# RozDavid/LanguageGroundedSemseg

Measured on AMD Instinct MI355X. Metric: voxels/sec fwd+bwd Res16UNet34C @2cm ScanNet200, higher is better.
Workload: dtype bf16

## Files before the change

### include/lgs_engine.h

```cpp
#ifndef LGS_ENGINE_H
#define LGS_ENGINE_H

#include <stdint.h>

#ifdef __cplusplus
extern "C" {
#endif

#define LGS_ABI_VERSION 18

enum lgs_dtype { LGS_F32 = 0, LGS_BF16 = 1 };
enum lgs_supcon_distance { LGS_SUPCON_COS = 0, LGS_SUPCON_L2 = 1 };

typedef struct lgs_manager lgs_manager;
typedef struct lgs_kmap lgs_kmap;
typedef struct lgs_segmap lgs_segmap;

int lgs_abi_version(void);
const char *lgs_last_error(void);

int lgs_tuning_set(const char *name, int64_t value);
int lgs_tuning_get(const char *name, int64_t *value);
int64_t lgs_tuning_describe(char *buf, int64_t cap);
int64_t lgs_debug_dispatch_counts(char *buf, int64_t cap, int reset);

int lgs_manager_create(int device, lgs_manager **out);
int lgs_manager_destroy(lgs_manager *mgr);
int lgs_manager_insert(lgs_manager *mgr, const int32_t *coords, int64_t n, int64_t *unique_index,
                       int64_t *inverse, void *stream, int *key, int64_t *n_unique);

int lgs_manager_stride2(lgs_manager *mgr, int in_key, void *stream, int *out_key, int64_t *n_out);
int lgs_manager_check(lgs_manager *mgr, int *flags);

int lgs_manager_parent_of(lgs_manager *mgr, int key, int *fine_key);

int lgs_manager_map_size(lgs_manager *mgr, int key, int64_t *n, int *tensor_stride);
int lgs_manager_get_coords(lgs_manager *mgr, int key, int32_t *dst, void *stream);

int lgs_manager_kernel_map(lgs_manager *mgr, int in_key, int out_key, int kernel_size, void *stream,
                           lgs_kmap **out);

int lgs_manager_kernel_map_ex(lgs_manager *mgr, int in_key, int out_key, int kernel_size, int dilation, void *stream,
                              lgs_kmap **out);

typedef struct lgs_kmap_relation_query {
  int entry;
  int ks, dilation;
  int link;
  int tensor_stride;
  int out_sorted;
  int in_origin, out_origin;
} lgs_kmap_relation_query;
typedef struct lgs_kmap_relation_info {
  int rc;
  int relation;
  int K;
  int strided;
  int bwd_mirror;
  int transposed_ok;
  int pairs_only[2];
  int served_by_old_entry;
} lgs_kmap_relation_info;
int lgs_debug_kmap_relation(const lgs_kmap_relation_query *q, lgs_kmap_relation_info *out);

int lgs_kmap_export(lgs_kmap *km, int32_t *k, int32_t *in_row, int32_t *out_row, void *stream, int64_t *m);

int lgs_manager_origin(lgs_manager *mgr, void *stream, int *out_key, int64_t *n_out);
int lgs_manager_segment_map(lgs_manager *mgr, int fine_key, int coarse_key, void *stream, lgs_segmap **out);
int lgs_segmap_size(const lgs_segmap *sm, int64_t *n_fine, int64_t *n_coarse);
int64_t lgs_seg_workspace_bytes(const lgs_segmap *sm, int c);
int lgs_seg_reduce(lgs_segmap *sm, int op, const void *x, const void *x2, int64_t x_ld, int c, void *out, int32_t *argmax,
                   int dtype, void *workspace, void *stream);
int lgs_seg_broadcast(lgs_segmap *sm, int op, const void *g, int c, const void *x, int64_t x_ld, void *out, int64_t out_ld,
                      int dtype, void *stream);
int lgs_seg_max_backward(lgs_segmap *sm, const void *dy, const int32_t *argmax, int c, void *dx, int dtype, void *stream);

int64_t lgs_in_workspace_bytes(const lgs_segmap *sm, int c);
int lgs_in_forward(lgs_segmap *sm, const void *x, int c, const float *weight, const float *bias, float eps, void *y,
                   float *stats , int dtype, void *workspace, void *stream);
int lgs_in_backward(lgs_segmap *sm, const void *x, const void *dy, int c, const float *weight, const float *stats, void *dx,
                    float *dweight, float *dbias, int dtype, void *workspace, void *stream);

int64_t lgs_conv_workspace_bytes(const lgs_kmap *km, int cin, int cout, int dtype, int op );

typedef struct lgs_pack_desc {
  const float *weight;
  void *packed;
  int64_t bytes, total;
  int K, cin_w, cout_w, transposed, mirror, g_real, o_real, ncp, nbp, dtype;
} lgs_pack_desc;
int lgs_conv_pack_desc(const lgs_kmap *km, int op , int transposed, int cin, int cout, int dtype,
                       lgs_pack_desc *out);
int lgs_pack_weights_batch(const lgs_pack_desc *descs_device, int n, int64_t max_total, void *stream);

int lgs_conv_bn_partial_rows(const lgs_kmap *km, int transposed, int cout, int dtype);
int lgs_conv_forward(lgs_kmap *km, int transposed, const void *in, int cin, const float *weight, int cout,
                     const float *bias, void *out, int dtype, void *workspace, float *bn_partial, const float *bn_pivot,
                     void *packed, int pack_mode, int in_row_stride , void *stream);
int lgs_conv_dgrad(lgs_kmap *km, int transposed, const void *grad_out, int cout, const float *weight, int cin,
                   void *grad_in, int dtype, void *workspace, void *packed, int pack_mode, void *stream);

int lgs_conv_dgrad_can_accumulate(const lgs_kmap *km, int transposed, int cin, int cout, int dtype);
int lgs_conv_dgrad_accumulate(lgs_kmap *km, int transposed, const void *grad_out, int cout, const float *weight, int cin,
                              void *grad_in, int dtype, void *workspace, void *packed, int pack_mode, void *stream);
int lgs_conv_wgrad(lgs_kmap *km, int transposed, const void *in, int cin, const void *grad_out, int cout,
                   float *grad_weight, int dtype, void *workspace, int in_row_stride , void *stream);
int lgs_conv_wgrad_supports_stride(const lgs_kmap *km, int transposed, int cin, int cout, int dtype, int in_row_stride);

typedef struct lgs_conv_plan_view {
  int64_t n_pad, n_in, n_out;
  int KS, K;
  int has_nbr, has_tile_k, has_out_row;
} lgs_conv_plan_view;
typedef struct lgs_conv_plan_query {
  lgs_conv_plan_view fwd, bwd;
  int ks;
  int op, transposed, cin, cout, dtype;
  int epilogue;
} lgs_conv_plan_query;
typedef struct lgs_conv_plan_region { int64_t offset, bytes; } lgs_conv_plan_region;
typedef struct lgs_conv_plan_info {
  int path;
  int tile_id, sc, wb, tm;
  int nc, nb_total, ncp, nbp, gc, wld;
  int64_t total;
  int pad_input, scratch_out, packed_ext_ok, split, bn_rows, can_accumulate;
  int64_t grid_x; int grid_y, grid_z;
  lgs_conv_plan_region packed, padded_in, scratch, bias, partials;
  int64_t bytes_total;
  int64_t workspace_bytes;
  int q_bn_partial_rows, q_can_accumulate;
  lgs_pack_desc pack_desc;
} lgs_conv_plan_info;
int lgs_debug_conv_plan(const lgs_conv_plan_query *q, lgs_conv_plan_info *out);

typedef struct lgs_wgrad_plan_query {
  lgs_conv_plan_view fwd, bwd;
  int ks, transposed, cin, cout, dtype, in_row_stride;
} lgs_wgrad_plan_query;
typedef struct lgs_wgrad_plan_info {
  int path;
  int bwd_view;
  int in_place;
  int pad_in, pad_gout;
  int all_cus;
  int f32_kernel;
  int t0, t1;
  int pad_a, pad_b;
  int slots;
  int64_t span;
  int n_ranges, kpw;
  int tasks_a, tasks_b;
  int cpl, n_chunks, xcd_map;
  int ntile;
  int64_t grid_x; int grid_y, grid_z, lds_bytes;
  int64_t reduce_blocks;
  lgs_conv_plan_region partials, padded_in, padded_gout, ww_count, ww_offset, ww_total, ww_pair_in, ww_pair_out;
  int64_t bytes_total;
  int64_t workspace_bytes;
  int supports_stride;
} lgs_wgrad_plan_info;
int lgs_debug_wgrad_plan(const lgs_wgrad_plan_query *q, lgs_wgrad_plan_info *out);

int64_t lgs_bn_workspace_bytes(int64_t n, int c);
int lgs_bn_forward(const void *x, int64_t n, int c, const float *gamma, const float *beta, float eps,
                   float momentum, float *running_mean, float *running_var, int64_t *num_batches_tracked,
                   const void *residual, int relu, void *y, float *stats, int dtype, void *workspace,
                   const float *conv_partials , int conv_partial_rows,
                   const float *pivot , int64_t y_row_stride ,
                   void *stream);
int lgs_bn_backward(const void *x, const void *y, const void *dy, int64_t dy_row_stride, int64_t n, int c,
                    const float *gamma, const float *beta, const float *stats, int relu, void *dx, void *dresidual,
                    float *dgamma, float *dbeta, int dtype, void *workspace, int64_t y_row_stride ,
                    void *stream);

int lgs_bn_stats(const void *x, int64_t n, int c, float *rec , int dtype, void *workspace,
                 const float *conv_partials, int conv_partial_rows, const float *pivot, void *stream);
int lgs_bn_sync_combine(const float *all_stats, int world, int c, float eps, float momentum, float *running_mean,
                        float *running_var, int64_t *num_batches_tracked, float *stats, float *inv_n_total, void *stream);
int lgs_bn_apply(const void *x, int64_t n, int c, const float *gamma, const float *beta, const float *stats,
                 const void *residual, int relu, void *y, int dtype, int64_t y_row_stride, void *stream);
int lgs_bn_backward_reduce(const void *x, const void *y, const void *dy, int64_t n, int c, const float *gamma,
                           const float *beta, const float *stats, int relu, float *sums, float *dgamma, float *dbeta,
                           int dtype, void *workspace, int64_t dy_row_stride, int64_t y_row_stride, void *stream);
int lgs_bn_backward_apply(const void *x, const void *y, const void *dy, int64_t n, int c, const float *gamma,
                          const float *beta, const float *stats, const float *sums, float inv_n_total,
                          const float *inv_n_device, int relu, void *dx, void *dresidual, int dtype, int64_t dy_row_stride,
                          int64_t y_row_stride, void *stream);

typedef struct lgs_norm_plan_query {
  int direction;
  int c, dtype;
  int conv_partial_rows;
  int resident_cap;
  int64_t n;
} lgs_norm_plan_query;
typedef struct lgs_norm_plan_info {
  int path;
  int from_partials;
  int reduce_grid;
  int64_t rows_per_block;
  int partial_rpb;
  int fold_rows;
  int fold_grid;
  int apply_grid;
  lgs_conv_plan_region partials, sums, spill;
  int64_t bytes_total;
  int64_t workspace_bytes;
} lgs_norm_plan_info;
int lgs_debug_norm_plan(const lgs_norm_plan_query *q, lgs_norm_plan_info *out);

struct lgs_bn_params;
typedef struct lgs_norm_pair_plan_info {
  int path;
  int single_path;
  int launches;
  int reduce_grid;
  int64_t rows_per_block;
  int fold_rows, fold_grid, apply_grid;
  lgs_conv_plan_region partials_a, partials_b, sums_a, sums_b;
  int64_t bytes_total;
  int64_t workspace_bytes;
} lgs_norm_pair_plan_info;
int64_t lgs_bn_pair_workspace_bytes(int64_t n, int c);
int lgs_bn_pair_plan(int direction , int64_t n, int c, int dtype, lgs_norm_pair_plan_info *out);
int lgs_debug_norm_pair_plan(const lgs_norm_plan_query *q , lgs_norm_pair_plan_info *out);
int lgs_bn_forward_pair(const void *xa, const struct lgs_bn_params *norm_a, float *stats_a, const void *xb,
                        const struct lgs_bn_params *norm_b, float *stats_b, int64_t n, int c, int relu, void *y,
                        int64_t y_row_stride , void *res , int dtype, void *workspace, void *stream);
int lgs_bn_backward_pair(const void *xa, const void *ya, const float *gamma_a, const float *beta_a, const float *stats_a, int relu,
                         const void *xb, const float *gamma_b, const float *stats_b, const void *dy, int64_t dy_row_stride,
                         int64_t n, int c, void *dxa, void *dxb, float *dgamma_a, float *dbeta_a, float *dgamma_b, float *dbeta_b,
                         void *dresidual , int dtype, void *workspace, int64_t ya_row_stride ,
                         void *stream);

typedef struct lgs_instnorm_plan_query {
  int direction;
  int c, dtype;
  int64_t n_fine, n_seg, n_items;
} lgs_instnorm_plan_query;
typedef struct lgs_instnorm_plan_info {
  int vec;
  int lanes_log2;
  int rows_per_apply_block;
  int64_t reduce_grid;
  int64_t combine_grid;
  int64_t apply_grid;
  lgs_conv_plan_region partials, sums;
  int64_t bytes_total;
  int64_t workspace_bytes;
} lgs_instnorm_plan_info;
int lgs_debug_instnorm_plan(const lgs_instnorm_plan_query *q, lgs_instnorm_plan_info *out);

typedef struct lgs_seg_plan_query {
  int family;
  int c, dtype;
  int single_pass;
  int vec_ok;
  int64_t n_fine, n_coarse, n_items;
} lgs_seg_plan_query;
typedef struct lgs_seg_plan_info {
  int vec;
  int lanes_log2;
  int combine_lanes_log2;
  int64_t reduce_grid;
  int64_t combine_grid;
  int64_t bcast_grid;
  int64_t max_bwd_grid;
  lgs_conv_plan_region partials, partial_argmax;
  int64_t bytes_total;
  int64_t workspace_bytes;
} lgs_seg_plan_info;
int lgs_debug_seg_plan(const lgs_seg_plan_query *q, lgs_seg_plan_info *out);

typedef struct lgs_comm lgs_comm;
int lgs_comm_unique_id(void *id128);
int lgs_comm_create(const void *id128, int world, int rank, int device, lgs_comm **out);
int lgs_comm_create_ipc(int world, int rank, int device, lgs_comm **out, void *handle64);
int lgs_comm_ipc_open(lgs_comm *comm, const void *handles64);
int lgs_comm_destroy(lgs_comm *comm);
int lgs_comm_world(const lgs_comm *comm);
int64_t lgs_bn_sync_workspace_bytes(int64_t n, int c, int world);
int lgs_bn_forward_sync(lgs_comm *comm, const void *x, int64_t n, int c, const float *gamma, const float *beta, float eps,
                        float momentum, float *running_mean, float *running_var, int64_t *num_batches_tracked,
                        const void *residual, int relu, void *y, float *stats, float *inv_n, int dtype, void *workspace,
                        int64_t y_row_stride, void *stream);
int lgs_bn_backward_sync(lgs_comm *comm, const void *x, const void *y, const void *dy, int64_t n, int c, const float *gamma,
                         const float *beta, const float *stats, const float *inv_n, int relu, void *dx, void *dresidual,
                         float *dgamma, float *dbeta, int dtype, void *workspace, int64_t dy_row_stride, int64_t y_row_stride,
                         void *stream);

typedef struct lgs_bn_params {
  const float *gamma, *beta;
  float *running_mean, *running_var;
  int64_t *num_batches_tracked;
  float eps, momentum;
} lgs_bn_params;
typedef struct lgs_block_fwd {
  lgs_kmap *km3, *km1;
  int dtype, relu_final, cin, planes;
  int64_t n;
  const void *x;
  const float *w1, *w2, *wd;
  void *pk1, *pk2, *pkd;
  int pm1, pm2, pmd;
  lgs_bn_params n1, n2, nd;
  void *o1, *y1, *o2, *od, *res, *y2;
  float *st1, *st2, *std_;
  void *conv_ws, *bn_ws;
} lgs_block_fwd;
typedef struct lgs_block_bwd {
  lgs_kmap *km3, *km1;
  int dtype, relu_final, cin, planes, want_gin, x_row_stride;
  int64_t n, dy_row_stride;
  const void *dy;
  const void *x, *o1, *y1, *o2, *y2, *od;
  const float *st1, *st2, *std_;
  const float *w1, *w2, *wd;
  void *pk1, *pk2, *pkd;
  int pm1, pm2, pmd;
  const float *gamma1, *beta1, *gamma2, *beta2, *gammad, *betad;
  void *dx2, *dres, *dy1, *dx1, *dxd, *gind;
  float *gw1, *gw2, *gwd;
  float *dgamma1, *dbeta1, *dgamma2, *dbeta2, *dgammad, *dbetad;
  void *conv_ws, *bn_ws;
  void *wgrad_stream, *wgrad_ws, *fork_event, *ev_w1, *ev_w2, *ev_wd;
} lgs_block_bwd;
int64_t lgs_block_workspace_bytes(const lgs_kmap *km3, const lgs_kmap *km1, int cin, int planes, int dtype);
int lgs_block_forward(const lgs_block_fwd *args, void *stream);
int lgs_block_backward(const lgs_block_bwd *args, void *stream);

int lgs_clip_similarity(const void *feat, int64_t n, int c, const float *anchors, int n_anchor, float *sim,
                        float *inv_norm_f, int dtype, void *workspace, void *stream);
int64_t lgs_clip_workspace_bytes(int c, int n_anchor, int dtype);

int64_t lgs_clip_loss_workspace_bytes(int c, int n_anchor, int dtype);
int lgs_clip_loss_forward(const void *feat, int64_t n, int c, const float *anchors, int n_anchor, const int64_t *labels,
                          const int64_t *neg, int k_neg, int64_t ignore_label, float *d_pos, float *d_neg, int64_t *pred,
                          float *inv_norm_f, float *anchors_n, float *sim, int dtype, void *workspace, void *stream);
int lgs_clip_loss_backward(const void *feat, int64_t n, int c, const float *anchors_n, int n_anchor, const int64_t *labels,
                           const int64_t *neg, int k_neg, int64_t ignore_label, const float *inv_norm_f, const float *d_pos,
                           const float *d_neg, const float *g_dpos, const float *g_dneg, void *grad_feat, int dtype,
                           void *stream);
int64_t lgs_clip_anchor_grad_workspace_bytes(int64_t n, int c, int n_anchor, int dtype);
int lgs_clip_loss_backward_anchors(const void *feat, int64_t n, int c, int n_anchor, const int64_t *labels, const int64_t *neg,
                                   int k_neg, int64_t ignore_label, const float *inv_norm_f, const float *g_dpos,
                                   const float *g_dneg, float *grad_anchors_t, int dtype, void *workspace, void *stream);

int lgs_sgd_step(float *params, const float *grads, float *momentum_buf, const float *mask, int64_t n, float lr,
                 float momentum, float dampening, float weight_decay, int first_step, void *stream);

int lgs_voxelize(const float *points, int64_t n, const double *affine, int batch, int32_t *coords, void *stream);
int lgs_label_vote(const int64_t *labels, int64_t n, const int64_t *unique_index, const int64_t *inverse,
                   int64_t n_unique, int64_t ignore_label, int64_t *labels_out, void *stream);

int64_t lgs_cluster_workspace_bytes(int64_t n);
int lgs_cluster(const float *xyz, const int32_t *batch_idx, const int32_t *semantic_label, int64_t n, float radius,
                int threshold, int32_t *component, int32_t *n_clusters, void *workspace, void *stream);

int lgs_ce_forward_backward(const void *logits, int64_t n, int c, const int64_t *labels, int64_t ignore_index,
                            const float *scale, float *loss_rows, void *dlogits, int dtype, void *stream);
int lgs_ce_forward_backward_rows(const void *logits, int64_t n, int c, const int64_t *labels, int64_t ignore_index,
                                 const float *scale, const float *row_scale, float *loss_rows, void *dlogits, int dtype,
                                 void *stream);
int lgs_split_stats(const float *loss_rows, const int64_t *labels, int64_t n, const int32_t *group_of_class, int n_classes,
                    int64_t ignore_index, float *partial, int partial_rows, void *stream);
int lgs_ce_count_valid(const int64_t *labels, int64_t n, int c, int64_t ignore_index, int32_t *count, void *stream);

// ... 54 lines not shown
```

### languagegroundedsemseg_amd/csrc/lgs_common.h

```cpp
#pragma once
#include <hip/hip_runtime.h>
#include <stdint.h>
#include <stdio.h>
#include <string>
#include <vector>

#include "../../include/lgs_engine.h"

struct lgs_kmap;
struct lgs_segmap;

namespace lgs {

void set_error(const std::string &msg);

#define LGS_HIP(expr)                                                                              \
  do {                                                                                             \
    hipError_t _e = (expr);                                                                        \
    if (_e != hipSuccess) {                                                                        \
      lgs::set_error(std::string(#expr) + " failed: " + hipGetErrorString(_e) + " (" __FILE__ ":" + \
                     std::to_string(__LINE__) + ")");                                              \
      return 1;                                                                                    \
    }                                                                                              \
  } while (0)

#define LGS_REQUIRE(cond, msg)                                                     \
  do {                                                                             \
    if (!(cond)) {                                                                 \
      lgs::set_error(std::string(msg) + " [" #cond "] (" __FILE__ ":" + std::to_string(__LINE__) + ")"); \
      return 2;                                                                    \
    }                                                                              \
  } while (0)

enum Tune {
  T_WW_MIN_ROWS, T_WW_RANGE, T_WGRAD_WIDE, T_BN_FUSED, T_BN_FUSED_MAX_MB, T_BN_FUSED_FWD_MAX_MB, T_BN_FUSED_BLOCKS, T_PS_CUS, T_PS_WIDE3, T_WGRAD_PS,
  T_MASK_WINDOW, T_CONV_SPLIT, T_SMALL_CFG, T_WIDE_GC64, T_ARENA_DBG, T_CONV_WIDE, T_MASK_ORDER,
  T_BN_FOLD, T_BN_FOLD_MAX_MB, T_BN_FOLD_PARTS, T_BN_FOLD_GRID, T_FP32_SPLIT, T_BLOCK_WGRAD_LATE, T_WGRAD_F32_LDS, T_WIDE_SCHED, T_HEAD_TILE, T_POINTWISE,
  T_INSTANCE_NORM, T_METRICS_BLOCKS, T_SUPCON_FUSED, T_BN_PAIR,
  T_COUNT
};
int64_t tune(Tune t);
int dispatch_site(const char *kernel_text, const char *pretty_function);
void dispatch_hit(int site);
#define LGS_KLAUNCH(kernel, ...)                                                                 \
  do {                                                                                           \
    static const int _lgs_site = lgs::dispatch_site(#kernel, __PRETTY_FUNCTION__);               \
    lgs::dispatch_hit(_lgs_site);                                                                \
    hipLaunchKernelGGL(kernel, __VA_ARGS__);                                                     \
  } while (0)

constexpr int kPadRows = 256;
constexpr int kGroup = 64;

inline int64_t pad_rows(int64_t n) { return (n + kPadRows - 1) / kPadRows * kPadRows; }

struct View {
  const int32_t *nbr = nullptr;
  const uint32_t *mask64 = nullptr;
  const int32_t *tile_k = nullptr;
  const int32_t *out_row = nullptr;
  int64_t n_pad = 0;
  int64_t n_out = 0;
  int64_t n_in = 0;
  int KS = 1;
  int K = 1;
  int mirror = 0;
};

constexpr int kSegChunk = 512;
struct SegMap {
  const int32_t *fine_row = nullptr;
  const int32_t *seg_start = nullptr;
  const int32_t *coarse_of = nullptr;
  const int32_t *item_start = nullptr;
  const int32_t *item_seg = nullptr;
  const int32_t *row_seg = nullptr;
  int64_t n_fine = 0, n_coarse = 0, n_items = 0;
  int64_t max_len = 0;
  bool single_pass() const { return max_len > 0 && max_len <= kSegChunk; }
};

inline int pad32(int c) { return (c + 31) / 32 * 32; }
inline int esize(int dtype) { return dtype == LGS_BF16 ? 2 : 4; }
inline int epl(int dtype) { return dtype == LGS_BF16 ? 8 : 4; }
inline int64_t align256(int64_t b) { return (b + 255) / 256 * 256; }

#if defined(__HIPCC__)
using f32x16 = __attribute__((ext_vector_type(16))) float;
using bf16x8 = __attribute__((ext_vector_type(8))) __bf16;
typedef uint16_t bf16_t;
__device__ inline float bf16_to_f32(uint16_t b) { return __uint_as_float((uint32_t)b << 16); }
__device__ inline uint16_t f32_to_bf16(float f) {
  uint32_t u = __float_as_uint(f);
  u += 0x7fffu + ((u >> 16) & 1u);
  return (uint16_t)(u >> 16);
}
__device__ inline float ld_elem(const float *p) { return *p; }
__device__ inline float ld_elem(const bf16_t *p) { return bf16_to_f32(*p); }
template <typename T>
__global__ void k_pad_rows(const T *__restrict__ src, int64_t n, int c, int cpad, T *__restrict__ dst) {
  int64_t i = (int64_t)blockIdx.x * blockDim.x + threadIdx.x;
  if (i >= n * cpad) return;
  int64_t r = i / cpad;
  int ch = (int)(i % cpad);
  dst[i] = ch < c ? src[r * c + ch] : (T)0;
}
#define LGS_AS3(p) ((__attribute__((address_space(3))) void *)(p))
#define LGS_VMCNT(n) __builtin_amdgcn_s_waitcnt((((n) & 15) | (7 << 4) | (15 << 8) | (((n) >> 4) << 14)))
#endif

using WgradPlan = lgs_wgrad_plan_info;
enum WgradPath { kWgEmpty = 0, kWgWide = 1, kWgPs = 2, kWgPairs = 3, kWgF32 = 4 };
int64_t wgrad_workspace_bytes(const lgs_kmap *km, int cin, int cout, int dtype);
inline lgs_conv_plan_region take_region(int64_t &used, int64_t bytes) {
  const lgs_conv_plan_region r = {used, align256(bytes)};
  used += r.bytes;
  return r;
}
bool pointwise_supported(const View &v, int K, int g_real, int o_real, int64_t in_ld);
int launch_pointwise(const View &v, const void *in, int64_t in_ld, int g_real, const float *w, int cin_w, int cout_w, int transposed,
                     int o_real, const float *bias, void *out, hipStream_t s);
bool pointwise_f32_supported(const View &v, int K, int g_real, int o_real, int64_t in_ld);
int launch_pointwise_f32(const View &v, const void *in, int64_t in_ld, int g_real, const float *w, int cin_w, int cout_w, int transposed,
                         int o_real, const float *bias, void *out, hipStream_t s);
int launch_conv_wide(const View &v, const void *in, int cin_real, int in_ld, const void *wp, int nb_total, int ncp, int nbp, int K,
                     void *out, int cout_real, const float *bias, int gc64, hipStream_t s);
bool wgrad_wide_plan(const View &v, int cin, int cout, int in_ld, WgradPlan &p);
int launch_wgrad_wide(const View &v, const WgradPlan &p, const void *in, int cin, int in_ld, const void *gout, int cout, float *gw,
                      void *workspace, hipStream_t s);
int kmap_wait(lgs_kmap *km, hipStream_t stream);
int segmap_wait(lgs_segmap *sm, hipStream_t stream);

}

namespace lgs {
enum KmapRelation {
  kRelIdentity = 0,
  kRelConv3 = 1,
  kRelConv2S2 = 2,
  kRelConv3Dilated = 3,
  kRelConv3S2 = 4,
  kRelConv1S2 = 5,
};
struct KmapTraits {
  int ks, K;
  bool strided;
  bool bwd_mirror;
  bool transposed_ok;
  bool old_entry;
  constexpr bool wgrad_pairs_only(bool transposed) const { return ks == 3 && (strided || transposed); }
};
constexpr KmapTraits traits_of(KmapRelation r) {
  switch (r) {
    case kRelConv3:        return KmapTraits{3, 27, false, true, false, true};
    case kRelConv2S2:      return KmapTraits{2, 8, true, false, true, true};
    case kRelConv3Dilated: return KmapTraits{3, 27, false, true, true, false};
    case kRelConv3S2:      return KmapTraits{3, 27, true, false, true, false};
    case kRelConv1S2:      return KmapTraits{1, 1, true, false, true, false};
    default:               return KmapTraits{1, 1, false, false, true, true};
  }
}
constexpr int kCoordBits = 18;
struct KmapRequest {
  bool ex;
  bool same_key;
  bool out_is_stride2;
  bool out_sorted;
  bool origin;
  int ks, dilation, ts_in;
};
inline const char *classify_kmap(const KmapRequest &q, KmapRelation &rel) {
  if (q.origin) return q.ex ? "lgs_manager_kernel_map_ex: no kernel maps on the origin map" : "lgs_manager_kernel_map: no kernel maps on the origin map";
  const int d = q.ex ? q.dilation : 1;
  const bool strided = !q.same_key && q.out_is_stride2;
  if (d < 1) return "lgs_manager_kernel_map_ex: dilation must be >= 1";
  if (strided && d > 1) return "lgs_manager_kernel_map_ex: stride 2 combined with dilation > 1 is not supported";
  if (d > 1 && q.ks != 3) return "lgs_manager_kernel_map_ex: dilation > 1 needs kernel_size 3";
  if (d > 1) {
    if (!q.same_key) return "lgs_manager_kernel_map_ex: out_key must be in_key or stride2(in_key)";
    rel = kRelConv3Dilated;
  } else if (q.ks == 1 || q.ks == 3) {
    const char *refusal = q.ks == 1 ? "kernel_size 1 needs in_key == out_key" : "kernel_size 3 is supported for stride 1 (in_key == out_key) only";
    if (!q.same_key && !strided) return refusal;
    rel = q.ks == 1 ? (strided ? kRelConv1S2 : kRelIdentity) : (strided ? kRelConv3S2 : kRelConv3);
    if (!q.ex && !traits_of(rel).old_entry) return refusal;
  } else if (q.ks == 2) {
    if (!strided) return "kernel_size 2 needs out_key == stride2(in_key)";
    rel = kRelConv2S2;
  } else {
    return "unsupported kernel_size (the model family uses 1, 2 and 3 only)";
  }
  if (!traits_of(rel).old_entry) {
    if (strided && !q.out_sorted) return "lgs_manager_kernel_map_ex: the stride-2 map's rows are not in sorted order";
    if ((int64_t)d * q.ts_in >= (1ll << (kCoordBits - 1))) return "lgs_manager_kernel_map_ex: dilation * tensor_stride must stay below 2^17";
  }
  return nullptr;
}
}

struct lgs_kmap {
  lgs_manager *mgr = nullptr;
  int in_key = -1, out_key = -1, ks = 1, K = 1;
  lgs::KmapRelation relation = lgs::kRelIdentity;
  int dilation = 1;
  lgs::View fwd;
  lgs::View bwd;
};

namespace lgs {
inline KmapTraits traits_of(const lgs_kmap *km) { return traits_of(km->relation); }
inline const char *synthetic_kmap_relation(lgs_kmap &km) {
  const bool same = km.ks != 2 && km.fwd.n_in == km.fwd.n_out;
  const char *refusal = classify_kmap(KmapRequest{true, same, !same, true, false, km.ks, 1, 1}, km.relation);
  if (!refusal) km.bwd.mirror = traits_of(km.relation).bwd_mirror ? 1 : 0;
  return refusal;
}
}

struct lgs_segmap {
  lgs_manager *mgr = nullptr;
  int fine_key = -1, coarse_key = -1;
  lgs::SegMap sm;
};
```

### languagegroundedsemseg_amd/csrc/lgs_manager.hip

```cpp
#include "lgs_common.h"

#include <cstring>
#include <memory>
#include <rocprim/rocprim.hpp>

namespace lgs {

static thread_local std::string g_err;
void set_error(const std::string &msg) { g_err = msg; }

constexpr int kBias = 1 << (kCoordBits - 1);
constexpr uint64_t kEmpty = ~0ull;

__host__ __device__ inline uint64_t spread3(uint64_t x) {
  x &= 0x1fffff;
  x = (x | x << 32) & 0x1f00000000ffffull;
  x = (x | x << 16) & 0x1f0000ff0000ffull;
  x = (x | x << 8) & 0x100f00f00f00f00full;
  x = (x | x << 4) & 0x10c30c30c30c30c3ull;
  x = (x | x << 2) & 0x1249249249249249ull;
  return x;
}
__host__ __device__ inline uint32_t compact3(uint64_t x) {
  x &= 0x1249249249249249ull;
  x = (x ^ (x >> 2)) & 0x10c30c30c30c30c3ull;
  x = (x ^ (x >> 4)) & 0x100f00f00f00f00full;
  x = (x ^ (x >> 8)) & 0x1f0000ff0000ffull;
  x = (x ^ (x >> 16)) & 0x1f00000000ffffull;
  x = (x ^ (x >> 32)) & 0x1fffff;
  return (uint32_t)x;
}
__device__ inline uint64_t pack_key(int b, int xb, int yb, int zb) {
  return ((uint64_t)b << 54) | spread3((uint64_t)xb) | (spread3((uint64_t)yb) << 1) | (spread3((uint64_t)zb) << 2);
}
__device__ inline void unpack_key(uint64_t key, int &b, int &xb, int &yb, int &zb) {
  b = (int)(key >> 54);
  uint64_t m = key & ((1ull << 54) - 1);
  xb = (int)compact3(m);
  yb = (int)compact3(m >> 1);
  zb = (int)compact3(m >> 2);
}
__device__ inline uint64_t hash64(uint64_t k) {
  k ^= k >> 33; k *= 0xff51afd7ed558ccdull; k ^= k >> 33; k *= 0xc4ceb9fe1a85ec53ull; k ^= k >> 33;
  return k;
}

__global__ void k_pack_keys(const int32_t *coords, int64_t n, uint64_t *keys, int32_t *vals, int *err) {
  int64_t i = (int64_t)blockIdx.x * blockDim.x + threadIdx.x;
  if (i >= n) return;
  int4 c = reinterpret_cast<const int4 *>(coords)[i];
  bool ok = c.x >= 0 && c.x < 1024 && c.y > -kBias && c.y < kBias - 64 && c.z > -kBias && c.z < kBias - 64 &&
            c.w > -kBias && c.w < kBias - 64;
  if (!ok) { atomicOr(err, 1); c = make_int4(0, 0, 0, 0); }
  keys[i] = pack_key(c.x, c.y + kBias, c.z + kBias, c.w + kBias);
  vals[i] = (int32_t)i;
}

__global__ void k_heads(const uint64_t *skeys, int64_t n, uint64_t keep_mask, int32_t *head) {
  int64_t p = (int64_t)blockIdx.x * blockDim.x + threadIdx.x;
  if (p >= n) return;
  uint64_t k = skeys[p] & keep_mask;
  head[p] = (p == 0 || (skeys[p - 1] & keep_mask) != k) ? 1 : 0;
}

__global__ void k_mark_first(const int32_t *svals, const int32_t *head, int64_t n, int32_t *is_first) {
  int64_t p = (int64_t)blockIdx.x * blockDim.x + threadIdx.x;
  if (p >= n) return;
  is_first[svals[p]] = head[p];
}
__global__ void k_emit_unique(const int32_t *coords, const int32_t *is_first, const int32_t *urow, int64_t n,
                              int32_t *ucoords, int64_t *unique_index) {
  int64_t i = (int64_t)blockIdx.x * blockDim.x + threadIdx.x;
  if (i >= n || !is_first[i]) return;
  int32_t u = urow[i];
  reinterpret_cast<int4 *>(ucoords)[u] = reinterpret_cast<const int4 *>(coords)[i];
  if (unique_index) unique_index[u] = i;
}
__global__ void k_emit_sorted(const uint64_t *skeys, const int32_t *svals, const int32_t *head,
                              const int32_t *runid_incl, const int32_t *urow, int64_t n, uint64_t *ukeys,
                              int32_t *order) {
  int64_t p = (int64_t)blockIdx.x * blockDim.x + threadIdx.x;
  if (p >= n || !head[p]) return;
  int32_t q = runid_incl[p] - 1;
  ukeys[q] = skeys[p];
  order[q] = urow[svals[p]];
}
__global__ void k_emit_inverse(const int32_t *svals, const int32_t *runid_incl, const int32_t *order, int64_t n,
                               int64_t *inverse) {
  int64_t p = (int64_t)blockIdx.x * blockDim.x + threadIdx.x;
  if (p >= n) return;
  inverse[svals[p]] = order[runid_incl[p] - 1];
}

__global__ void k_emit_coarse(const uint64_t *fkeys, const int32_t *head, const int32_t *cidx_incl, int64_t n,
                              uint64_t keep_mask, uint64_t *ckeys, int32_t *ccoords, int32_t *cstart,
                              int32_t *fine_cidx, int64_t nc, int *d_err) {
  int64_t p = (int64_t)blockIdx.x * blockDim.x + threadIdx.x;
  if (p >= n) return;
  int32_t q = cidx_incl[p] - 1;
  fine_cidx[p] = q;
  if (p == n - 1 && (int64_t)q + 1 != nc && d_err) atomicOr(d_err, 2);
  if (q >= nc) return;
  if (head[p]) {
    uint64_t k = fkeys[p] & keep_mask;
    ckeys[q] = k;
    cstart[q] = (int32_t)p;
    int b, x, y, z;
    unpack_key(k, b, x, y, z);
    reinterpret_cast<int4 *>(ccoords)[q] = make_int4(b, x - kBias, y - kBias, z - kBias);
  }
  if (p == n - 1) cstart[q + 1] = (int32_t)n;
}

__global__ void k_hash_fill(uint64_t *hkeys, int64_t cap) {
  int64_t i = (int64_t)blockIdx.x * blockDim.x + threadIdx.x;
  if (i < cap) hkeys[i] = kEmpty;
}
__global__ void k_hash_insert(const uint64_t *skeys, const int32_t *order, int64_t n, uint64_t *hkeys,
                              int32_t *hvals, uint64_t capm1) {
  int64_t p = (int64_t)blockIdx.x * blockDim.x + threadIdx.x;
  if (p >= n) return;
  uint64_t key = skeys[p];
  uint64_t s = hash64(key) & capm1;
  for (;;) {
    unsigned long long prev = atomicCAS(reinterpret_cast<unsigned long long *>(hkeys + s), (unsigned long long)kEmpty,
                                        (unsigned long long)key);
    if (prev == kEmpty) { hvals[s] = order ? order[p] : (int32_t)p; return; }
    s = (s + 1) & capm1;
  }
}

constexpr int kPreLevels = 8;
constexpr int kCountPerThread = 16;
constexpr int kBatchShift = 54;
__global__ __launch_bounds__(256) void k_count_levels(const uint64_t *__restrict__ skeys, int64_t n, int32_t *__restrict__ counts) {
  __shared__ int32_t l_cnt[kPreLevels + 1];
  if (threadIdx.x <= kPreLevels) l_cnt[threadIdx.x] = 0;
  __syncthreads();
  int32_t c[kPreLevels + 1];
#pragma unroll
  for (int L = 0; L <= kPreLevels; ++L) c[L] = 0;
  const int64_t base = (int64_t)blockIdx.x * 256 * kCountPerThread;
#pragma unroll 4
  for (int i = 0; i < kCountPerThread; ++i) {
    const int64_t p = base + (int64_t)i * 256 + threadIdx.x;
    if (p >= n) break;
    const uint64_t k = skeys[p], q = p > 0 ? skeys[p - 1] : ~0ull, d = k ^ q;
#pragma unroll
    for (int L = 1; L <= kPreLevels; ++L) c[L - 1] += (p == 0 || (d >> (3 * L)) != 0) ? 1 : 0;
    c[kPreLevels] += (p == 0 || (d >> kBatchShift) != 0) ? 1 : 0;
  }
#pragma unroll
  for (int L = 0; L <= kPreLevels; ++L) {
    int32_t v = c[L];
#pragma unroll
    for (int o = 32; o > 0; o >>= 1) v += __shfl_down(v, o, 64);
    if ((threadIdx.x & 63) == 0 && v) atomicAdd(&l_cnt[L], v);
  }
  __syncthreads();
  if (threadIdx.x <= kPreLevels && l_cnt[threadIdx.x]) atomicAdd(&counts[threadIdx.x], l_cnt[threadIdx.x]);
}

__global__ void k_build_map3(const uint64_t *skeys, int64_t n, int64_t n_pad, int ts, const uint64_t *hkeys,
                             const int32_t *hvals, uint64_t capm1, int32_t *nbr, uint32_t *pmask) {
  int64_t p = (int64_t)blockIdx.x * blockDim.x + threadIdx.x;
  bool live = p < n;
  int b = 0, x = 0, y = 0, z = 0;
  if (live) unpack_key(skeys[p], b, x, y, z);
  uint32_t m = 0;
#pragma unroll 1
  for (int g = 0; g < 3; ++g) {
    uint64_t key[9], slot[9], hk[9];
    bool ok[9];
    const int zz = z + (g - 1) * ts;
#pragma unroll
    for (int j = 0; j < 9; ++j) {
      const int xx = x + (j % 3 - 1) * ts, yy = y + (j / 3 - 1) * ts;
      ok[j] = live && (((unsigned)xx | (unsigned)yy | (unsigned)zz) < (1u << kCoordBits));
      key[j] = ok[j] ? pack_key(b, xx, yy, zz) : 0ull;
      slot[j] = hash64(key[j]) & capm1;
    }
#pragma unroll
    for (int j = 0; j < 9; ++j) hk[j] = ok[j] ? hkeys[slot[j]] : kEmpty;
#pragma unroll
    for (int j = 0; j < 9; ++j) {
      if (ok[j]) {
        uint64_t cur = hk[j], sl = slot[j];
        while (cur != key[j] && cur != kEmpty) {
          sl = (sl + 1) & capm1;
          cur = hkeys[sl];
        }
        slot[j] = sl;
        ok[j] = cur == key[j];
      }
    }
    int32_t r[9];
#pragma unroll
    for (int j = 0; j < 9; ++j) r[j] = ok[j] ? hvals[slot[j]] : -1;
#pragma unroll
    for (int j = 0; j < 9; ++j) {
      const int k = 9 * g + j;
      nbr[(int64_t)k * n_pad + p] = r[j];
      if (r[j] >= 0) m |= 1u << k;
    }
  }
  pmask[p] = m;
}

constexpr int kMaskWindow = 16384;
__device__ inline uint32_t mask_sort_code(uint32_t m, int order) {
  if (order == 0) return m;
  if (order == 3) return ((uint32_t)__popc(m) << 27) | m;
  uint32_t corner = 0, edge = 0, face = 0, centre = (m >> 13) & 1u;
  int nc = 0, ne = 0, nf = 0;
#pragma unroll
  for (int k = 0; k < 27; ++k) {
    const int dx = k % 3 - 1, dy = (k / 3) % 3 - 1, dz = k / 9 - 1;
    const int cls = (dx != 0) + (dy != 0) + (dz != 0);
    const uint32_t b = (m >> k) & 1u;
    if (cls == 3) corner |= b << nc++;
    else if (cls == 2) edge |= b << ne++;
    else if (cls == 1) face |= b << nf++;
  }
  if (order == 1) return (corner << 19) | (edge << 7) | (face << 1) | centre;
  return (face << 21) | (edge << 9) | (corner << 1) | centre;
}
__global__ void k_mask_sort_keys(const uint32_t *pmask, int64_t n, int64_t n_pad, int window, int order, uint64_t *keys, int32_t *vals) {
  int64_t p = (int64_t)blockIdx.x * blockDim.x + threadIdx.x;
  if (p >= n_pad) return;
  keys[p] = p < n ? (((uint64_t)(p / window)) << 32) | mask_sort_code(pmask[p], order) : ~0ull;
  vals[p] = (int32_t)p;
}
inline unsigned mask_sort_bits(int64_t n_pad, int window) {
  const uint64_t nw = (uint64_t)((n_pad + window - 1) / window);
  unsigned wb = 1;
  while ((1ull << wb) - 1 < nw) ++wb;
  return 32u + wb > 64u ? 64u : 32u + wb;
}
__global__ void k_permute_map3(const int32_t *nbr_tmp, const uint32_t *pmask, const int32_t *perm, const int32_t *order,
                               int64_t n, int64_t n_pad, int32_t *nbr, int32_t *out_row, uint32_t *mask64) {
  int64_t q = (int64_t)blockIdx.x * blockDim.x + threadIdx.x;
  int32_t src = q < n ? perm[q] : -1;
  uint32_t pm = src >= 0 ? pmask[src] : 0u;
  out_row[q] = src >= 0 ? (order ? order[src] : src) : -1;
  uint32_t m = 0;
  for (int k = 0; k < 27; ++k) {
    nbr[(int64_t)k * n_pad + q] = src >= 0 ? nbr_tmp[(int64_t)k * n_pad + src] : -1;
    if (__ballot((pm >> k) & 1u)) m |= 1u << k;
  }
  if ((threadIdx.x & 63) == 0) mask64[q >> 6] = m;
}

__global__ void k_build_map3_fine(const uint64_t *fkeys, int64_t n, int64_t n_pad, int log2ts, const uint64_t *hkeys,
                                  const int32_t *hvals, uint64_t capm1, int32_t *nbr, uint32_t *pmask) {
  int64_t p = (int64_t)blockIdx.x * blockDim.x + threadIdx.x;
  const bool live = p < n;
  int b = 0, x = 0, y = 0, z = 0;
  if (live) unpack_key(fkeys[p], b, x, y, z);
  const int ts = 1 << log2ts;
  const int ox = (x >> log2ts) & 1, oy = (y >> log2ts) & 1, oz = (z >> log2ts) & 1;
  uint64_t key[8], slot[8], hk[8];
  int kk[8];
  bool ok[8];
#pragma unroll
  for (int j = 0; j < 8; ++j) {
    const int jx = j & 1, jy = (j >> 1) & 1, jz = j >> 2;
    const int dx = ox ? 2 * jx - 1 : 0, dy = oy ? 2 * jy - 1 : 0, dz = oz ? 2 * jz - 1 : 0;
    const int xx = x - dx * ts, yy = y - dy * ts, zz = z - dz * ts;
    ok[j] = live && (ox || !jx) && (oy || !jy) && (oz || !jz) && (((unsigned)xx | (unsigned)yy | (unsigned)zz) < (1u << kCoordBits));
    kk[j] = (dx + 1) + 3 * (dy + 1) + 9 * (dz + 1);
    key[j] = ok[j] ? pack_key(b, xx, yy, zz) : 0ull;
    slot[j] = hash64(key[j]) & capm1;
  }
#pragma unroll
  for (int j = 0; j < 8; ++j) hk[j] = ok[j] ? hkeys[slot[j]] : kEmpty;
#pragma unroll
  for (int j = 0; j < 8; ++j) {
    if (ok[j]) {
      uint64_t cur = hk[j], sl = slot[j];
      while (cur != key[j] && cur != kEmpty) {
        sl = (sl + 1) & capm1;
        cur = hkeys[sl];
      }
      slot[j] = sl;
      ok[j] = cur == key[j];
    }
  }
  uint32_t m = 0;
#pragma unroll
  for (int j = 0; j < 8; ++j)
    if (ok[j]) m |= 1u << kk[j];
  int32_t r[8];
#pragma unroll
  for (int j = 0; j < 8; ++j) r[j] = ok[j] ? hvals[slot[j]] : -1;
  for (int k = 0; k < 27; ++k) {
    int32_t v = -1;
#pragma unroll
    for (int j = 0; j < 8; ++j)
      if (ok[j] && kk[j] == k) v = r[j];
    nbr[(int64_t)k * n_pad + p] = v;
  }
  pmask[p] = m;
}

__global__ void k_build_map1_coarse(const uint64_t *fkeys, const int32_t *forder, const uint64_t *ckeys, const int32_t *cstart,
                                    int64_t n_c, int64_t nc_pad, int32_t *nbr) {
  int64_t q = (int64_t)blockIdx.x * blockDim.x + threadIdx.x;
  if (q >= nc_pad) return;
  int32_t r = -1;
  if (q < n_c) {
    const int32_t p = cstart[q];
    if (fkeys[p] == ckeys[q]) r = forder ? forder[p] : p;
  }
  nbr[q] = r;
}
__global__ void k_build_map1_fine(const uint64_t *fkeys, const int32_t *forder, const int32_t *fine_cidx, int64_t n, int64_t n_pad,
                                  uint64_t child_bits, int32_t *nbr, int32_t *out_row) {
  int64_t p = (int64_t)blockIdx.x * blockDim.x + threadIdx.x;
  if (p >= n_pad) return;
  const bool live = p < n;
  nbr[p] = (live && (fkeys[p] & child_bits) == 0) ? fine_cidx[p] : -1;
  out_row[p] = live ? (forder ? forder[p] : (int32_t)p) : -1;
}

__global__ void k_build_map2_coarse(const uint64_t *fkeys, const int32_t *forder, const int32_t *cstart,
                                    int64_t n_c, int64_t nc_pad, int shift, int32_t *nbr8, uint32_t *mask64) {
  int64_t q = (int64_t)blockIdx.x * blockDim.x + threadIdx.x;
  int32_t child[8];
#pragma unroll
  for (int k = 0; k < 8; ++k) child[k] = -1;
  if (q < n_c) {
    int32_t s = cstart[q], e = cstart[q + 1];
    for (int32_t p = s; p < e; ++p) {
      int k = (int)((fkeys[p] >> shift) & 7);
      int32_t row = forder ? forder[p] : p;
#pragma unroll
      for (int j = 0; j < 8; ++j)
        if (j == k) child[j] = row;
    }
  }
  uint32_t m = 0;
#pragma unroll
  for (int k = 0; k < 8; ++k) {
    nbr8[(int64_t)k * nc_pad + q] = child[k];
    if (__ballot(child[k] >= 0)) m |= 1u << k;
  }
  if ((threadIdx.x & 63) == 0) mask64[q >> 6] = m;
}

__global__ void k_child_keys(const uint64_t *fkeys, int64_t n, int shift, uint32_t *kk, int32_t *pp, int32_t *cnt) {
  __shared__ int32_t h[8];
  if (threadIdx.x < 8) h[threadIdx.x] = 0;
  __syncthreads();
  int64_t p = (int64_t)blockIdx.x * blockDim.x + threadIdx.x;
  if (p < n) {
    uint32_t k = (uint32_t)((fkeys[p] >> shift) & 7);
    kk[p] = k;
    pp[p] = (int32_t)p;
    atomicAdd(&h[k], 1);
  }
  __syncthreads();
  if (threadIdx.x < 8 && h[threadIdx.x]) atomicAdd(&cnt[threadIdx.x], h[threadIdx.x]);
}
__global__ void k_group_offsets(const int32_t *cnt, int32_t *goff , int32_t *gsrc ) {
  if (threadIdx.x == 0 && blockIdx.x == 0) {
    int32_t a = 0, b = 0;
    for (int k = 0; k < 8; ++k) {
      goff[k] = a; gsrc[k] = b;
      a += (cnt[k] + kPadRows - 1) / kPadRows * kPadRows;
      b += cnt[k];
    }
    goff[8] = a; gsrc[8] = b;
  }
}
__global__ void k_fill_i32(int32_t *p, int64_t n, int32_t v) {
  int64_t i = (int64_t)blockIdx.x * blockDim.x + threadIdx.x;
  if (i < n) p[i] = v;
}
__global__ void k_build_map2_fine(const uint32_t *kk_sorted, const int32_t *pp_sorted, int64_t n, const int32_t *goff,
                                  const int32_t *gsrc, const int32_t *fine_cidx, const int32_t *forder,
                                  int32_t *g_nbr, int32_t *g_out, int32_t *tile_k) {
  int64_t s = (int64_t)blockIdx.x * blockDim.x + threadIdx.x;
  if (s >= n) return;
  int k = (int)kk_sorted[s];
  int32_t p = pp_sorted[s];
  int32_t slot = goff[k] + ((int32_t)s - gsrc[k]);
  g_nbr[slot] = fine_cidx[p];
  g_out[slot] = forder ? forder[p] : p;
  if (((s - gsrc[k]) & (kGroup - 1)) == 0) tile_k[slot >> 6] = k;
}

__global__ void k_view_count(View v, int32_t *count) {
  int64_t p = (int64_t)blockIdx.x * blockDim.x + threadIdx.x;
  if (p >= v.n_pad) return;
  int32_t orow = v.out_row ? v.out_row[p] : (p < v.n_out ? (int32_t)p : -1);
  int c = 0;
  if (orow >= 0) {
    if (!v.nbr) c = 1;
    else
      for (int s = 0; s < v.KS; ++s) c += v.nbr[(int64_t)s * v.n_pad + p] >= 0;
  }
  if (c) atomicAdd(count, c);
}
__global__ void k_view_export(View v, int32_t *cursor, int32_t *ek, int32_t *ein, int32_t *eout) {
  int64_t p = (int64_t)blockIdx.x * blockDim.x + threadIdx.x;
  if (p >= v.n_pad) return;
  int32_t orow = v.out_row ? v.out_row[p] : (p < v.n_out ? (int32_t)p : -1);
  if (orow < 0) return;
  for (int s = 0; s < v.KS; ++s) {
    int32_t i = v.nbr ? v.nbr[(int64_t)s * v.n_pad + p] : (int32_t)p;
    if (i < 0) continue;
    int k = v.tile_k ? v.tile_k[p >> 6] : (v.mirror ? v.K - 1 - s : s);
    int32_t at = atomicAdd(cursor, 1);
    ek[at] = k; ein[at] = i; eout[at] = orow;
  }
}

__global__ void k_origin_coords(const uint64_t *skeys, const int32_t *head, const int32_t *cincl, int64_t n, int64_t nb,
                                int32_t *coords, int *d_err) {
  int64_t p = (int64_t)blockIdx.x * blockDim.x + threadIdx.x;
  if (p >= n) return;
  const int32_t q = cincl[p] - 1;
  if (p == n - 1 && (int64_t)q + 1 != nb && d_err) atomicOr(d_err, 4);
  if (q >= nb || !head[p]) return;
  reinterpret_cast<int4 *>(coords)[q] = make_int4((int)(skeys[p] >> kBatchShift), 0, 0, 0);
}
__global__ void k_origin_segments(const int32_t *head, const int32_t *cincl, int64_t n, int64_t nb, int32_t *seg_start,
                                  int32_t *coarse_of) {
  int64_t p = (int64_t)blockIdx.x * blockDim.x + threadIdx.x;
  if (p >= n) return;
  const int32_t q = cincl[p] - 1;
  coarse_of[p] = q < nb ? q : (int32_t)(nb - 1);
  if (q >= nb) return;
  if (head[p]) seg_start[q] = (int32_t)p;
  if (p == n - 1) seg_start[q + 1] = (int32_t)n;
}
__global__ void k_row_seg(const int32_t *fine_row, const int32_t *coarse_of, int64_t n, int32_t *row_seg) {
  int64_t p = (int64_t)blockIdx.x * blockDim.x + threadIdx.x;
  if (p >= n) return;
  const int32_t r = fine_row[p];
  if (r >= 0 && r < n) row_seg[r] = coarse_of[p];
}
constexpr int kMaxChain = 12;
struct Chain {
  const int32_t *fine_cidx[kMaxChain];
  const int32_t *cstart[kMaxChain];
  int k;
};
__global__ void k_compose_coarse_of(Chain ch, int64_t n, int32_t *coarse_of) {
  int64_t p = (int64_t)blockIdx.x * blockDim.x + threadIdx.x;
  if (p >= n) return;
  int32_t v = (int32_t)p;
  for (int j = 0; j < ch.k; ++j) v = ch.fine_cidx[j][v];
  coarse_of[p] = v;
}
__global__ void k_compose_seg_start(Chain ch, int64_t nc, int32_t *seg_start) {
  int64_t q = (int64_t)blockIdx.x * blockDim.x + threadIdx.x;
  if (q > nc) return;
  int32_t v = (int32_t)q;
  for (int j = ch.k - 1; j >= 0; --j) v = ch.cstart[j][v];
  seg_start[q] = v;
}
__global__ void k_item_counts(const int32_t *seg_start, int64_t nc, int32_t *cnt) {
  int64_t q = (int64_t)blockIdx.x * blockDim.x + threadIdx.x;
  if (q >= nc) return;
  cnt[q] = (seg_start[q + 1] - seg_start[q] + kSegChunk - 1) / kSegChunk;
}
__global__ void k_item_fill(const int32_t *item_start, int64_t nc, int64_t n_items, int32_t *item_seg) {
  int64_t q = (int64_t)blockIdx.x * blockDim.x + threadIdx.x;
  if (q >= nc) return;
  for (int32_t j = item_start[q]; j < item_start[q + 1] && j < n_items; ++j) item_seg[j] = (int32_t)q;
}

struct CoordMap {
  int ts = 1, log2ts = 0;
  int64_t n = 0, n_pad = 0;
  int32_t *coords = nullptr;
  int32_t *order = nullptr;
  uint64_t *skeys = nullptr;
  uint64_t *hkeys = nullptr;
  int32_t *hvals = nullptr;
  int64_t hcap = 0;
  int fine_key = -1, coarse_key = -1;
  bool origin = false;
  int32_t *cstart = nullptr;
  int32_t *fine_cidx = nullptr;
};

}

using namespace lgs;

struct lgs_manager {
  int device = 0;
  hipMemPool_t pool = nullptr;
  hipStream_t ms = nullptr;
  hipEvent_t ev_ready = nullptr, ev_in = nullptr;
  std::vector<hipStream_t> users;
  hipStream_t last_stream = nullptr;
  std::vector<CoordMap> maps;
  std::vector<lgs_kmap *> kmaps;
  std::vector<void *> allocs;
  int *d_err = nullptr;
  char *arena = nullptr;
  size_t arena_cap = 0, arena_used = 0, arena_peak = 0;
  struct Blk { size_t off, size; bool freed; };
  std::vector<Blk> blks;
  size_t pool_live = 0, pool_peak = 0;
  int64_t precount[8] = {-1, -1, -1, -1, -1, -1, -1, -1};
  int64_t precount_batches = -1;
  int origin_key = -1;
  std::vector<lgs_segmap *> segmaps;
};

namespace {

struct DeviceGuard {
  int prev = -1;
  bool switched = false;
  explicit DeviceGuard(int dev) {
    if (hipGetDevice(&prev) == hipSuccess && prev != dev) switched = hipSetDevice(dev) == hipSuccess;
  }
  ~DeviceGuard() {
    if (switched) (void)hipSetDevice(prev);
  }
};

hipMemPool_t g_pool[64] = {nullptr};
int ensure_pool(int device) {
  if (g_pool[device]) return 0;
  hipMemPoolProps props;
  memset(&props, 0, sizeof(props));
  props.allocType = hipMemAllocationTypePinned;
  props.handleTypes = hipMemHandleTypeNone;
  props.location.type = hipMemLocationTypeDevice;
  props.location.id = device;
  hipMemPool_t pool = nullptr;
  LGS_HIP(hipMemPoolCreate(&pool, &props));
  uint64_t thr = UINT64_MAX;
  LGS_HIP(hipMemPoolSetAttribute(pool, hipMemPoolAttrReleaseThreshold, &thr));
  int off = 0;
  (void)hipMemPoolSetAttribute(pool, hipMemPoolReuseAllowInternalDependencies, &off);
  g_pool[device] = pool;
  return 0;
}
struct ArenaBlock { char *base; size_t cap; std::vector<hipEvent_t> ready; };
std::vector<ArenaBlock> g_arenas[64];
size_t g_arena_need[64] = {0};

inline hipError_t pool_alloc(lgs_manager *m, void **q, size_t bytes, hipStream_t s) {
  return hipMallocFromPoolAsync(q, bytes, m->pool, s);
}
int raw_alloc(lgs_manager *m, void **p, size_t bytes, hipStream_t s) {
  bytes = (bytes + 255) / 256 * 256;
  if (m->arena && m->arena_used + bytes <= m->arena_cap) {
    *p = m->arena + m->arena_used;
    m->blks.push_back({m->arena_used, bytes, false});
    m->arena_used += bytes;
    if (m->arena_used > m->arena_peak) m->arena_peak = m->arena_used;
    return 0;
  }
  void *q = nullptr;
  LGS_HIP(pool_alloc(m, &q, bytes, s));
  m->allocs.push_back(q);
  m->pool_live += bytes;
  if (m->pool_live > m->pool_peak) m->pool_peak = m->pool_live;
  *p = q;
  return 0;
}
template <typename T>
int dalloc(lgs_manager *m, T **p, int64_t count, hipStream_t s) {
  void *q = nullptr;
  if (raw_alloc(m, &q, sizeof(T) * (size_t)(count > 0 ? count : 1), s)) return 1;
  *p = reinterpret_cast<T *>(q);
  return 0;
}
int dfree_now(lgs_manager *m, void *q, hipStream_t s) {
  char *c = reinterpret_cast<char *>(q);
  if (m->arena && c >= m->arena && c < m->arena + m->arena_cap) {
    const size_t off = (size_t)(c - m->arena);
    for (size_t i = m->blks.size(); i-- > 0;)
      if (m->blks[i].off == off) { m->blks[i].freed = true; break; }
    while (!m->blks.empty() && m->blks.back().freed) { m->arena_used = m->blks.back().off; m->blks.pop_back(); }
    return 0;
  }
  for (size_t i = 0; i < m->allocs.size(); ++i)
    if (m->allocs[i] == q) { m->allocs[i] = m->allocs.back(); m->allocs.pop_back(); break; }
  LGS_HIP(hipFreeAsync(q, s));
  return 0;
}
int arena_acquire(lgs_manager *m) {
  const int dev = m->device;
  const size_t need = g_arena_need[dev];
  if (need == 0) return 0;
  std::vector<ArenaBlock> &q = g_arenas[dev];
  for (size_t i = 0; q.size() >= 2 && i + 1 < q.size(); ++i) {
    if (q[i].cap >= need) {
      ArenaBlock b = q[i];
      q.erase(q.begin() + (long)i);
      if (tune(T_ARENA_DBG)) {
        int pending = 0;
        for (hipEvent_t e : b.ready) pending += hipEventQuery(e) == hipSuccess ? 0 : 1;
        fprintf(stderr, "[arena] reuse block %zu of %zu (cap %zu MB, need %zu MB): %d of %zu events still pending\n", i, q.size() + 1, b.cap >> 20,
                need >> 20, pending, b.ready.size());
      }
      for (hipEvent_t e : b.ready) { (void)hipStreamWaitEvent(m->ms, e, 0); (void)hipEventDestroy(e); }
      m->arena = b.base; m->arena_cap = b.cap;
      return 0;
    }
    if (i == 0 && q.size() >= 4) {
      for (hipEvent_t e : q[0].ready) { (void)hipEventSynchronize(e); (void)hipEventDestroy(e); }
      (void)hipFree(q[0].base);
      q.erase(q.begin());
      i = (size_t)-1;
    }
  }
  const size_t cap = (need + need / 4 + (2u << 20)) / (2u << 20) * (2u << 20);
  if (tune(T_ARENA_DBG)) fprintf(stderr, "[arena] hipMalloc %zu MB (need %zu MB, %zu queued)\n", cap >> 20, need >> 20, q.size());
  void *p = nullptr;
  if (hipMalloc(&p, cap) != hipSuccess) { (void)hipGetLastError(); return 0; }
  m->arena = reinterpret_cast<char *>(p); m->arena_cap = cap;
  return 0;
}
void arena_release(lgs_manager *m) {
  const size_t need = m->arena_peak + m->pool_peak;
  if (need > g_arena_need[m->device]) g_arena_need[m->device] = need;
  if (!m->arena) return;
  ArenaBlock b{m->arena, m->arena_cap, {}};
  std::vector<hipStream_t> streams = m->users;
  streams.push_back(m->ms);
  for (hipStream_t u : streams) {
    hipEvent_t e = nullptr;
    if (hipEventCreateWithFlags(&e, hipEventDisableTiming) == hipSuccess) {
      if (hipEventRecord(e, u) == hipSuccess) b.ready.push_back(e); else (void)hipEventDestroy(e);
    }
  }
  g_arenas[m->device].push_back(b);
  m->arena = nullptr;
}
void add_user(lgs_manager *m, hipStream_t caller) {
  for (hipStream_t u : m->users)
    if (u == caller) return;
  m->users.push_back(caller);
}
int begin_from_caller(lgs_manager *m, hipStream_t caller) {
  LGS_HIP(hipEventRecord(m->ev_in, caller));
  LGS_HIP(hipStreamWaitEvent(m->ms, m->ev_in, 0));
  return 0;
}
int publish(lgs_manager *m, hipStream_t caller, bool caller_waits) {
  LGS_HIP(hipEventRecord(m->ev_ready, m->ms));
  if (caller_waits) {
    LGS_HIP(hipStreamWaitEvent(caller, m->ev_ready, 0));
    add_user(m, caller);
  }
  return 0;
}
inline unsigned nblk(int64_t n, int t = 256) { return (unsigned)((n + t - 1) / t > 0 ? (n + t - 1) / t : 1); }

int ensure_hash(lgs_manager *m, CoordMap &cm, hipStream_t s) {
  if (cm.hkeys) return 0;
  int64_t cap = 1024;
  while (cap < 2 * cm.n) cap <<= 1;
  cm.hcap = cap;
  if (dalloc(m, &cm.hkeys, cap, s)) return 1;
  if (dalloc(m, &cm.hvals, cap, s)) return 1;
  LGS_KLAUNCH(k_hash_fill, nblk(cap), 256, 0, s, cm.hkeys, cap);
  if (cm.n > 0)
    LGS_KLAUNCH(k_hash_insert, nblk(cm.n), 256, 0, s, cm.skeys, cm.order, cm.n, cm.hkeys, cm.hvals,
                       (uint64_t)(cap - 1));
  LGS_HIP(hipGetLastError());
  return 0;
}

int scan_incl(lgs_manager *m, const int32_t *in, int32_t *out, int64_t n, hipStream_t s) {
  size_t tb = 0;
  LGS_HIP(rocprim::inclusive_scan(nullptr, tb, in, out, (size_t)n, rocprim::plus<int32_t>(), s));
  void *tmp = nullptr;
  if (raw_alloc(m, &tmp, tb ? tb : 16, s)) return 1;
  LGS_HIP(rocprim::inclusive_scan(tmp, tb, in, out, (size_t)n, rocprim::plus<int32_t>(), s));
  if (dfree_now(m, tmp, s)) return 1;
  return 0;
}

template <typename K, typename V>
int sort_pairs(lgs_manager *m, K *keys, K *keys_out, V *vals, V *vals_out, int64_t n, unsigned begin_bit, unsigned end_bit, hipStream_t s) {
  size_t tb = 0;
  LGS_HIP(rocprim::radix_sort_pairs(nullptr, tb, keys, keys_out, vals, vals_out, (size_t)n, begin_bit, end_bit, s));
  void *tmp = nullptr;
  if (raw_alloc(m, &tmp, tb ? tb : 16, s)) return 1;
  LGS_HIP(rocprim::radix_sort_pairs(tmp, tb, keys, keys_out, vals, vals_out, (size_t)n, begin_bit, end_bit, s));
  return dfree_now(m, tmp, s);
}

int batch_heads(lgs_manager *m, const uint64_t *skeys, int64_t n, int32_t *head, int32_t *cincl, hipStream_t s) {
  LGS_KLAUNCH(k_heads, nblk(n), 256, 0, s, skeys, n, ~((1ull << kBatchShift) - 1), head);
  return scan_incl(m, head, cincl, n, s);
}

int sort_map3(lgs_manager *m, int64_t n, int64_t n_pad, const int32_t *nbr_tmp, const uint32_t *pmask, const int32_t *order, uint64_t *keys,
              uint64_t *skeys2, int32_t *vals, int32_t *perm, int32_t *nbr, int32_t *orow, uint32_t *mask, hipStream_t s) {
  const int window = (int)tune(T_MASK_WINDOW);
  LGS_KLAUNCH(k_mask_sort_keys, (unsigned)(n_pad / 256), 256, 0, s, pmask, n, n_pad, window, (int)tune(T_MASK_ORDER), keys, vals);
  if (sort_pairs(m, keys, skeys2, vals, perm, n_pad, 0, mask_sort_bits(n_pad, window), s)) return 1;
  LGS_KLAUNCH(k_permute_map3, (unsigned)(n_pad / 256), 256, 0, s, nbr_tmp, pmask, perm, order, n, n_pad, nbr, orow, mask);
  LGS_HIP(hipGetLastError());
  return 0;
}

template <typename Build>
int make_view27(lgs_manager *m, const CoordMap &st, int64_t n_in, hipStream_t s, View &v, Build &&build) {
  v = View();
  v.n_pad = st.n_pad; v.n_out = st.n; v.n_in = n_in; v.KS = 27; v.K = 27;
  if (st.n == 0) return 0;
  int32_t *nbr, *orow, *nbr_tmp, *vals, *perm; uint32_t *mask, *pmask; uint64_t *keys, *skeys2;
  if (dalloc(m, &nbr, 27 * st.n_pad, s) || dalloc(m, &mask, st.n_pad / kGroup, s) || dalloc(m, &orow, st.n_pad, s) ||
      dalloc(m, &nbr_tmp, 27 * st.n_pad, s) || dalloc(m, &pmask, st.n_pad, s) || dalloc(m, &keys, st.n_pad, s) ||
      dalloc(m, &skeys2, st.n_pad, s) || dalloc(m, &vals, st.n_pad, s) || dalloc(m, &perm, st.n_pad, s))
    return 1;
  if (build(nbr_tmp, pmask)) return 1;
  if (sort_map3(m, st.n, st.n_pad, nbr_tmp, pmask, st.order, keys, skeys2, vals, perm, nbr, orow, mask, s)) return 1;
  if (dfree_now(m, nbr_tmp, s) || dfree_now(m, pmask, s) || dfree_now(m, keys, s) || dfree_now(m, skeys2, s) ||
      dfree_now(m, vals, s) || dfree_now(m, perm, s))
    return 1;
  v.nbr = nbr; v.mask64 = mask; v.out_row = orow;
  return 0;
}


void build_identity(const CoordMap &ci, lgs_kmap *km) {
  View v; v.n_pad = ci.n_pad; v.n_out = ci.n; v.n_in = ci.n; v.KS = 1; v.K = 1;
  km->fwd = v; km->bwd = v;
}

int probe_view27(lgs_manager *m, const CoordMap &st, const CoordMap &probed, int scale, hipStream_t s, View &v) {
  return make_view27(m, st, probed.n, s, v, [&](int32_t *nbr_tmp, uint32_t *pmask) {
    LGS_KLAUNCH(k_build_map3, (unsigned)(st.n_pad / 256), 256, 0, s, st.skeys, st.n, st.n_pad, scale, probed.hkeys, probed.hvals,
                (uint64_t)(probed.hcap - 1), nbr_tmp, pmask);
    return 0;
  });
}

int build_conv3(lgs_manager *m, CoordMap &ci, int dilation, hipStream_t s, lgs_kmap *km) {
  if (ci.n > 0 && ensure_hash(m, ci, s)) return 1;
  View v;
  if (probe_view27(m, ci, ci, dilation * ci.ts, s, v)) return 1;
  km->fwd = v;
  km->bwd = v; km->bwd.mirror = 1;
  return 0;
}

int build_conv2_s2(lgs_manager *m, const CoordMap &ci, const CoordMap &co, hipStream_t s, lgs_kmap *km) {
  int shift = 3 * ci.log2ts;
  View vf, vb;
  vf.KS = 8; vf.K = 8; vf.n_pad = co.n_pad; vf.n_out = co.n; vf.n_in = ci.n;
  vb.KS = 1; vb.K = 8; vb.n_out = ci.n; vb.n_in = co.n;
  if (ci.n > 0) {
    int32_t *nbr8; uint32_t *mask;
    if (dalloc(m, &nbr8, 8 * co.n_pad, s) || dalloc(m, &mask, co.n_pad / kGroup, s)) return 1;
    LGS_KLAUNCH(k_build_map2_coarse, (unsigned)(co.n_pad / 256), 256, 0, s, ci.skeys, ci.order, co.cstart, co.n,
                       co.n_pad, shift, nbr8, mask);
    vf.nbr = nbr8; vf.mask64 = mask;
    int64_t n = ci.n, gp = pad_rows(n + 8 * kPadRows);
    uint32_t *kk, *kks; int32_t *pp, *pps, *cnt, *goff, *gsrc, *g_nbr, *g_out, *tile_k;
    if (dalloc(m, &kk, n, s) || dalloc(m, &kks, n, s) || dalloc(m, &pp, n, s) || dalloc(m, &pps, n, s) ||
        dalloc(m, &cnt, 8, s) || dalloc(m, &goff, 9, s) || dalloc(m, &gsrc, 9, s) || dalloc(m, &g_nbr, gp, s) ||
        dalloc(m, &g_out, gp, s) || dalloc(m, &tile_k, gp / kGroup, s))
      return 1;
    LGS_HIP(hipMemsetAsync(cnt, 0, 8 * sizeof(int32_t), s));
    LGS_KLAUNCH(k_child_keys, nblk(n), 256, 0, s, ci.skeys, n, shift, kk, pp, cnt);
    if (sort_pairs(m, kk, kks, pp, pps, n, 0, 3, s)) return 1;
    LGS_KLAUNCH(k_group_offsets, 1, 64, 0, s, cnt, goff, gsrc);
    LGS_KLAUNCH(k_fill_i32, nblk(gp), 256, 0, s, g_nbr, gp, -1);
    LGS_KLAUNCH(k_fill_i32, nblk(gp), 256, 0, s, g_out, gp, -1);
    LGS_KLAUNCH(k_fill_i32, nblk(gp / kGroup), 256, 0, s, tile_k, gp / kGroup, -1);
    LGS_KLAUNCH(k_build_map2_fine, nblk(n), 256, 0, s, kks, pps, n, goff, gsrc, co.fine_cidx, ci.order, g_nbr,
                       g_out, tile_k);
    LGS_HIP(hipGetLastError());
    vb.nbr = g_nbr; vb.out_row = g_out; vb.tile_k = tile_k; vb.n_pad = gp;
    if (dfree_now(m, kk, s) || dfree_now(m, kks, s) || dfree_now(m, pp, s) || dfree_now(m, pps, s) ||
        dfree_now(m, cnt, s) || dfree_now(m, goff, s) || dfree_now(m, gsrc, s))
      return 1;
  }
  km->fwd = vf; km->bwd = vb;
  return 0;
}

int build_conv3_s2(lgs_manager *m, CoordMap &ci, CoordMap &co, hipStream_t s, lgs_kmap *km) {
  if (ci.n > 0 && (ensure_hash(m, ci, s) || ensure_hash(m, co, s))) return 1;
  if (probe_view27(m, co, ci, ci.ts, s, km->fwd)) return 1;
  return make_view27(m, ci, co.n, s, km->bwd, [&](int32_t *nbr_tmp, uint32_t *pmask) {
    LGS_KLAUNCH(k_build_map3_fine, (unsigned)(ci.n_pad / 256), 256, 0, s, ci.skeys, ci.n, ci.n_pad, ci.log2ts, co.hkeys, co.hvals,
                (uint64_t)(co.hcap - 1), nbr_tmp, pmask);
    return 0;
  });
}

int build_conv1_s2(lgs_manager *m, const CoordMap &ci, const CoordMap &co, hipStream_t s, lgs_kmap *km) {
  View vf, vb;
  vf.KS = 1; vf.K = 1; vf.n_pad = co.n_pad; vf.n_out = co.n; vf.n_in = ci.n;
  vb.KS = 1; vb.K = 1; vb.n_pad = ci.n_pad; vb.n_out = ci.n; vb.n_in = co.n;
  if (ci.n > 0) {
    int32_t *nf, *nb, *ob;
    if (dalloc(m, &nf, co.n_pad, s) || dalloc(m, &nb, ci.n_pad, s) || dalloc(m, &ob, ci.n_pad, s)) return 1;
    LGS_KLAUNCH(k_build_map1_coarse, nblk(co.n_pad), 256, 0, s, ci.skeys, ci.order, co.skeys, co.cstart, co.n, co.n_pad, nf);
    LGS_KLAUNCH(k_build_map1_fine, nblk(ci.n_pad), 256, 0, s, ci.skeys, ci.order, co.fine_cidx, ci.n, ci.n_pad, 7ull << (3 * ci.log2ts), nb, ob);
    LGS_HIP(hipGetLastError());
    vf.nbr = nf; vb.nbr = nb; vb.out_row = ob;
  }
  km->fwd = vf; km->bwd = vb;
  return 0;
}

int kernel_map(bool ex, const char *who, lgs_manager *m, int in_key, int out_key, int ks, int dilation, lgs_kmap **out) {
  LGS_REQUIRE(m && out, std::string(who) + ": null argument");
  const int nm = (int)m->maps.size();
  LGS_REQUIRE(in_key >= 0 && in_key < nm && out_key >= 0 && out_key < nm, std::string(who) + ": bad key");
  CoordMap &ci = m->maps[in_key], &co = m->maps[out_key];
  KmapRelation rel = kRelIdentity;
  const char *refusal = classify_kmap(KmapRequest{ex, in_key == out_key, co.fine_key == in_key, co.order == nullptr, ci.origin || co.origin, ks,
                                                  dilation, ci.ts}, rel);
  LGS_REQUIRE(refusal == nullptr, refusal);
  const KmapTraits t = traits_of(rel);
  if (rel != kRelConv3Dilated) dilation = 1;
  for (lgs_kmap *k : m->kmaps)
    if (k->in_key == in_key && k->out_key == out_key && k->relation == rel && k->dilation == dilation) { *out = k; return 0; }
  hipStream_t s = m->ms;
  DeviceGuard guard(m->device);
  std::unique_ptr<lgs_kmap> km(new lgs_kmap());
  km->mgr = m; km->in_key = in_key; km->out_key = out_key; km->ks = t.ks; km->K = t.K; km->relation = rel; km->dilation = dilation;
  int rc = 0;
  switch (rel) {
    case kRelIdentity: build_identity(ci, km.get()); break;
    case kRelConv3:
    case kRelConv3Dilated: rc = build_conv3(m, ci, dilation, s, km.get()); break;
    case kRelConv2S2: rc = build_conv2_s2(m, ci, co, s, km.get()); break;
    case kRelConv3S2: rc = build_conv3_s2(m, ci, co, s, km.get()); break;
    case kRelConv1S2: rc = build_conv1_s2(m, ci, co, s, km.get()); break;
  }
  if (rc) return rc;
  m->kmaps.push_back(km.get());
  *out = km.release();
  return publish(m, nullptr, false);
}
}

namespace lgs {
int kmap_wait(lgs_kmap *km, hipStream_t stream) {
  lgs_manager *m = km->mgr;
  LGS_HIP(hipStreamWaitEvent(stream, m->ev_ready, 0));
  add_user(m, stream);
  return 0;
}
int segmap_wait(lgs_segmap *sm, hipStream_t stream) {
  lgs_manager *m = sm->mgr;
  LGS_HIP(hipStreamWaitEvent(stream, m->ev_ready, 0));
  add_user(m, stream);
  return 0;
}
}

extern "C" {

int lgs_abi_version(void) { return LGS_ABI_VERSION; }
const char *lgs_last_error(void) { return g_err.c_str(); }

int lgs_manager_create(int device, lgs_manager **out) {
  LGS_REQUIRE(out != nullptr, "lgs_manager_create: null out");
  LGS_REQUIRE(device >= 0 && device < 64, "lgs_manager_create: device index out of range");
  DeviceGuard guard(device);
  if (ensure_pool(device)) return 1;
  lgs_manager *m = new lgs_manager();
  m->device = device;
  m->pool = g_pool[device];
  static hipStream_t g_map_stream[64] = {nullptr};
  if (!g_map_stream[device]) LGS_HIP(hipStreamCreateWithFlags(&g_map_stream[device], hipStreamNonBlocking));
  m->ms = g_map_stream[device];
  LGS_HIP(hipEventCreateWithFlags(&m->ev_ready, hipEventDisableTiming));
  LGS_HIP(hipEventCreateWithFlags(&m->ev_in, hipEventDisableTiming));
  arena_acquire(m);
  *out = m;
  return 0;
}

int lgs_manager_destroy(lgs_manager *m) {
  if (!m) return 0;
  DeviceGuard guard(m->device);
  hipStream_t fs = m->users.empty() ? m->ms : m->users.back();
  if (!m->users.empty()) {
    for (hipStream_t u : m->users) {
      if (u == fs) continue;
      if (hipEventRecord(m->ev_in, u) == hipSuccess) (void)hipStreamWaitEvent(fs, m->ev_in, 0);
    }
    (void)hipStreamWaitEvent(fs, m->ev_ready, 0);
  }
  for (void *p : m->allocs) (void)hipFreeAsync(p, fs);
  arena_release(m);
  for (lgs_kmap *k : m->kmaps) delete k;
  for (lgs_segmap *k : m->segmaps) delete k;
  (void)hipEventDestroy(m->ev_ready);
  (void)hipEventDestroy(m->ev_in);
  delete m;
  return 0;
}

int lgs_manager_insert(lgs_manager *m, const int32_t *coords, int64_t n, int64_t *unique_index, int64_t *inverse,
                       void *stream, int *key, int64_t *n_unique) {
  LGS_REQUIRE(m && key && n_unique, "lgs_manager_insert: null argument");
  LGS_REQUIRE(m->maps.empty(), "lgs_manager_insert: manager already holds a stride-1 map");
  LGS_REQUIRE(n >= 0 && n < (1ll << 31) - 1024, "lgs_manager_insert: row count out of range");
  hipStream_t caller = (hipStream_t)stream;
  hipStream_t s = m->ms;
  DeviceGuard guard(m->device);
  m->last_stream = caller;
  if (begin_from_caller(m, caller)) return 1;
  CoordMap cm;
  if (n == 0) {
    cm.n = 0; cm.n_pad = 0;
    m->maps.push_back(cm);
    *key = 0; *n_unique = 0;
    return 0;
  }
  if (!m->d_err) { if (dalloc(m, &m->d_err, 1, s)) return 1; }
  LGS_HIP(hipMemsetAsync(m->d_err, 0, sizeof(int), s));
  uint64_t *keys, *skeys; int32_t *vals, *svals, *head, *runid, *is_first, *urow;
  if (dalloc(m, &keys, n, s) || dalloc(m, &skeys, n, s) || dalloc(m, &vals, n, s) || dalloc(m, &svals, n, s) ||
      dalloc(m, &head, n, s) || dalloc(m, &runid, n, s) || dalloc(m, &is_first, n, s) || dalloc(m, &urow, n + 1, s))
    return 1;
  LGS_KLAUNCH(k_pack_keys, nblk(n), 256, 0, s, coords, n, keys, vals, m->d_err);
  if (sort_pairs(m, keys, skeys, vals, svals, n, 0, 64, s)) return 1;
  LGS_KLAUNCH(k_heads, nblk(n), 256, 0, s, skeys, n, ~0ull, head);
  LGS_KLAUNCH(k_mark_first, nblk(n), 256, 0, s, svals, head, n, is_first);
  if (scan_incl(m, head, runid, n, s)) return 1;
  {
    LGS_HIP(hipMemsetAsync(urow, 0, sizeof(int32_t), s));
    if (scan_incl(m, is_first, urow + 1, n, s)) return 1;
  }
  int32_t *lvl_counts;
  if (dalloc(m, &lvl_counts, kPreLevels + 1, s)) return 1;
  LGS_HIP(hipMemsetAsync(lvl_counts, 0, sizeof(int32_t) * (kPreLevels + 1), s));
  LGS_KLAUNCH(k_count_levels, (unsigned)((n + 256 * kCountPerThread - 1) / (256 * kCountPerThread)), 256, 0, s, skeys, n, lvl_counts);
  int32_t h_nu = 0; int h_err = 0; int32_t h_lvl[kPreLevels + 1];
  LGS_HIP(hipMemcpyAsync(&h_nu, urow + n, sizeof(int32_t), hipMemcpyDeviceToHost, s));
  LGS_HIP(hipMemcpyAsync(&h_err, m->d_err, sizeof(int), hipMemcpyDeviceToHost, s));
  LGS_HIP(hipMemcpyAsync(h_lvl, lvl_counts, sizeof(int32_t) * (kPreLevels + 1), hipMemcpyDeviceToHost, s));
  LGS_HIP(hipStreamSynchronize(s));
  for (int i = 0; i < kPreLevels; ++i) m->precount[i] = h_lvl[i];
  m->precount_batches = h_lvl[kPreLevels];
  LGS_REQUIRE(h_err == 0,
              "lgs_manager_insert: coordinate out of range (batch must be in [0,1024), |x|,|y|,|z| < 131008)");
  int64_t nu = h_nu;
  cm.n = nu; cm.n_pad = pad_rows(nu);
  if (dalloc(m, &cm.coords, nu * 4, s) || dalloc(m, &cm.order, nu, s) || dalloc(m, &cm.skeys, nu, s)) return 1;
  LGS_KLAUNCH(k_emit_unique, nblk(n), 256, 0, s, coords, is_first, urow, n, cm.coords, unique_index);
  LGS_KLAUNCH(k_emit_sorted, nblk(n), 256, 0, s, skeys, svals, head, runid, urow, n, cm.skeys, cm.order);
  if (inverse) LGS_KLAUNCH(k_emit_inverse, nblk(n), 256, 0, s, svals, runid, cm.order, n, inverse);
  LGS_HIP(hipGetLastError());
  if (dfree_now(m, keys, s) || dfree_now(m, skeys, s) || dfree_now(m, vals, s) || dfree_now(m, svals, s) ||
      dfree_now(m, head, s) || dfree_now(m, runid, s) || dfree_now(m, is_first, s) || dfree_now(m, urow, s) || dfree_now(m, lvl_counts, s))
    return 1;
  m->maps.push_back(cm);
  *key = 0; *n_unique = nu;
  return publish(m, caller, true);
}

int lgs_manager_stride2(lgs_manager *m, int in_key, void *stream, int *out_key, int64_t *n_out) {
  LGS_REQUIRE(m && out_key && n_out, "lgs_manager_stride2: null argument");
  LGS_REQUIRE(in_key >= 0 && in_key < (int)m->maps.size(), "lgs_manager_stride2: bad key");
  LGS_REQUIRE(!m->maps[in_key].origin, "lgs_manager_stride2: the origin map has no coarser map");
  hipStream_t s = m->ms;
  (void)stream;
  DeviceGuard guard(m->device);
  if (m->maps[in_key].coarse_key >= 0) {
    *out_key = m->maps[in_key].coarse_key; *n_out = m->maps[*out_key].n;
    return 0;
  }
  CoordMap f = m->maps[in_key];
  LGS_REQUIRE(f.log2ts < 12, "lgs_manager_stride2: tensor stride too large");
  CoordMap c;
  c.ts = f.ts * 2; c.log2ts = f.log2ts + 1; c.fine_key = in_key;
  int64_t n = f.n;
  if (n == 0) {
    m->maps.push_back(c);
    m->maps[in_key].coarse_key = (int)m->maps.size() - 1;
    *out_key = m->maps[in_key].coarse_key; *n_out = 0;
    return 0;
  }
  uint64_t keep = ~(7ull << (3 * f.log2ts));
  int32_t *head, *cincl;
  if (dalloc(m, &head, n, s) || dalloc(m, &cincl, n, s)) return 1;
  LGS_KLAUNCH(k_heads, nblk(n), 256, 0, s, f.skeys, n, keep, head);
  if (scan_incl(m, head, cincl, n, s)) return 1;
  int64_t nc;
  if (c.log2ts >= 1 && c.log2ts <= kPreLevels && m->precount[c.log2ts - 1] >= 0) {
    nc = m->precount[c.log2ts - 1];
  } else {
    int32_t h_nc = 0;
    LGS_HIP(hipMemcpyAsync(&h_nc, cincl + (n - 1), sizeof(int32_t), hipMemcpyDeviceToHost, s));
    LGS_HIP(hipStreamSynchronize(s));
    nc = h_nc;
  }
  c.n = nc; c.n_pad = pad_rows(nc);
  if (dalloc(m, &c.coords, nc * 4, s) || dalloc(m, &c.skeys, nc, s) || dalloc(m, &c.cstart, nc + 1, s) ||
      dalloc(m, &c.fine_cidx, n, s))
    return 1;
  LGS_KLAUNCH(k_emit_coarse, nblk(n), 256, 0, s, f.skeys, head, cincl, n, keep, c.skeys, c.coords, c.cstart,
                     c.fine_cidx, nc, m->d_err);
  LGS_HIP(hipGetLastError());
  if (dfree_now(m, head, s) || dfree_now(m, cincl, s)) return 1;
  m->maps.push_back(c);
  int ck = (int)m->maps.size() - 1;
  m->maps[in_key].coarse_key = ck;
  *out_key = ck; *n_out = nc;
  return publish(m, nullptr, false);
}

int lgs_manager_check(lgs_manager *m, int *flags) {
  LGS_REQUIRE(m && flags, "lgs_manager_check: null argument");
  *flags = 0;
  if (!m->d_err) return 0;
  DeviceGuard guard(m->device);
  int h = 0;
  LGS_HIP(hipMemcpyAsync(&h, m->d_err, sizeof(int), hipMemcpyDeviceToHost, m->ms));
  LGS_HIP(hipStreamSynchronize(m->ms));
  *flags = h;
  return 0;
}

int lgs_manager_parent_of(lgs_manager *m, int key, int *fine_key) {
  LGS_REQUIRE(m && fine_key && key >= 0 && key < (int)m->maps.size(), "lgs_manager_parent_of: bad argument");
  *fine_key = m->maps[key].fine_key;
  return 0;
}

int lgs_manager_map_size(lgs_manager *m, int key, int64_t *n, int *tensor_stride) {
  LGS_REQUIRE(m && key >= 0 && key < (int)m->maps.size(), "lgs_manager_map_size: bad key");
  if (n) *n = m->maps[key].n;
  if (tensor_stride) *tensor_stride = m->maps[key].ts;
  return 0;
}

int lgs_manager_get_coords(lgs_manager *m, int key, int32_t *dst, void *stream) {
  LGS_REQUIRE(m && key >= 0 && key < (int)m->maps.size(), "lgs_manager_get_coords: bad key");
  const CoordMap &cm = m->maps[key];
  if (begin_from_caller(m, (hipStream_t)stream)) return 1;
  if (cm.n > 0)
    LGS_HIP(hipMemcpyAsync(dst, cm.coords, sizeof(int32_t) * 4 * (size_t)cm.n, hipMemcpyDeviceToDevice, m->ms));
  return publish(m, (hipStream_t)stream, true);
}

int lgs_manager_kernel_map(lgs_manager *m, int in_key, int out_key, int ks, void *stream, lgs_kmap **out) {
  (void)stream;
  return kernel_map(false, "lgs_manager_kernel_map", m, in_key, out_key, ks, 1, out);
}

int lgs_manager_kernel_map_ex(lgs_manager *m, int in_key, int out_key, int ks, int dilation, void *stream, lgs_kmap **out) {
  (void)stream;
  return kernel_map(true, "lgs_manager_kernel_map_ex", m, in_key, out_key, ks, dilation, out);
}

int lgs_debug_kmap_relation(const lgs_kmap_relation_query *q, lgs_kmap_relation_info *out) {
  LGS_REQUIRE(q && out && (q->entry == 0 || q->entry == 1) && q->link >= 0 && q->link <= 3, "lgs_debug_kmap_relation: bad argument");
  *out = lgs_kmap_relation_info{};
  KmapRelation rel = kRelIdentity;
  const char *refusal = classify_kmap(KmapRequest{q->entry == 1, q->link == 0, q->link == 1, q->out_sorted != 0, q->in_origin || q->out_origin, q->ks,
                                                  q->dilation, q->tensor_stride}, rel);
  out->rc = refusal ? 2 : 0;
  out->relation = -1;
  LGS_REQUIRE(refusal == nullptr, refusal);
  const KmapTraits t = traits_of(rel);
  out->relation = rel; out->K = t.K; out->strided = t.strided; out->bwd_mirror = t.bwd_mirror; out->transposed_ok = t.transposed_ok;
  out->pairs_only[0] = t.wgrad_pairs_only(false); out->pairs_only[1] = t.wgrad_pairs_only(true);
  out->served_by_old_entry = t.old_entry;
  return 0;
}

int lgs_manager_origin(lgs_manager *m, void *stream, int *out_key, int64_t *n_out) {
  LGS_REQUIRE(m && out_key && n_out, "lgs_manager_origin: null argument");
  LGS_REQUIRE(!m->maps.empty(), "lgs_manager_origin: the manager holds no map yet");
  (void)stream;
  if (m->origin_key >= 0) {
    *out_key = m->origin_key; *n_out = m->maps[m->origin_key].n;
    return 0;
  }
  hipStream_t s = m->ms;
  DeviceGuard guard(m->device);
  const CoordMap f = m->maps[0];
  CoordMap o;
  o.ts = 0; o.log2ts = 0; o.origin = true;
  const int64_t n = f.n;
  const int64_t nb = n > 0 ? m->precount_batches : 0;
  LGS_REQUIRE(nb >= 0, "lgs_manager_origin: batch count unknown");
  o.n = nb; o.n_pad = pad_rows(nb);
  if (n > 0) {
    int32_t *head, *cincl;
    if (dalloc(m, &o.coords, nb * 4, s) || dalloc(m, &head, n, s) || dalloc(m, &cincl, n, s)) return 1;
    if (batch_heads(m, f.skeys, n, head, cincl, s)) return 1;
    LGS_KLAUNCH(k_origin_coords, nblk(n), 256, 0, s, f.skeys, head, cincl, n, nb, o.coords, m->d_err);
    LGS_HIP(hipGetLastError());
    if (dfree_now(m, head, s) || dfree_now(m, cincl, s)) return 1;
  }
  m->maps.push_back(o);
  m->origin_key = (int)m->maps.size() - 1;
  *out_key = m->origin_key; *n_out = nb;
  return publish(m, nullptr, false);
}

int lgs_manager_segment_map(lgs_manager *m, int fine_key, int coarse_key, void *stream, lgs_segmap **out) {
  LGS_REQUIRE(m && out, "lgs_manager_segment_map: null argument");
  const int nm = (int)m->maps.size();
  LGS_REQUIRE(fine_key >= 0 && fine_key < nm && coarse_key >= 0 && coarse_key < nm, "lgs_manager_segment_map: bad key");
  LGS_REQUIRE(!m->maps[fine_key].origin, "lgs_manager_segment_map: the fine map is the origin map");
  for (lgs_segmap *k : m->segmaps)
    if (k->fine_key == fine_key && k->coarse_key == coarse_key) { *out = k; return 0; }
  (void)stream;
  const CoordMap &cf = m->maps[fine_key];
  const CoordMap &cc = m->maps[coarse_key];
  Chain ch;
  ch.k = 0;
  if (!cc.origin) {
    int levels[kMaxChain];
    int c = coarse_key;
    while (c != fine_key) {
      LGS_REQUIRE(c >= 0 && !m->maps[c].origin && ch.k < kMaxChain,
                  "lgs_manager_segment_map: the coarse map is neither the origin map nor a stride-2^k descendant of the fine map");
      levels[ch.k++] = c;
      c = m->maps[c].fine_key;
    }
    LGS_REQUIRE(ch.k >= 1, "lgs_manager_segment_map: fine and coarse map are the same map");
    for (int j = 0; j < ch.k; ++j) {
      const CoordMap &lv = m->maps[levels[ch.k - 1 - j]];
      ch.fine_cidx[j] = lv.fine_cidx;
      ch.cstart[j] = lv.cstart;
    }
  }
  hipStream_t s = m->ms;
  DeviceGuard guard(m->device);
  SegMap sm;
  sm.n_fine = cf.n; sm.n_coarse = cc.n;
  sm.fine_row = cf.order;
  sm.max_len = cc.origin ? 0 : (int64_t)1 << (3 * ch.k);
  const int64_t n = cf.n, nc = cc.n;
  if (n > 0) {
    if (cc.origin) {
      int32_t *head, *cincl, *seg_start, *coarse_of;
      if (dalloc(m, &seg_start, nc + 1, s) || dalloc(m, &coarse_of, n, s) || dalloc(m, &head, n, s) || dalloc(m, &cincl, n, s))
        return 1;
      if (batch_heads(m, cf.skeys, n, head, cincl, s)) return 1;
      LGS_KLAUNCH(k_origin_segments, nblk(n), 256, 0, s, head, cincl, n, nc, seg_start, coarse_of);
      LGS_HIP(hipGetLastError());
      if (dfree_now(m, head, s) || dfree_now(m, cincl, s)) return 1;
      sm.seg_start = seg_start; sm.coarse_of = coarse_of; sm.row_seg = coarse_of;
      if (cf.order) {
        int32_t *row_seg;
        if (dalloc(m, &row_seg, n, s)) return 1;
        LGS_KLAUNCH(k_row_seg, nblk(n), 256, 0, s, cf.order, coarse_of, n, row_seg);
        LGS_HIP(hipGetLastError());
        sm.row_seg = row_seg;
      }
    } else if (ch.k == 1) {
      sm.seg_start = ch.cstart[0]; sm.coarse_of = ch.fine_cidx[0];
    } else {
      int32_t *seg_start, *coarse_of;
      if (dalloc(m, &seg_start, nc + 1, s) || dalloc(m, &coarse_of, n, s)) return 1;
      LGS_KLAUNCH(k_compose_coarse_of, nblk(n), 256, 0, s, ch, n, coarse_of);
      LGS_KLAUNCH(k_compose_seg_start, nblk(nc + 1), 256, 0, s, ch, nc, seg_start);
      LGS_HIP(hipGetLastError());
      sm.seg_start = seg_start; sm.coarse_of = coarse_of;
    }
    if (!sm.single_pass()) {
      const int64_t n_items = n / kSegChunk + nc + 1;
      int32_t *cnt, *item_start, *item_seg;
      if (dalloc(m, &item_start, nc + 1, s) || dalloc(m, &item_seg, n_items, s) || dalloc(m, &cnt, nc, s)) return 1;
      LGS_KLAUNCH(k_item_counts, nblk(nc), 256, 0, s, sm.seg_start, nc, cnt);
      LGS_HIP(hipMemsetAsync(item_start, 0, sizeof(int32_t), s));
      if (scan_incl(m, cnt, item_start + 1, nc, s)) return 1;
      LGS_KLAUNCH(k_fill_i32, nblk(n_items), 256, 0, s, item_seg, n_items, -1);
      LGS_KLAUNCH(k_item_fill, nblk(nc), 256, 0, s, item_start, nc, n_items, item_seg);
      LGS_HIP(hipGetLastError());
      if (dfree_now(m, cnt, s)) return 1;
      sm.item_start = item_start; sm.item_seg = item_seg; sm.n_items = n_items;
    }
  }
  lgs_segmap *h = new lgs_segmap();
  h->mgr = m; h->fine_key = fine_key; h->coarse_key = coarse_key; h->sm = sm;
  m->segmaps.push_back(h);
  *out = h;
  return publish(m, nullptr, false);
}

int lgs_kmap_export(lgs_kmap *km, int32_t *ek, int32_t *ein, int32_t *eout, void *stream, int64_t *mcount) {
  LGS_REQUIRE(km && mcount, "lgs_kmap_export: null argument");
  lgs_manager *m = km->mgr;
  hipStream_t caller = (hipStream_t)stream;
  hipStream_t s = m->ms;
  DeviceGuard guard(m->device);
  if (begin_from_caller(m, caller)) return 1;
  const View &v = km->fwd;
  int32_t *cnt;
  if (raw_alloc(m, (void **)&cnt, sizeof(int32_t), s)) return 1;
  LGS_HIP(hipMemsetAsync(cnt, 0, sizeof(int32_t), s));
  if (v.n_pad > 0) {
    if (ek) LGS_KLAUNCH(k_view_export, nblk(v.n_pad), 256, 0, s, v, cnt, ek, ein, eout);
    else LGS_KLAUNCH(k_view_count, nblk(v.n_pad), 256, 0, s, v, cnt);
  }
  int32_t h = 0;
  LGS_HIP(hipMemcpyAsync(&h, cnt, sizeof(int32_t), hipMemcpyDeviceToHost, s));
  LGS_HIP(hipStreamSynchronize(s));
  if (dfree_now(m, cnt, s)) return 1;
  *mcount = h;
  return publish(m, caller, true);
}

}
```

### languagegroundedsemseg_amd/csrc/lgs_tuning.hip

```cpp
#include <atomic>
#include <mutex>
#include <stdio.h>
#include <stdlib.h>
#include <string.h>

#include "lgs_common.h"

namespace lgs {

namespace {
struct Knob { Tune id; const char *name; int64_t def; const char *doc; };
const Knob kKnobs[T_COUNT] = {
    {T_WW_MIN_ROWS, "WW_MIN_ROWS", 200000, "k_wgrad_wide (per-offset GEMM over compacted pair lists) is used for 3^3 weight gradients with >= 256 x 256 "
                            "channels on maps of at least this many positions; below, k_wgrad_ps wins (81 k rows, 256->256: 0.82 vs 0.31 ms)"},
    {T_WW_RANGE, "WW_RANGE", 16384, "positions per k_wgrad_wide workgroup range (multiple of 256; 8192 overflows the partial-tile cap, 65536: 8.6 vs 7.5 ms)"},
    {T_WGRAD_WIDE, "WGRAD_WIDE", 1, "0 = never use k_wgrad_wide (A/B)"},
    {T_BN_FUSED, "BN_FUSED", 1, "0 = BatchNorm always as three launches (column sums, fold, apply) instead of the persistent grid-barrier kernels; "
                    "required when several processes time-share one GPU"},
    {T_BN_FUSED_MAX_MB, "BN_FUSED_MAX_MB", 24, "layers above this size use the three-launch BatchNorm (they are bandwidth-bound; the 4096-workgroup apply streams faster)"},
    {T_BN_FUSED_FWD_MAX_MB, "BN_FUSED_FWD_MAX_MB", 0, "the same bound for the FORWARD direction alone; 0 = the forward is always three launches.  Round 4: with the host "
                               "no longer the bound the one-launch forward loses at every size (8-scene step 27.93 vs 28.15 ms, one scene 10.17 vs "
                               "10.30; stand-alone 20 MB: 22.8 vs 33.0 us), the one-launch BACKWARD still wins (16.4 vs 16.8 ms of backward)"},
    {T_BN_FUSED_BLOCKS, "BN_FUSED_BLOCKS", 0, "workgroups of the fused BatchNorm kernels; 0 = min(256, co-resident workgroups of the device)"},
    {T_PS_CUS, "PS_CUS", 20, "CUs per XCD that k_wgrad_ps fills (of 32): the compute stream keeps CUs of its own next to the CU-owning weight gradient"},
    {T_PS_WIDE3, "PS_WIDE3", 1, "k_wgrad_ps: three-block stationary slices for >= 256-channel layers (0 = two-block)"},
    {T_WGRAD_PS, "WGRAD_PS", 1, "0 = force the round-1 pair-list weight gradient (k_wgrad_bf16) everywhere (debugging)"},
    {T_MASK_WINDOW, "MASK_WINDOW", 16384, "3^3 maps: positions per window inside which rows are re-sorted by their 27-bit neighbour mask (1024 .. 65536 swept)"},
    {T_CONV_SPLIT, "CONV_SPLIT", 1, "0 = no slot split (3 x 9 offsets into fp32 partial images) for under-filled coarse-level 3^3 launches"},
    {T_SMALL_CFG, "SMALL_CFG", 0, "k_conv_gather tile for maps < 65536 positions: 0 = automatic (id 8), 5 / 9 / 10 / 11 = the other measured shapes"},
    {T_WIDE_GC64, "WIDE_GC64", 1, "k_conv_wide: 64-channel stages per reduction group"},
    {T_ARENA_DBG, "ARENA_DBG", 0, "print coordinate-manager arena allocations to stderr"},
    {T_CONV_WIDE, "CONV_WIDE", 1, "0 = >= 256-output-channel layers stay on k_conv_gather's 8-wave tile (id 16) instead of k_conv_wide (A/B)"},
    {T_MASK_ORDER, "MASK_ORDER", 0, "3^3 maps: sort code of the neighbourhood mask inside a window: 0 the mask, 1 corners > edges > faces, 2 faces > edges > corners, 3 popcount-major"},
    {T_BN_FOLD, "BN_FOLD", 1, "1 = BatchNorm layers up to BN_FOLD_MAX_MB run as TWO launches per direction: column sums into <= BN_FOLD_PARTS partial rows, "
                   "then an apply kernel whose workgroups fold the partial rows themselves (no fold launch, no grid barrier); 0 = the round-4 "
                   "policies (grid-barrier kernel backward, three launches forward)"},
    {T_BN_FOLD_MAX_MB, "BN_FOLD_MAX_MB", 6, "layers above this size keep the round-4 policies.  Stand-alone (tools/dbg/bn_small.py, bf16): 2.6 MB 15.2 / 21.1 us forward / backward against 16.1 / 29.0 (three launches / grid barriers), 5 MB 17.8 / 26.0 against 16.0 / 27.6; at 10 - 20 MB the wider 512-row reduction wins (22 / 37 - 59 against 16 - 23 / 32 - 46)"},
    {T_BN_FOLD_PARTS, "BN_FOLD_PARTS", 64, "partial rows of the two-launch BatchNorm (<= 64): fewer = a shorter fold in every apply workgroup, more = a wider reduction"},
    {T_BN_FOLD_GRID, "BN_FOLD_GRID", 256, "apply workgroups of the two-launch BatchNorm (each folds the partial rows redundantly)"},
    {T_FP32_SPLIT, "FP32_SPLIT", 1, "fp32 tensors: 1 = convolution forward / dgrad multiply on the bf16 matrix pipe with exactly split operands (x = hi + mid + lo, "
                      "six bf16 products accumulated in fp32: error below 2^-22 |x||w|, 2.7 x the MFMA rate of v_mfma_f32_32x32x2_f32); "
                      "0 = the exact-fp32 MFMA instance"},
    {T_BLOCK_WGRAD_LATE, "BLOCK_WGRAD_LATE", 0, "A/B: 1 = lgs_block_backward forks the FIRST convolution's weight gradient after the block's last dgrad instead of "
                            "beside it (the 96->128 dgrad of block8.0 runs 2.1 x its stand-alone time next to k_wgrad_ps 128->96)"},
    {T_WGRAD_F32_LDS, "WGRAD_F32_LDS", 2, "fp32 weight gradients: 2 = rows staged through LDS as three exactly-split bf16 planes, six bf16 MFMAs per 16 pairs "
                                          "(k_wgrad_f32s_lds; dropped terms < 2^-24 |x g|, fp32 accumulate).  Stand-alone it wins at >= 96 input channels only "
                                          "(96 -> 96: 3.06 vs 3.38 ms; 32 -> 32: 1.06 vs 0.84), in the STEP it wins everywhere: 82.4 - 82.9 vs 86.1 - 86.7 ms -- it "
                                          "holds the matrix pipe 2.7 x shorter than the exact-fp32 MFMA and the convolutions on the other stream get it "
                                          "(round 6); 3 = split only where it also wins stand-alone (83.5 - 83.7 ms); 1 = exact-fp32 MFMA on staged rows "
                                          "(k_wgrad_f32_lds; bit-identical to 0); 0 = k_wgrad_f32 (one 4-byte load per lane and MFMA operand)"},
    {T_WIDE_SCHED, "WIDE_SCHED", 0, "k_conv_wide: where the two waves of a SIMD issue the next stage's LDS-DMA between their four row blocks.  0 = "
                                    "weights first / gathers after block 1 (round 3); 1 = gathers first, weights after block 1; 2 = gathers first, "
                                    "weights after block 0; 3 = gathers first, weights after block 2; 4 = both first (round 2's schedule)"},
    {T_HEAD_TILE, "HEAD_TILE", 0, "1x1 layers with 5 - 7 output blocks on the big maps (the 200-class head): 0 = one 128-position tile spans all output "
                                  "channels (the feature matrix is streamed once; 7 x 16 accumulator registers per wave), 1 = the generic 4-block tile "
                                  "(two column tiles, features read twice, 3 waves per SIMD)"},
    {T_POINTWISE, "POINTWISE", 1, "bf16 1x1 stride-1 convolutions (and their dgrads) on maps of >= 65536 positions with <= 224 output channels run on "
                                  "k_pointwise (persistent streaming GEMM, lgs_pointwise.hip) instead of k_conv_gather's identity-map tiles where that wins (5 - 7 output "
                                  "blocks, or > 128 reduction channels into 3 blocks: the 200-class head and its dgrad); 2 = every shape it serves; 0 = off (A/B)"},
    {T_INSTANCE_NORM, "INSTANCE_NORM", 1, "MinkowskiInstanceNorm on HIP tensors: 1 = the per-scene kernels of lgs_instnorm.hip (two passes per direction, no host "
                                          "synchronisation, reproducible); 0 = the torch lines the CPU path uses (index_add_ on fp32 copies, one .item() per "
                                          "call) -- read at call time: for timing the old path in the same process and for switching the kernels off in the field"},
    {T_METRICS_BLOCKS, "METRICS_BLOCKS", 8192, "most workgroups of a k_seg_metrics launch (lgs_metrics.hip); each walks tiles blockIdx.x, + gridDim.x, ... and adds its "
                                               "LDS table of (label, pred) counts to the confusion matrix once at its end, so a cell costs at most this many "
                                               "global atomics per call.  1.2 M x 200 bf16, no prob, uniform / 90 %-on-one-cell labels: 2048 373 / 273 us (two "
                                               "uneven rounds of resident workgroups), 4096 284 / 228, 8192 242 / 220, 16384 231 / 264, one tile per workgroup "
                                               "234 / 497 (37 500 adds on one address); small values let a test walk many tiles per workgroup on a few thousand rows"},
    {T_SUPCON_FUSED, "SUPCON_FUSED", 1, "PointSupConLoss on HIP tensors: 1 = the kernels of lgs_supcon.hip (k_supcon_sample, k_supcon_fwd, k_supcon_bwd: (1 + P + K) row "
                                        "reads per point, no [N, P + K, C] tensor); 0 = the torch gather path CPU tensors take (index gathers, normalise, mean) and "
                                        "the torch restatement of the sampler -- read at call time: for timing the two next to each other and for switching "
                                        "the kernels off in the field"},
    {T_BN_PAIR, "BN_PAIR", 1, "BatchNorm passes shared inside a residual block (paths `three` and `fold`; A/B): 1 = lgs_bn_backward masks dy ONCE when it "
                              "also returns the residual gradient (the reduce launch writes the masked gradient, the apply reads it back: 7 tensor "
                              "passes instead of 8), and lgs_bn_forward_pair / lgs_bn_backward_pair run the two norms of a downsample block on shared "
                              "reads (5 instead of 7 passes forward, 10 instead of 13 backward, 3 launches instead of 6); 0 = the single calls, dy "
                              "masked in both launches.  Bit-identical either way"},
};
std::atomic<int64_t> g_val[T_COUNT];
std::once_flag g_once;

void init_knobs() {
  for (int i = 0; i < T_COUNT; ++i) {
    if ((int)kKnobs[i].id != i) {
      fprintf(stderr, "lgs_engine: tuning table row %d is %s but enum Tune says otherwise -- fix csrc/lgs_tuning.hip\n", i, kKnobs[i].name);
      abort();
    }
    const std::string env = std::string("LGS_") + kKnobs[i].name;
    const char *e = getenv(env.c_str());
    g_val[i].store(e ? atoll(e) : kKnobs[i].def, std::memory_order_relaxed);
  }
}
int find_knob(const char *name) {
  if (!name) return -1;
  if (!strncmp(name, "LGS_", 4)) name += 4;
  for (int i = 0; i < T_COUNT; ++i)
    if (!strcmp(name, kKnobs[i].name)) return i;
  return -1;
}

constexpr int kMaxSites = 1024;
struct Site { std::string name; std::atomic<int64_t> hits{0}; };
Site g_sites[kMaxSites];
int g_nsites = 0;
std::mutex g_site_mu;

std::string squeeze(const char *s) {
  std::string o;
  for (; *s; ++s)
    if (*s != ' ' && *s != '\t' && *s != '\n') o.push_back(*s);
  while (o.size() >= 2 && o.front() == '(' && o.back() == ')') o = o.substr(1, o.size() - 2);
  return o;
}
}

int64_t tune(Tune t) {
  std::call_once(g_once, init_knobs);
  return g_val[t].load(std::memory_order_relaxed);
}

int dispatch_site(const char *kernel_text, const char *pretty_function) {
  std::string name = squeeze(kernel_text);
  if (pretty_function) {
    const char *b = strrchr(pretty_function, '[');
    if (b && strchr(b, '=')) name += " " + squeeze(b);
  }
  std::lock_guard<std::mutex> lk(g_site_mu);
  for (int i = 0; i < g_nsites; ++i)
    if (g_sites[i].name == name) return i;
  if (g_nsites >= kMaxSites) return kMaxSites - 1;
  g_sites[g_nsites].name = name;
  return g_nsites++;
}

void dispatch_hit(int site) { g_sites[site].hits.fetch_add(1, std::memory_order_relaxed); }

}

extern "C" {

int lgs_tuning_set(const char *name, int64_t value) {
  std::call_once(lgs::g_once, lgs::init_knobs);
  const int i = lgs::find_knob(name);
  LGS_REQUIRE(i >= 0, std::string("lgs_tuning_set: unknown knob '") + (name ? name : "(null)") + "'");
  lgs::g_val[i].store(value, std::memory_order_relaxed);
  return 0;
}

int lgs_tuning_get(const char *name, int64_t *value) {
  std::call_once(lgs::g_once, lgs::init_knobs);
  const int i = lgs::find_knob(name);
  LGS_REQUIRE(i >= 0 && value, std::string("lgs_tuning_get: unknown knob '") + (name ? name : "(null)") + "'");
  *value = lgs::g_val[i].load(std::memory_order_relaxed);
  return 0;
}

int64_t lgs_tuning_describe(char *buf, int64_t cap) {
  std::call_once(lgs::g_once, lgs::init_knobs);
  std::string s;
  for (int i = 0; i < lgs::T_COUNT; ++i)
    s += std::string(lgs::kKnobs[i].name) + "\t" + std::to_string(lgs::kKnobs[i].def) + "\t" +
         std::to_string(lgs::g_val[i].load()) + "\t" + lgs::kKnobs[i].doc + "\n";
  if (buf && cap > 0) {
    const int64_t n = std::min<int64_t>(cap - 1, (int64_t)s.size());
    memcpy(buf, s.data(), (size_t)n);
    buf[n] = 0;
  }
  return (int64_t)s.size() + 1;
}

int64_t lgs_debug_dispatch_counts(char *buf, int64_t cap, int reset) {
  std::string s;
  {
    std::lock_guard<std::mutex> lk(lgs::g_site_mu);
    for (int i = 0; i < lgs::g_nsites; ++i) {
      const int64_t h = reset ? lgs::g_sites[i].hits.exchange(0) : lgs::g_sites[i].hits.load();
      if (h > 0) s += std::to_string(h) + "\t" + lgs::g_sites[i].name + "\n";
    }
  }
  if (buf && cap > 0) {
    const int64_t n = std::min<int64_t>(cap - 1, (int64_t)s.size());
    memcpy(buf, s.data(), (size_t)n);
    buf[n] = 0;
  }
  return (int64_t)s.size() + 1;
}

}
```

### languagegroundedsemseg_amd/engine.py

```python
import ctypes
import os

from . import build as _build

LGS_F32, LGS_BF16 = 0, 1
LGS_SUPCON_COS, LGS_SUPCON_L2 = 0, 1
LGS_AUG_MAX_SCENES = 32
LGS_AUG_F32X3, LGS_AUG_I32X4 = 0, 1
LGS_COLOR_AUTOCONTRAST, LGS_COLOR_TRANSLATION, LGS_COLOR_JITTER = 1, 2, 4
ABI_VERSION = 18


class PackDesc(ctypes.Structure):
    _fields_ = [("weight", ctypes.c_void_p), ("packed", ctypes.c_void_p), ("bytes", ctypes.c_int64), ("total", ctypes.c_int64),
                ("K", ctypes.c_int), ("cin_w", ctypes.c_int), ("cout_w", ctypes.c_int), ("transposed", ctypes.c_int),
                ("mirror", ctypes.c_int), ("g_real", ctypes.c_int), ("o_real", ctypes.c_int), ("ncp", ctypes.c_int),
                ("nbp", ctypes.c_int), ("dtype", ctypes.c_int)]

class ConvPlanView(ctypes.Structure):
    _fields_ = [("n_pad", ctypes.c_int64), ("n_in", ctypes.c_int64), ("n_out", ctypes.c_int64), ("KS", ctypes.c_int), ("K", ctypes.c_int),
                ("has_nbr", ctypes.c_int), ("has_tile_k", ctypes.c_int), ("has_out_row", ctypes.c_int)]


class ConvPlanQuery(ctypes.Structure):
    _fields_ = [("fwd", ConvPlanView), ("bwd", ConvPlanView), ("ks", ctypes.c_int), ("op", ctypes.c_int), ("transposed", ctypes.c_int),
                ("cin", ctypes.c_int), ("cout", ctypes.c_int), ("dtype", ctypes.c_int), ("epilogue", ctypes.c_int)]


class ConvPlanRegion(ctypes.Structure):
    _fields_ = [("offset", ctypes.c_int64), ("bytes", ctypes.c_int64)]


class ConvPlanInfo(ctypes.Structure):
    _fields_ = [(n, ctypes.c_int) for n in ("path", "tile_id", "sc", "wb", "tm", "nc", "nb_total", "ncp", "nbp", "gc", "wld")] + \
               [("total", ctypes.c_int64)] + \
               [(n, ctypes.c_int) for n in ("pad_input", "scratch_out", "packed_ext_ok", "split", "bn_rows", "can_accumulate")] + \
               [("grid_x", ctypes.c_int64), ("grid_y", ctypes.c_int), ("grid_z", ctypes.c_int)] + \
               [(n, ConvPlanRegion) for n in ("packed", "padded_in", "scratch", "bias", "partials")] + \
               [("bytes_total", ctypes.c_int64), ("workspace_bytes", ctypes.c_int64),
                ("q_bn_partial_rows", ctypes.c_int), ("q_can_accumulate", ctypes.c_int), ("pack_desc", PackDesc)]


class WgradPlanQuery(ctypes.Structure):
    _fields_ = [("fwd", ConvPlanView), ("bwd", ConvPlanView)] + \
               [(n, ctypes.c_int) for n in ("ks", "transposed", "cin", "cout", "dtype", "in_row_stride")]


class WgradPlanInfo(ctypes.Structure):
    _fields_ = [(n, ctypes.c_int) for n in ("path", "bwd_view", "in_place", "pad_in", "pad_gout", "all_cus", "f32_kernel", "t0", "t1",
                                            "pad_a", "pad_b", "slots")] + \
               [("span", ctypes.c_int64)] + \
               [(n, ctypes.c_int) for n in ("n_ranges", "kpw", "tasks_a", "tasks_b", "cpl", "n_chunks", "xcd_map", "ntile")] + \
               [("grid_x", ctypes.c_int64), ("grid_y", ctypes.c_int), ("grid_z", ctypes.c_int), ("lds_bytes", ctypes.c_int),
                ("reduce_blocks", ctypes.c_int64)] + \
               [(n, ConvPlanRegion) for n in ("partials", "padded_in", "padded_gout", "ww_count", "ww_offset", "ww_total", "ww_pair_in",
                                              "ww_pair_out")] + \
               [("bytes_total", ctypes.c_int64), ("workspace_bytes", ctypes.c_int64), ("supports_stride", ctypes.c_int)]


class NormPlanQuery(ctypes.Structure):
    _fields_ = [(n, ctypes.c_int) for n in ("direction", "c", "dtype", "conv_partial_rows", "resident_cap")] + [("n", ctypes.c_int64)]


class NormPlanInfo(ctypes.Structure):
    _fields_ = [("path", ctypes.c_int), ("from_partials", ctypes.c_int), ("reduce_grid", ctypes.c_int), ("rows_per_block", ctypes.c_int64)] + \
               [(n, ctypes.c_int) for n in ("partial_rpb", "fold_rows", "fold_grid", "apply_grid")] + \
               [(n, ConvPlanRegion) for n in ("partials", "sums", "spill")] + \
               [("bytes_total", ctypes.c_int64), ("workspace_bytes", ctypes.c_int64)]


class NormPairPlanInfo(ctypes.Structure):
    _fields_ = [(n, ctypes.c_int) for n in ("path", "single_path", "launches", "reduce_grid")] + [("rows_per_block", ctypes.c_int64)] + \
               [(n, ctypes.c_int) for n in ("fold_rows", "fold_grid", "apply_grid")] + \
               [(n, ConvPlanRegion) for n in ("partials_a", "partials_b", "sums_a", "sums_b")] + \
               [("bytes_total", ctypes.c_int64), ("workspace_bytes", ctypes.c_int64)]


class InstNormPlanQuery(ctypes.Structure):
    _fields_ = [(n, ctypes.c_int) for n in ("direction", "c", "dtype")] + [(n, ctypes.c_int64) for n in ("n_fine", "n_seg", "n_items")]


class InstNormPlanInfo(ctypes.Structure):
    _fields_ = [(n, ctypes.c_int) for n in ("vec", "lanes_log2", "rows_per_apply_block")] + \
               [(n, ctypes.c_int64) for n in ("reduce_grid", "combine_grid", "apply_grid")] + \
               [(n, ConvPlanRegion) for n in ("partials", "sums")] + \
               [("bytes_total", ctypes.c_int64), ("workspace_bytes", ctypes.c_int64)]


class SegPlanQuery(ctypes.Structure):
    _fields_ = [(n, ctypes.c_int) for n in ("family", "c", "dtype", "single_pass", "vec_ok")] + \
               [(n, ctypes.c_int64) for n in ("n_fine", "n_coarse", "n_items")]


class SegPlanInfo(ctypes.Structure):
    _fields_ = [(n, ctypes.c_int) for n in ("vec", "lanes_log2", "combine_lanes_log2")] + \
               [(n, ctypes.c_int64) for n in ("reduce_grid", "combine_grid", "bcast_grid", "max_bwd_grid")] + \
               [(n, ConvPlanRegion) for n in ("partials", "partial_argmax")] + \
               [("bytes_total", ctypes.c_int64), ("workspace_bytes", ctypes.c_int64)]


class KmapRelationQuery(ctypes.Structure):
    _fields_ = [(n, ctypes.c_int) for n in ("entry", "ks", "dilation", "link", "tensor_stride", "out_sorted", "in_origin", "out_origin")]


class KmapRelationInfo(ctypes.Structure):
    _fields_ = [(n, ctypes.c_int) for n in ("rc", "relation", "K", "strided", "bwd_mirror", "transposed_ok")] + \
               [("pairs_only", ctypes.c_int * 2), ("served_by_old_entry", ctypes.c_int)]


class ColorScene(ctypes.Structure):
    _fields_ = [("flags", ctypes.c_int32), ("seed", ctypes.c_int32), ("blend", ctypes.c_float), ("translation", ctypes.c_float * 3),
                ("jitter_std", ctypes.c_float), ("reserved", ctypes.c_float)]


class BnParams(ctypes.Structure):
    _fields_ = [("gamma", ctypes.c_void_p), ("beta", ctypes.c_void_p), ("running_mean", ctypes.c_void_p), ("running_var", ctypes.c_void_p),
                ("num_batches_tracked", ctypes.c_void_p), ("eps", ctypes.c_float), ("momentum", ctypes.c_float)]


class BlockFwd(ctypes.Structure):
    _fields_ = [("km3", ctypes.c_void_p), ("km1", ctypes.c_void_p),
                ("dtype", ctypes.c_int), ("relu_final", ctypes.c_int), ("cin", ctypes.c_int), ("planes", ctypes.c_int),
                ("n", ctypes.c_int64), ("x", ctypes.c_void_p),
                ("w1", ctypes.c_void_p), ("w2", ctypes.c_void_p), ("wd", ctypes.c_void_p),
                ("pk1", ctypes.c_void_p), ("pk2", ctypes.c_void_p), ("pkd", ctypes.c_void_p),
                ("pm1", ctypes.c_int), ("pm2", ctypes.c_int), ("pmd", ctypes.c_int),
                ("n1", BnParams), ("n2", BnParams), ("nd", BnParams),
                ("o1", ctypes.c_void_p), ("y1", ctypes.c_void_p), ("o2", ctypes.c_void_p), ("od", ctypes.c_void_p),
                ("res", ctypes.c_void_p), ("y2", ctypes.c_void_p),
                ("st1", ctypes.c_void_p), ("st2", ctypes.c_void_p), ("std_", ctypes.c_void_p),
                ("conv_ws", ctypes.c_void_p), ("bn_ws", ctypes.c_void_p)]


class BlockBwd(ctypes.Structure):
    _fields_ = [("km3", ctypes.c_void_p), ("km1", ctypes.c_void_p),
                ("dtype", ctypes.c_int), ("relu_final", ctypes.c_int), ("cin", ctypes.c_int), ("planes", ctypes.c_int),
                ("want_gin", ctypes.c_int), ("x_row_stride", ctypes.c_int),
                ("n", ctypes.c_int64), ("dy_row_stride", ctypes.c_int64), ("dy", ctypes.c_void_p),
                ("x", ctypes.c_void_p), ("o1", ctypes.c_void_p), ("y1", ctypes.c_void_p), ("o2", ctypes.c_void_p),
                ("y2", ctypes.c_void_p), ("od", ctypes.c_void_p),
                ("st1", ctypes.c_void_p), ("st2", ctypes.c_void_p), ("std_", ctypes.c_void_p),
                ("w1", ctypes.c_void_p), ("w2", ctypes.c_void_p), ("wd", ctypes.c_void_p),
                ("pk1", ctypes.c_void_p), ("pk2", ctypes.c_void_p), ("pkd", ctypes.c_void_p),
                ("pm1", ctypes.c_int), ("pm2", ctypes.c_int), ("pmd", ctypes.c_int),
                ("gamma1", ctypes.c_void_p), ("beta1", ctypes.c_void_p), ("gamma2", ctypes.c_void_p), ("beta2", ctypes.c_void_p),
                ("gammad", ctypes.c_void_p), ("betad", ctypes.c_void_p),
                ("dx2", ctypes.c_void_p), ("dres", ctypes.c_void_p), ("dy1", ctypes.c_void_p), ("dx1", ctypes.c_void_p),
                ("dxd", ctypes.c_void_p), ("gind", ctypes.c_void_p),
                ("gw1", ctypes.c_void_p), ("gw2", ctypes.c_void_p), ("gwd", ctypes.c_void_p),
                ("dgamma1", ctypes.c_void_p), ("dbeta1", ctypes.c_void_p), ("dgamma2", ctypes.c_void_p), ("dbeta2", ctypes.c_void_p),
                ("dgammad", ctypes.c_void_p), ("dbetad", ctypes.c_void_p),
                ("conv_ws", ctypes.c_void_p), ("bn_ws", ctypes.c_void_p),
                ("wgrad_stream", ctypes.c_void_p), ("wgrad_ws", ctypes.c_void_p), ("fork_event", ctypes.c_void_p),
                ("ev_w1", ctypes.c_void_p), ("ev_w2", ctypes.c_void_p), ("ev_wd", ctypes.c_void_p)]


BLOCK_FWD_FMT = "@PPiiiiqP" + "PPP" + "PPP" + "iii" + "PPPPPff" * 3 + "PPPPPP" + "PPP" + "PP"
BLOCK_BWD_FMT = "@PPiiiiiiqqP" + "PPPPPP" + "PPP" + "PPP" + "PPP" + "iii" + "PPPPPP" + "PPPPPP" + "PPP" + "PPPPPP" + "PP" + "PPPPPP"
import struct as _struct
assert _struct.calcsize(BLOCK_FWD_FMT) == ctypes.sizeof(BlockFwd), (_struct.calcsize(BLOCK_FWD_FMT), ctypes.sizeof(BlockFwd))
assert _struct.calcsize(BLOCK_BWD_FMT) == ctypes.sizeof(BlockBwd), (_struct.calcsize(BLOCK_BWD_FMT), ctypes.sizeof(BlockBwd))
BLOCK_FWD_PACK = _struct.Struct(BLOCK_FWD_FMT)
BLOCK_BWD_PACK = _struct.Struct(BLOCK_BWD_FMT)

_lib = None

EXPORTS = [
    "lgs_abi_version", "lgs_last_error",
    "lgs_tuning_set", "lgs_tuning_get", "lgs_tuning_describe", "lgs_debug_dispatch_counts", "lgs_debug_conv_plan", "lgs_debug_wgrad_plan",
    "lgs_debug_norm_plan", "lgs_debug_instnorm_plan", "lgs_debug_seg_plan", "lgs_debug_kmap_relation",
    "lgs_manager_create", "lgs_manager_destroy", "lgs_manager_insert", "lgs_manager_stride2", "lgs_manager_check",
    "lgs_manager_parent_of", "lgs_manager_map_size", "lgs_manager_get_coords", "lgs_manager_kernel_map", "lgs_manager_kernel_map_ex",
    "lgs_kmap_export",
    "lgs_manager_origin", "lgs_manager_segment_map", "lgs_segmap_size", "lgs_seg_workspace_bytes", "lgs_seg_reduce",
    "lgs_seg_broadcast", "lgs_seg_max_backward",
    "lgs_in_workspace_bytes", "lgs_in_forward", "lgs_in_backward",
    "lgs_conv_workspace_bytes", "lgs_conv_bn_partial_rows", "lgs_conv_forward", "lgs_conv_dgrad", "lgs_conv_wgrad",
    "lgs_conv_wgrad_supports_stride", "lgs_conv_dgrad_can_accumulate", "lgs_conv_dgrad_accumulate",
    "lgs_conv_pack_desc", "lgs_pack_weights_batch",
    "lgs_bn_workspace_bytes", "lgs_bn_forward", "lgs_bn_backward",
    "lgs_bn_pair_workspace_bytes", "lgs_bn_pair_plan", "lgs_debug_norm_pair_plan", "lgs_bn_forward_pair", "lgs_bn_backward_pair",
    "lgs_block_workspace_bytes", "lgs_block_forward", "lgs_block_backward",
    "lgs_bn_stats", "lgs_bn_sync_combine", "lgs_bn_apply", "lgs_bn_backward_reduce", "lgs_bn_backward_apply",
    "lgs_clip_similarity", "lgs_clip_workspace_bytes",
    "lgs_clip_loss_workspace_bytes", "lgs_clip_loss_forward", "lgs_clip_loss_backward",
    "lgs_clip_anchor_grad_workspace_bytes", "lgs_clip_loss_backward_anchors",
    "lgs_ce_forward_backward", "lgs_ce_forward_backward_rows", "lgs_split_stats",
    "lgs_ce_count_valid", "lgs_focal_forward_backward", "lgs_ce_weight_sum", "lgs_seg_metrics",
    "lgs_supcon_sample", "lgs_supcon_forward", "lgs_supcon_backward",
    "lgs_comm_unique_id", "lgs_comm_create", "lgs_comm_create_ipc", "lgs_comm_ipc_open", "lgs_comm_destroy", "lgs_comm_world", "lgs_bn_sync_workspace_bytes",
    "lgs_bn_forward_sync", "lgs_bn_backward_sync",
    "lgs_voxelize", "lgs_label_vote", "lgs_cluster_workspace_bytes", "lgs_cluster", "lgs_sgd_step",
    "lgs_aug_bounds", "lgs_elastic_workspace_bytes", "lgs_elastic_distort", "lgs_voxelize_batched", "lgs_coords_flip_shift",
    "lgs_color_augment", "lgs_aug_status", "lgs_debug_philox",
]


def lib_path():
    return _build.LIB_PATH


def lib():
    global _lib
    if _lib is not None:
        return _lib
    path = lib_path()
    if not os.path.exists(path):
        raise RuntimeError(
            "liblgs_engine.so not found at %s -- run `python -c 'import __graft_entry__ as g; g.build()'` "
            "(or languagegroundedsemseg_amd.build.build()). There is no fallback path." % path)
    L = ctypes.CDLL(path)
    vp, i64, ci = ctypes.c_void_p, ctypes.c_int64, ctypes.c_int
    pi, pi64, pvp = ctypes.POINTER(ctypes.c_int), ctypes.POINTER(ctypes.c_int64), ctypes.POINTER(ctypes.c_void_p)
    cf = ctypes.c_float
    L.lgs_abi_version.restype = ci
    L.lgs_abi_version.argtypes = []
    L.lgs_last_error.restype = ctypes.c_char_p
    L.lgs_last_error.argtypes = []
    sig = {
        "lgs_block_forward": [vp, vp],
        "lgs_block_backward": [vp, vp],
        "lgs_tuning_set": [ctypes.c_char_p, i64],
        "lgs_tuning_get": [ctypes.c_char_p, pi64],
        "lgs_manager_create": [ci, pvp],
        "lgs_manager_destroy": [vp],
        "lgs_manager_insert": [vp, vp, i64, vp, vp, vp, pi, pi64],
        "lgs_manager_stride2": [vp, ci, vp, pi, pi64],
        "lgs_manager_check": [vp, pi],
        "lgs_manager_parent_of": [vp, ci, pi],
        "lgs_manager_map_size": [vp, ci, pi64, pi],
        "lgs_manager_get_coords": [vp, ci, vp, vp],
        "lgs_manager_kernel_map": [vp, ci, ci, ci, vp, pvp],
        "lgs_manager_kernel_map_ex": [vp, ci, ci, ci, ci, vp, pvp],
        "lgs_kmap_export": [vp, vp, vp, vp, vp, pi64],
        "lgs_manager_origin": [vp, vp, pi, pi64],
        "lgs_manager_segment_map": [vp, ci, ci, vp, pvp],
        "lgs_segmap_size": [vp, pi64, pi64],
        "lgs_seg_reduce": [vp, ci, vp, vp, i64, ci, vp, vp, ci, vp, vp],
        "lgs_seg_broadcast": [vp, ci, vp, ci, vp, i64, vp, i64, ci, vp],
        "lgs_seg_max_backward": [vp, vp, vp, ci, vp, ci, vp],
        "lgs_in_forward": [vp, vp, ci, vp, vp, cf, vp, vp, ci, vp, vp],
        "lgs_in_backward": [vp, vp, vp, ci, vp, vp, vp, vp, vp, ci, vp, vp],
        "lgs_conv_forward": [vp, ci, vp, ci, vp, ci, vp, vp, ci, vp, vp, vp, vp, ci, ci, vp],
        "lgs_conv_pack_desc": [vp, ci, ci, ci, ci, ci, ctypes.POINTER(PackDesc)],
        "lgs_pack_weights_batch": [vp, ci, i64, vp],
        "lgs_debug_conv_plan": [ctypes.POINTER(ConvPlanQuery), ctypes.POINTER(ConvPlanInfo)],
        "lgs_debug_wgrad_plan": [ctypes.POINTER(WgradPlanQuery), ctypes.POINTER(WgradPlanInfo)],
        "lgs_debug_norm_plan": [ctypes.POINTER(NormPlanQuery), ctypes.POINTER(NormPlanInfo)],
        "lgs_debug_instnorm_plan": [ctypes.POINTER(InstNormPlanQuery), ctypes.POINTER(InstNormPlanInfo)],
        "lgs_debug_seg_plan": [ctypes.POINTER(SegPlanQuery), ctypes.POINTER(SegPlanInfo)],
        "lgs_debug_kmap_relation": [ctypes.POINTER(KmapRelationQuery), ctypes.POINTER(KmapRelationInfo)],
        "lgs_conv_bn_partial_rows": [vp, ci, ci, ci],
        "lgs_conv_dgrad": [vp, ci, vp, ci, vp, ci, vp, ci, vp, vp, ci, vp],
        "lgs_sgd_step": [vp, vp, vp, vp, i64, cf, cf, cf, cf, ci, vp],
        "lgs_cluster": [vp, vp, vp, i64, cf, ci, vp, ctypes.POINTER(ctypes.c_int32), vp, vp],
        "lgs_voxelize": [vp, i64, ctypes.POINTER(ctypes.c_double), ci, vp, vp],
        "lgs_label_vote": [vp, i64, vp, vp, i64, i64, vp, vp],
        "lgs_conv_wgrad": [vp, ci, vp, ci, vp, ci, vp, ci, vp, ci, vp],
        "lgs_conv_wgrad_supports_stride": [vp, ci, ci, ci, ci, ci],
        "lgs_conv_dgrad_can_accumulate": [vp, ci, ci, ci, ci],
        "lgs_conv_dgrad_accumulate": [vp, ci, vp, ci, vp, ci, vp, ci, vp, vp, ci, vp],
        "lgs_bn_forward": [vp, i64, ci, vp, vp, cf, cf, vp, vp, vp, vp, ci, vp, vp, ci, vp, vp, ci, vp, i64, vp],
        "lgs_bn_backward": [vp, vp, vp, i64, i64, ci, vp, vp, vp, ci, vp, vp, vp, vp, ci, vp, i64, vp],
        "lgs_bn_pair_plan": [ci, i64, ci, ci, ctypes.POINTER(NormPairPlanInfo)],
        "lgs_debug_norm_pair_plan": [ctypes.POINTER(NormPlanQuery), ctypes.POINTER(NormPairPlanInfo)],
        "lgs_bn_forward_pair": [vp, ctypes.POINTER(BnParams), vp, vp, ctypes.POINTER(BnParams), vp, i64, ci, ci, vp, i64, vp, ci, vp, vp],
        "lgs_bn_backward_pair": [vp, vp, vp, vp, vp, ci, vp, vp, vp, vp, i64, i64, ci, vp, vp, vp, vp, vp, vp, vp, ci, vp, i64, vp],
        "lgs_bn_stats": [vp, i64, ci, vp, ci, vp, vp, ci, vp, vp],
        "lgs_bn_apply": [vp, i64, ci, vp, vp, vp, vp, ci, vp, ci, i64, vp],
        "lgs_bn_backward_reduce": [vp, vp, vp, i64, ci, vp, vp, vp, ci, vp, vp, vp, ci, vp, i64, i64, vp],
        "lgs_bn_sync_combine": [vp, ci, ci, cf, cf, vp, vp, vp, vp, vp, vp],
        "lgs_bn_backward_apply": [vp, vp, vp, i64, ci, vp, vp, vp, vp, cf, vp, ci, vp, vp, ci, i64, i64, vp],
        "lgs_clip_similarity": [vp, i64, ci, vp, ci, vp, vp, ci, vp, vp],
        "lgs_ce_forward_backward": [vp, i64, ci, vp, i64, vp, vp, vp, ci, vp],
        "lgs_ce_forward_backward_rows": [vp, i64, ci, vp, i64, vp, vp, vp, vp, ci, vp],
        "lgs_split_stats": [vp, vp, i64, vp, ci, i64, vp, ci, vp],
        "lgs_ce_count_valid": [vp, i64, ci, i64, vp, vp],
        "lgs_focal_forward_backward": [vp, i64, ci, vp, i64, vp, cf, vp, vp, vp, vp, ci, vp],
        "lgs_ce_weight_sum": [vp, i64, ci, i64, vp, vp, ci, vp],
        "lgs_seg_metrics": [vp, i64, ci, vp, i64, vp, vp, vp, ci, vp],
        "lgs_supcon_sample": [vp, i64, ci, i64, vp, vp, vp, vp, vp, ci, ci, i64, vp, vp, vp],
        "lgs_supcon_forward": [vp, i64, ci, vp, vp, ci, vp, ci, i64, ci, ci, vp, vp, vp, vp, ci, vp],
        "lgs_supcon_backward": [vp, i64, ci, vp, vp, ci, vp, ci, i64, ci, ci, vp, vp, vp, vp, vp, ci, vp],
        "lgs_aug_bounds": [vp, i64, ci, vp, ci, vp, vp],
        "lgs_elastic_distort": [vp, i64, vp, ci, vp, ctypes.c_double, ctypes.c_double, i64, vp, ci, ci, vp, i64, vp, vp, vp, vp],
        "lgs_voxelize_batched": [vp, i64, vp, ci, ctypes.POINTER(ctypes.c_double), ci, vp, vp],
        "lgs_coords_flip_shift": [vp, i64, vp, ci, vp, ctypes.POINTER(ctypes.c_int32), ctypes.POINTER(ctypes.c_int32), vp],
        "lgs_color_augment": [vp, i64, vp, ci, vp, ctypes.POINTER(ColorScene), cf, ci, i64, vp, vp],
        "lgs_aug_status": [vp, pi, vp],
        "lgs_debug_philox": [vp, i64, i64, vp, vp],
        "lgs_comm_unique_id": [vp],
        "lgs_comm_create": [vp, ci, ci, ci, ctypes.POINTER(vp)],
        "lgs_comm_create_ipc": [ci, ci, ci, ctypes.POINTER(vp), vp],
        "lgs_comm_ipc_open": [vp, vp],
        "lgs_comm_destroy": [vp],
        "lgs_comm_world": [vp],
        "lgs_bn_forward_sync": [vp, vp, i64, ci, vp, vp, cf, cf, vp, vp, vp, vp, ci, vp, vp, vp, ci, vp, i64, vp],
        "lgs_bn_backward_sync": [vp, vp, vp, vp, i64, ci, vp, vp, vp, vp, ci, vp, vp, vp, vp, ci, vp, i64, i64, vp],
        "lgs_clip_loss_forward": [vp, i64, ci, vp, ci, vp, vp, ci, i64, vp, vp, vp, vp, vp, vp, ci, vp, vp],
        "lgs_clip_loss_backward": [vp, i64, ci, vp, ci, vp, vp, ci, i64, vp, vp, vp, vp, vp, vp, ci, vp],
        "lgs_clip_loss_backward_anchors": [vp, i64, ci, ci, vp, vp, ci, i64, vp, vp, vp, vp, ci, vp, vp],
    }
    for name, args in sig.items():
        f = getattr(L, name)
        f.restype = ci
        f.argtypes = args
    L.lgs_tuning_describe.restype = i64
    L.lgs_tuning_describe.argtypes = [ctypes.c_char_p, i64]
    L.lgs_debug_dispatch_counts.restype = i64
    L.lgs_debug_dispatch_counts.argtypes = [ctypes.c_char_p, i64, ci]
    L.lgs_block_workspace_bytes.restype = i64
    L.lgs_block_workspace_bytes.argtypes = [vp, vp, ci, ci, ci]
    L.lgs_seg_workspace_bytes.restype = i64
    L.lgs_seg_workspace_bytes.argtypes = [vp, ci]
    L.lgs_in_workspace_bytes.restype = i64
    L.lgs_in_workspace_bytes.argtypes = [vp, ci]
    L.lgs_elastic_workspace_bytes.restype = i64
    L.lgs_elastic_workspace_bytes.argtypes = [ci, i64]
    L.lgs_cluster_workspace_bytes.restype = i64
    L.lgs_cluster_workspace_bytes.argtypes = [i64]
    L.lgs_conv_workspace_bytes.restype = i64
    L.lgs_conv_workspace_bytes.argtypes = [vp, ci, ci, ci, ci]
    L.lgs_bn_workspace_bytes.restype = i64
    L.lgs_bn_workspace_bytes.argtypes = [i64, ci]
    L.lgs_bn_pair_workspace_bytes.restype = i64
    L.lgs_bn_pair_workspace_bytes.argtypes = [i64, ci]
    L.lgs_bn_sync_workspace_bytes.restype = i64
    L.lgs_bn_sync_workspace_bytes.argtypes = [i64, ci, ci]
    L.lgs_clip_workspace_bytes.restype = i64
    L.lgs_clip_workspace_bytes.argtypes = [ci, ci, ci]
    L.lgs_clip_loss_workspace_bytes.restype = i64
    L.lgs_clip_loss_workspace_bytes.argtypes = [ci, ci, ci]
    L.lgs_clip_anchor_grad_workspace_bytes.restype = i64
    L.lgs_clip_anchor_grad_workspace_bytes.argtypes = [i64, ci, ci, ci]
    if L.lgs_abi_version() != ABI_VERSION:
        raise RuntimeError("liblgs_engine.so ABI version mismatch")
    _lib = L
    return L


def check(rc):
    if rc != 0:
        msg = lib().lgs_last_error()
        raise RuntimeError("lgs_engine: " + (msg.decode(errors="replace") if msg else "error %d" % rc))


TUNING_EPOCH = 0


def tuning_set(name, value):
    global TUNING_EPOCH
    check(lib().lgs_tuning_set(name.encode(), int(value)))
    TUNING_EPOCH += 1


def tuning_get(name):
    v = ctypes.c_int64()
    check(lib().lgs_tuning_get(name.encode(), ctypes.byref(v)))
    return int(v.value)


class tuning:

    def __init__(self, **knobs):
        self.knobs = knobs

    def __enter__(self):
        self.prev = {k: tuning_get(k) for k in self.knobs}
        for k, v in self.knobs.items():
            tuning_set(k, v)
        return self

    def __exit__(self, *exc):
        for k, v in self.prev.items():
            tuning_set(k, v)


def tuning_table():
    L = lib()
    n = L.lgs_tuning_describe(None, 0)
    buf = ctypes.create_string_buffer(int(n))
    L.lgs_tuning_describe(buf, n)
    rows = []
    for line in buf.value.decode().splitlines():
        name, d, v, doc = line.split("\t", 3)
        rows.append((name, int(d), int(v), doc))
    return rows


def dispatch_counts(reset=False):
    L = lib()
    cap = 1 << 19
    buf = ctypes.create_string_buffer(cap)
    L.lgs_debug_dispatch_counts(buf, cap, 1 if reset else 0)
    out = {}
    for line in buf.value.decode().splitlines():
        c, name = line.split("\t", 1)
        out[name] = int(c)
    return out
```

### languagegroundedsemseg_amd/me/backend_hip.py

```python
import ctypes
import os
import threading
import weakref

import torch

from .. import engine
from .kernel import ALL_CONV_RELATIONS
from .. import tuning as _tuning

_vp = ctypes.c_void_p


def _stream():
    return torch._C._cuda_getCurrentRawStream(torch._C._cuda_getDevice())


class _NoGuard:
    def __enter__(self):
        return self

    def __exit__(self, *exc):
        return False


_NOGUARD = _NoGuard()


def _dev(device):
    if device.index is None or device.index == torch._C._cuda_getDevice():
        return _NOGUARD
    return torch.cuda.device(device)


def _ptr(t):
    return t.data_ptr() if t is not None else None


def _dtype_code(t):
    if t.dtype == torch.float32:
        return engine.LGS_F32
    if t.dtype == torch.bfloat16:
        return engine.LGS_BF16
    raise RuntimeError("lgs_engine supports float32 and bfloat16 features, got %s" % t.dtype)


def _require_dev(t, what):
    if not t.is_cuda:
        raise RuntimeError("%s must live on a HIP device (got %s): the MI355X engine has no CPU fallback"
                           % (what, t.device))


_PACKED = None


def get_packed():
    global _PACKED
    if _PACKED is None:
        _PACKED = PackedWeights()
    return _PACKED


def _row_strided(t, c):
    if t.dim() == 2 and t.shape[1] == c and t.stride(1) == 1 and t.stride(0) > c:
        e = t.element_size()
        if (t.stride(0) * e) % 16 == 0 and t.data_ptr() % 16 == 0:
            return t.stride(0)
    return None


_WS = {}
_BN_WSB = {}


def _bn_ws_bytes(L, n, c):
    b = _BN_WSB.get((n, c))
    if b is None:
        if len(_BN_WSB) > 4096:
            _BN_WSB.clear()
        b = _BN_WSB[(n, c)] = L.lgs_bn_workspace_bytes(n, c)
    return b


_BN_PAIR = {}


def _bn_pair_plan(L, direction, n, c, dt):
    key = (direction, n, c, dt, engine.TUNING_EPOCH)
    v = _BN_PAIR.get(key)
    if v is None:
        if len(_BN_PAIR) > 4096:
            _BN_PAIR.clear()
        info = engine.NormPairPlanInfo()
        engine.check(L.lgs_bn_pair_plan(direction, n, c, dt, ctypes.byref(info)))
        v = _BN_PAIR[key] = (int(info.path), int(info.workspace_bytes))
    return v
_WGRAD_INLINE_BELOW = _tuning.host("WGRAD_INLINE_BELOW")


def _ws(nbytes, device, stream=None):
    if stream is None:
        raw_stream = torch._C._cuda_getCurrentRawStream(device.index if device.index is not None else torch._C._cuda_getDevice())
    else:
        raw_stream = stream.cuda_stream
    key = (device.index, raw_stream)
    t = _WS.get(key)
    nbytes = int(nbytes)
    if t is None or t.numel() < nbytes:
        size = max(nbytes + nbytes // 4, 1 << 20)
        if stream is None:
            t = torch.empty(size, dtype=torch.uint8, device=device)
        else:
            with torch.cuda.stream(stream):
                t = torch.empty(size, dtype=torch.uint8, device=device)
        _WS[key] = t
    return t


def _param_event(param):
    ev = getattr(param, "_lgs_wgrad_event", None)
    if ev is None:
        ev = param._lgs_wgrad_event = torch.cuda.Event()
    return ev


def _raw_event(ev, stream):
    h = ev.cuda_event
    if not h:
        ev.record(stream)
        h = ev.cuda_event
    return int(h.value if hasattr(h, "value") else h)


_DESC_FIELDS = [f for f, _ in engine.PackDesc._fields_]


class _PackEntry:
    __slots__ = ("buf", "desc", "valid", "param_ref", "__weakref__")

    def __init__(self, buf, desc, param):
        self.buf, self.desc, self.valid, self.param_ref = buf, desc, None, weakref.ref(param)

    def cdesc(self):
        d = engine.PackDesc()
        for f in _DESC_FIELDS:
            setattr(d, f, self.desc[f])
        return d


class PackedWeights:

    def __init__(self):
        self.entries = weakref.WeakSet()
        self.epoch = 0
        self._table = None
        self._dirty = True
        self.enabled = _tuning.host("PACK_CACHE") != 0

    def invalidate(self):
        self.epoch += 1

    def lookup(self, cache, km, op, transposed, weight, w32, cin, cout, dt):
        if not self.enabled or cache is None:
            return None, 0
        ck = (op, transposed, cin, cout, dt, engine.TUNING_EPOCH)
        d = km._pdesc.get(ck)
        if d is None:
            d = engine.PackDesc()
            engine.check(engine.lib().lgs_conv_pack_desc(km.h, int(op), int(transposed), int(cin), int(cout), int(dt), ctypes.byref(d)))
            km._pdesc[ck] = d
        if d.bytes == 0:
            return None, 0
        key = (op, int(transposed), dt, d.ncp, d.nbp, d.K, cin, cout, int(d.dtype), int(d.bytes))
        ent = cache.get(key)
        if ent is None:
            buf = torch.empty(int(d.bytes), dtype=torch.uint8, device=w32.device)
            desc = {f: getattr(d, f) for f in _DESC_FIELDS}
            desc["packed"], desc["weight"] = buf.data_ptr(), w32.data_ptr()
            ent = _PackEntry(buf, desc, weight)
            cache[key] = ent
            self.entries.add(ent)
            self._dirty = True
        stamp = (self.epoch, weight._version, w32.data_ptr())
        if ent.desc["weight"] != w32.data_ptr():
            ent.desc["weight"] = w32.data_ptr()
            self._dirty = True
        if ent.valid == stamp:
            return ent.buf, 2
        ent.valid = stamp
        return ent.buf, 1

    def repack_all(self):
        self.epoch += 1
        if not self.enabled:
            return
        live = []
        for e in list(self.entries):
            p = e.param_ref()
            if p is not None and p.dtype == torch.float32 and p.is_contiguous() and p.is_cuda:
                live.append((e, p))
        if not live:
            self._table = None
            return
        ids = tuple(id(e) for e, _ in live)
        if self._dirty or self._table is None or self._table[1] != ids or any(e.desc["weight"] != p.data_ptr() for e, p in live):
            for e, p in live:
                e.desc["weight"] = p.data_ptr()
            arr = (engine.PackDesc * len(live))(*[e.cdesc() for e, _ in live])
            host = torch.frombuffer(bytearray(bytes(arr)), dtype=torch.uint8).clone()
            self._table = (host.to(live[0][0].buf.device), ids, max(int(e.desc["total"]) for e, _ in live))
            self._dirty = False
        tab, _, max_total = self._table
        with _dev(tab.device):
            engine.check(engine.lib().lgs_pack_weights_batch(_ptr(tab), len(live), max_total, _stream()))
        for e, p in live:
            e.valid = (self.epoch, p._version, p.data_ptr())


def invalidate_packed_weights():
    from . import deferred as _deferred
    _deferred.flush_all()
    if _PACKED is not None:
        _PACKED.invalidate()


class HipKernelMap:
    def __init__(self, mgr, handle, in_key, out_key, ks):
        self.mgr, self.h, self.in_key, self.out_key, self.ks = mgr, handle, in_key, out_key, ks
        self.K = ks ** 3
        self._wsb = {}
        self._pdesc = {}

    def _ws_bytes(self, L, cin, cout, dt, op):
        key = (cin, cout, dt, op, engine.TUNING_EPOCH)
        b = self._wsb.get(key)
        if b is None:
            b = self._wsb[key] = L.lgs_conv_workspace_bytes(self.h, cin, cout, dt, op)
        return b

    def export(self):
        L = engine.lib()
        m = ctypes.c_int64(0)
        with _dev(self.mgr.device):
            engine.check(L.lgs_kmap_export(self.h, None, None, None, _stream(), ctypes.byref(m)))
            n = m.value
            k = torch.empty(n, dtype=torch.int32, device=self.mgr.device)
            i = torch.empty_like(k)
            o = torch.empty_like(k)
            if n:
                engine.check(L.lgs_kmap_export(self.h, _ptr(k), _ptr(i), _ptr(o), _stream(), ctypes.byref(m)))
        return k, i, o

    def _rows(self, transposed):
        n_in = self.mgr.map_size(self.in_key)
        n_out = self.mgr.map_size(self.out_key)
        return (n_out, n_in) if transposed else (n_in, n_out)

    def _w32(self, weight):
        cout = weight.shape[-1]
        if weight.dtype == torch.float32 and weight.is_contiguous():
            return weight, weight.numel() // (self.K * cout), cout
        w = weight.detach().reshape(self.K, -1, cout).contiguous().float()
        return w, w.shape[1], cout

    def conv_forward(self, x, weight, bias, transposed, bn_pivot=None, want_bn_stats=False, pack_cache=None):
        _require_dev(x, "features")
        L = engine.lib()
        w, cin, cout = self._w32(weight)
        ld = _row_strided(x, cin) if (cin % (8 if x.dtype == torch.bfloat16 else 4) == 0 and cout % 4 == 0) else None
        if ld is None:
            x = x.contiguous()
        n_in, n_out = self._rows(transposed)
        assert x.shape[0] == n_in and x.shape[1] == cin, (x.shape, n_in, cin)
        dt = _dtype_code(x)
        part = None
        with _dev(x.device):
            out = torch.empty((n_out, cout), dtype=x.dtype, device=x.device)
            ws = _ws(self._ws_bytes(L, cin, cout, dt, 0), x.device)
            b = bias.detach().reshape(-1).contiguous().float() if bias is not None else None
            if want_bn_stats:
                rows = L.lgs_conv_bn_partial_rows(self.h, int(transposed), cout, dt)
                if rows > 0:
                    part = torch.empty((rows, 2, cout), dtype=torch.float32, device=x.device)
            piv = bn_pivot if part is not None else None
            pk, mode = get_packed().lookup(pack_cache, self, 0, transposed, weight, w, cin, cout, dt)
            engine.check(L.lgs_conv_forward(self.h, int(transposed), _ptr(x), cin, _ptr(w), cout, _ptr(b), _ptr(out), dt,
                                            _ptr(ws), _ptr(part), _ptr(piv), _ptr(pk), int(mode), int(ld or 0), _stream()))
        if want_bn_stats:
            return out, ((part, piv) if part is not None else None)
        return out

    def conv_dgrad(self, gout, weight, transposed, pack_cache=None, accumulate_into=None):
        L = engine.lib()
        gout = gout.contiguous()
        w, cin, cout = self._w32(weight)
        n_in, n_out = self._rows(transposed)
        assert gout.shape[0] == n_out and gout.shape[1] == cout
        dt = _dtype_code(gout)
        acc = accumulate_into
        fuse = (acc is not None and acc.is_contiguous() and acc.dtype == gout.dtype and tuple(acc.shape) == (n_in, cin)
                and L.lgs_conv_dgrad_can_accumulate(self.h, int(transposed), cin, cout, dt))
        with _dev(gout.device):
            gin = acc if fuse else torch.empty((n_in, cin), dtype=gout.dtype, device=gout.device)
            ws = _ws(self._ws_bytes(L, cin, cout, dt, 1), gout.device)
            pk, mode = get_packed().lookup(pack_cache, self, 1, transposed, weight, w, cin, cout, dt)
            fn = L.lgs_conv_dgrad_accumulate if fuse else L.lgs_conv_dgrad
            engine.check(fn(self.h, int(transposed), _ptr(gout), cout, _ptr(w), cin, _ptr(gin), dt, _ptr(ws), _ptr(pk), int(mode), _stream()))
            if acc is not None and not fuse:
                gin += acc
        return gin

    def conv_wgrad(self, x, gout, transposed, out=None, stream=None):
        L = engine.lib()
        if stream is not None and (not gout.is_contiguous() or (not x.is_contiguous() and _row_strided(x, x.shape[1]) is None)):
            with torch.cuda.stream(stream):
                return self.conv_wgrad(x, gout, transposed, out=out)
        gout = gout.contiguous()
        cin, cout = x.shape[1], gout.shape[1]
        ld = _row_strided(x, cin) if (x.dtype == torch.bfloat16 and self.ks in (2, 3) and cin % 8 == 0 and cout % 8 == 0) else None
        dt = _dtype_code(x)
        if ld is not None and not L.lgs_conv_wgrad_supports_stride(self.h, int(transposed), cin, cout, dt, int(ld)):
            ld = None
        if ld is None and not x.is_contiguous():
            if stream is not None:
                with torch.cuda.stream(stream):
                    return self.conv_wgrad(x, gout, transposed, out=out)
            x = x.contiguous()
        assert gout.dtype == x.dtype
        raw = stream.cuda_stream if stream is not None else _stream()
        with _dev(x.device):
            if out is not None:
                assert out.dtype == torch.float32 and out.is_contiguous() and out.numel() == self.K * cin * cout
                gw = out
            else:
                gw = torch.empty((self.K, cin, cout), dtype=torch.float32, device=x.device)
            if out is None and stream is not None:
                gw.record_stream(stream)
            ws = _ws(self._ws_bytes(L, cin, cout, dt, 2), x.device, stream)
            engine.check(L.lgs_conv_wgrad(self.h, int(transposed), _ptr(x), cin, _ptr(gout), cout, _ptr(gw), dt, _ptr(ws),
                                          int(ld or 0), raw))
        return gw


class HipSegmentMap:

    def __init__(self, mgr, handle, fine_key, coarse_key):
        self.mgr, self.h, self.fine_key, self.coarse_key = mgr, handle, fine_key, coarse_key
        self.n_fine, self.n_coarse = mgr.map_size(fine_key), mgr.map_size(coarse_key)
        self._wsb = {}

    def _ws_bytes(self, L, c):
        b = self._wsb.get(c)
        if b is None:
            b = self._wsb[c] = L.lgs_seg_workspace_bytes(self.h, c)
        return b


class HipManager:

    def __init__(self, device):
        device = torch.device(device)
        if device.type != "cuda":
            raise RuntimeError("the MI355X engine needs a HIP device, got %s (no CPU fallback)" % device)
        self.device = device if device.index is not None else torch.device("cuda", torch.cuda.current_device())
        h = _vp(None)
        engine.check(engine.lib().lgs_manager_create(self.device.index, ctypes.byref(h)))
        self.h = h
        self._pid = os.getpid()
        self._sizes = {}
        self._kmaps = weakref.WeakValueDictionary()
        self._coords = {}

    def __del__(self):
        try:
            if getattr(self, "h", None) and getattr(self, "_pid", None) == os.getpid():
                engine.lib().lgs_manager_destroy(self.h)
            self.h = None
        except Exception:
            pass

    def check(self):
        f = ctypes.c_int(0)
        engine.check(engine.lib().lgs_manager_check(self.h, ctypes.byref(f)))
        return f.value

    def insert(self, coords):
        _require_dev(coords, "coordinates")
        L = engine.lib()
        coords = coords.to(torch.int32).contiguous()
        n = coords.shape[0]
        key, nu = ctypes.c_int(0), ctypes.c_int64(0)
        with _dev(self.device):
            ui = torch.empty(max(n, 1), dtype=torch.int64, device=self.device)
            inv = torch.empty(max(n, 1), dtype=torch.int64, device=self.device)
            engine.check(L.lgs_manager_insert(self.h, _ptr(coords), n, _ptr(ui), _ptr(inv), _stream(), ctypes.byref(key),
                                              ctypes.byref(nu)))
        self._sizes[key.value] = (nu.value, 1)
        self.inline_wgrad = nu.value < _WGRAD_INLINE_BELOW
        return key.value, nu.value, ui[:nu.value], inv[:n]

    def stride2(self, key):
        L = engine.lib()
        ok, n = ctypes.c_int(0), ctypes.c_int64(0)
        with _dev(self.device):
            engine.check(L.lgs_manager_stride2(self.h, key, _stream(), ctypes.byref(ok), ctypes.byref(n)))
        self._sizes[ok.value] = (n.value, self._sizes[key][1] * 2)
        return ok.value

    def parent_of(self, key):
        fk = ctypes.c_int(-1)
        engine.check(engine.lib().lgs_manager_parent_of(self.h, key, ctypes.byref(fk)))
        return fk.value

    def map_size(self, key):
        return self._sizes[key][0]

    def tensor_stride(self, key):
        return self._sizes[key][1]

    def coords(self, key):
        if key not in self._coords:
            n = self.map_size(key)
            with _dev(self.device):
                c = torch.empty((n, 4), dtype=torch.int32, device=self.device)
                engine.check(engine.lib().lgs_manager_get_coords(self.h, key, _ptr(c), _stream()))
            self._coords[key] = c
        return self._coords[key]

    def origin(self):
        ok, n = ctypes.c_int(0), ctypes.c_int64(0)
        with _dev(self.device):
            engine.check(engine.lib().lgs_manager_origin(self.h, _stream(), ctypes.byref(ok), ctypes.byref(n)))
        self._sizes[ok.value] = (n.value, 0)
        return ok.value

    def segment_map(self, fine_key, coarse_key):
        k = ("seg", fine_key, coarse_key)
        sm = self._kmaps.get(k)
        if sm is None:
            h = _vp(None)
            with _dev(self.device):
                engine.check(engine.lib().lgs_manager_segment_map(self.h, fine_key, coarse_key, _stream(), ctypes.byref(h)))
            sm = HipSegmentMap(self, h, fine_key, coarse_key)
            self._kmaps[k] = sm
        return sm

    kernel_map_relations = ALL_CONV_RELATIONS

    def kernel_map(self, in_key, out_key, ks, dilation=1):
        k = (in_key, out_key, ks, dilation)
        km = self._kmaps.get(k)
        if km is None:
            h = _vp(None)
            with _dev(self.device):
                engine.check(engine.lib().lgs_manager_kernel_map_ex(self.h, in_key, out_key, ks, dilation, _stream(), ctypes.byref(h)))
            km = HipKernelMap(self, h, in_key, out_key, ks)
            self._kmaps[k] = km
        return km


def _written_by_engine(*tensors):
    for t in tensors:
        if t is not None:
            torch.autograd.graph.increment_version(t)


class HipBackend:
    name = "hip"
    bn_counts_batches = True
    bn_out_into = _tuning.host("ZERO_COPY_CAT") != 0
    conv_bn_stats = _tuning.host("CONV_BN_STATS") in ("1", "big")
    conv_bn_stats_min_bytes = (24 << 20) if _tuning.host("CONV_BN_STATS") == "big" else 0

    def want_conv_bn_stats(self, n_rows, cout, esize):
        return self.conv_bn_stats and n_rows * cout * esize >= self.conv_bn_stats_min_bytes

    def __init__(self):
        self._side = {}
        self._cur = {}
        self._fork = {}

    def new_manager(self, device):
        return HipManager(device)

    def invalidate_packed_weights(self):
        invalidate_packed_weights()

    def weights_updated(self):
        get_packed().repack_all()

    def current_stream(self, device):
        idx = device.index if device.index is not None else torch._C._cuda_getDevice()
        raw = torch._C._cuda_getCurrentRawStream(idx)
        s = self._cur.get((idx, raw))
        if s is None:
            s = self._cur[(idx, raw)] = torch.cuda.current_stream(device)
        return s

    def fork_event(self, device):
        idx = device.index if device.index is not None else torch._C._cuda_getDevice()
        ev = self._fork.get(idx)
        if ev is None:
            ev = self._fork[idx] = torch.cuda.Event()
        return ev

    def side_stream(self, device):
        key = device.index if isinstance(device, torch.device) else torch.device(device).index
        if key not in self._side:
            self._side[key] = torch.cuda.Stream(device=device)
        return self._side[key]

    POOL_OPS = {"sum": 0, "avg": 1, "max": 2, "prod": 3}
    BCAST_OPS = {"copy": 0, "scale": 1, "add": 2, "mul": 3, "copy_x": 4}

    def pool_reduce(self, sm, op, x, x2=None):
        _require_dev(x, "features")
        L = engine.lib()
        c = x.shape[1]
        assert x.dim() == 2 and x.shape[0] == sm.n_fine, (tuple(x.shape), sm.n_fine)
        if x.stride(1) != 1 or x.stride(0) < c or (x2 is not None and x2.stride() != x.stride()):
            x = x.contiguous()
            x2 = x2.contiguous() if x2 is not None else None
        if x2 is not None:
            assert x2.shape == x.shape and x2.dtype == x.dtype
        dt = _dtype_code(x)
        with _dev(x.device):
            out = torch.empty((sm.n_coarse, c), dtype=x.dtype, device=x.device)
            amax = torch.empty((sm.n_coarse, c), dtype=torch.int32, device=x.device) if op == "max" else None
            wsb = sm._ws_bytes(L, c)
            ws = _ws(wsb, x.device) if wsb > 0 else None
            engine.check(L.lgs_seg_reduce(sm.h, self.POOL_OPS[op], _ptr(x), _ptr(x2), max(x.stride(0), c), c, _ptr(out), _ptr(amax),
                                          dt, _ptr(ws), _stream()))
        return out, amax

    def pool_broadcast(self, sm, op, g, x=None, out=None, col=0):
        src = x if op == "copy_x" else g
        _require_dev(src, "features")
        L = engine.lib()
        c = src.shape[1]
        if g is not None:
            g = g.contiguous()
            assert g.shape[0] == sm.n_coarse, (tuple(g.shape), sm.n_coarse)
        if x is not None:
            if x.stride(1) != 1 or x.stride(0) < c:
                x = x.contiguous()
            assert x.shape[0] == sm.n_fine and x.shape[1] == c, (tuple(x.shape), sm.n_fine, c)
        dt = _dtype_code(src)
        with _dev(src.device):
            if out is None:
                out = torch.empty((sm.n_fine, c), dtype=src.dtype, device=src.device)
            assert out.is_contiguous() and out.shape[0] == sm.n_fine and out.shape[1] >= col + c and out.dtype == src.dtype
            dst = out.data_ptr() + col * out.element_size()
            engine.check(L.lgs_seg_broadcast(sm.h, self.BCAST_OPS[op], _ptr(g), c, _ptr(x), x.stride(0) if x is not None else c,
                                             dst, out.shape[1], dt, _stream()))
# ... 650 lines not shown
```

Before: 45.58 million.

## Use block-occupancy directory for neighbour lookup and LDS bitonic window sort

Replaces the per-voxel open-addressing hash used to build 3^3 kernel maps with a directory holding one entry per occupied 4x4x4 block (block id, first sorted index, 64-bit occupancy), so a neighbour probe becomes one entry read plus a popcount. It also adds an LDS bitonic sort kernel that sorts the mask codes within each window in a single launch, replacing the multi-launch rocPRIM radix sort over the whole map. A combined fill kernel replaces several small memsets. Both new paths are on by default behind tuning flags, and the change adds more kernel code and some risk in the directory build and the sort.

```diff
diff --git a/include/lgs_engine.h b/include/lgs_engine.h
--- a/include/lgs_engine.h
+++ b/include/lgs_engine.h
@@ -64,6 +64,9 @@
 int lgs_debug_kmap_relation(const lgs_kmap_relation_query *q, lgs_kmap_relation_info *out);
 
 int lgs_kmap_export(lgs_kmap *km, int32_t *k, int32_t *in_row, int32_t *out_row, void *stream, int64_t *m);
+
+int lgs_debug_kmap_tables(lgs_kmap *km, int bwd, int32_t *nbr, int32_t *out_row, uint32_t *mask64, void *stream, int64_t *n_pad,
+                          int *slots, int *present);
 
 int lgs_manager_origin(lgs_manager *mgr, void *stream, int *out_key, int64_t *n_out);
 int lgs_manager_segment_map(lgs_manager *mgr, int fine_key, int coarse_key, void *stream, lgs_segmap **out);
diff --git a/languagegroundedsemseg_amd/csrc/lgs_common.h b/languagegroundedsemseg_amd/csrc/lgs_common.h
--- a/languagegroundedsemseg_amd/csrc/lgs_common.h
+++ b/languagegroundedsemseg_amd/csrc/lgs_common.h
@@ -36,7 +36,7 @@
   T_WW_MIN_ROWS, T_WW_RANGE, T_WGRAD_WIDE, T_BN_FUSED, T_BN_FUSED_MAX_MB, T_BN_FUSED_FWD_MAX_MB, T_BN_FUSED_BLOCKS, T_PS_CUS, T_PS_WIDE3, T_WGRAD_PS,
   T_MASK_WINDOW, T_CONV_SPLIT, T_SMALL_CFG, T_WIDE_GC64, T_ARENA_DBG, T_CONV_WIDE, T_MASK_ORDER,
   T_BN_FOLD, T_BN_FOLD_MAX_MB, T_BN_FOLD_PARTS, T_BN_FOLD_GRID, T_FP32_SPLIT, T_BLOCK_WGRAD_LATE, T_WGRAD_F32_LDS, T_WIDE_SCHED, T_HEAD_TILE, T_POINTWISE,
-  T_INSTANCE_NORM, T_METRICS_BLOCKS, T_SUPCON_FUSED, T_BN_PAIR,
+  T_INSTANCE_NORM, T_METRICS_BLOCKS, T_SUPCON_FUSED, T_BN_PAIR, T_MAP_WINDOW_SORT, T_MAP_BLOCK_DIR,
   T_COUNT
 };
 int64_t tune(Tune t);
diff --git a/languagegroundedsemseg_amd/csrc/lgs_manager.hip b/languagegroundedsemseg_amd/csrc/lgs_manager.hip
--- a/languagegroundedsemseg_amd/csrc/lgs_manager.hip
+++ b/languagegroundedsemseg_amd/csrc/lgs_manager.hip
@@ -1,7 +1,9 @@
 #include "lgs_common.h"
 
 #include <cstring>
+#include <initializer_list>
 #include <memory>
+#include <tuple>
 #include <rocprim/rocprim.hpp>
 
 namespace lgs {
@@ -161,29 +163,19 @@
   if (threadIdx.x <= kPreLevels && l_cnt[threadIdx.x]) atomicAdd(&counts[threadIdx.x], l_cnt[threadIdx.x]);
 }
 
-__global__ void k_build_map3(const uint64_t *skeys, int64_t n, int64_t n_pad, int ts, const uint64_t *hkeys,
-                             const int32_t *hvals, uint64_t capm1, int32_t *nbr, uint32_t *pmask) {
-  int64_t p = (int64_t)blockIdx.x * blockDim.x + threadIdx.x;
-  bool live = p < n;
-  int b = 0, x = 0, y = 0, z = 0;
-  if (live) unpack_key(skeys[p], b, x, y, z);
-  uint32_t m = 0;
-#pragma unroll 1
-  for (int g = 0; g < 3; ++g) {
-    uint64_t key[9], slot[9], hk[9];
-    bool ok[9];
-    const int zz = z + (g - 1) * ts;
-#pragma unroll
-    for (int j = 0; j < 9; ++j) {
-      const int xx = x + (j % 3 - 1) * ts, yy = y + (j / 3 - 1) * ts;
-      ok[j] = live && (((unsigned)xx | (unsigned)yy | (unsigned)zz) < (1u << kCoordBits));
-      key[j] = ok[j] ? pack_key(b, xx, yy, zz) : 0ull;
-      slot[j] = hash64(key[j]) & capm1;
-    }
-#pragma unroll
-    for (int j = 0; j < 9; ++j) hk[j] = ok[j] ? hkeys[slot[j]] : kEmpty;
-#pragma unroll
-    for (int j = 0; j < 9; ++j) {
+struct HashRef {
+  const uint64_t *hkeys;
+  const int32_t *hvals;
+  uint64_t capm1;
+  template <int NP>
+  __device__ inline void find(const uint64_t (&key)[NP], bool (&ok)[NP], int32_t (&r)[NP]) const {
+    uint64_t slot[NP], hk[NP];
+#pragma unroll
+    for (int j = 0; j < NP; ++j) slot[j] = hash64(key[j]) & capm1;
+#pragma unroll
+    for (int j = 0; j < NP; ++j) hk[j] = ok[j] ? hkeys[slot[j]] : kEmpty;
+#pragma unroll
+    for (int j = 0; j < NP; ++j) {
       if (ok[j]) {
         uint64_t cur = hk[j], sl = slot[j];
         while (cur != key[j] && cur != kEmpty) {
@@ -194,9 +186,95 @@
         ok[j] = cur == key[j];
       }
     }
+#pragma unroll
+    for (int j = 0; j < NP; ++j) r[j] = ok[j] ? hvals[slot[j]] : -1;
+  }
+};
+struct DirEnt { uint64_t id, occ; int32_t first, pad[3]; };
+static_assert(sizeof(DirEnt) == 32, "DirEnt is read as two 16-byte halves");
+struct DirRef {
+  const DirEnt *ent;
+  uint64_t capm1;
+  int sh;
+  const int32_t *order;
+  template <int NP>
+  __device__ inline void find(const uint64_t (&key)[NP], bool (&ok)[NP], int32_t (&r)[NP]) const {
+    uint32_t slot[NP];
+    ulonglong2 e[NP];
+    int32_t first[NP];
+#pragma unroll
+    for (int j = 0; j < NP; ++j) slot[j] = (uint32_t)(hash64(key[j] >> (sh + 6)) & capm1);
+#pragma unroll
+    for (int j = 0; j < NP; ++j) {
+      e[j] = ok[j] ? *reinterpret_cast<const ulonglong2 *>(ent + slot[j]) : make_ulonglong2(kEmpty, 0ull);
+      first[j] = ok[j] ? ent[slot[j]].first : 0;
+    }
+#pragma unroll
+    for (int j = 0; j < NP; ++j) {
+      if (ok[j]) {
+        const uint64_t id = key[j] >> (sh + 6);
+        uint32_t sl = slot[j];
+        while (e[j].x != id && e[j].x != kEmpty) {
+          sl = (sl + 1) & (uint32_t)capm1;
+          e[j] = *reinterpret_cast<const ulonglong2 *>(ent + sl);
+          first[j] = ent[sl].first;
+        }
+        const int cell = (int)((key[j] >> sh) & 63);
+        ok[j] = e[j].x == id && ((e[j].y >> cell) & 1ull);
+        first[j] += __popcll(e[j].y & ((1ull << cell) - 1ull));
+      }
+    }
+#pragma unroll
+    for (int j = 0; j < NP; ++j) r[j] = ok[j] ? (order ? order[first[j]] : first[j]) : -1;
+  }
+};
+__global__ void k_dir_fill(DirEnt *dir, int64_t cap) {
+  int64_t i = (int64_t)blockIdx.x * blockDim.x + threadIdx.x;
+  if (i >= cap) return;
+  ulonglong2 *q = reinterpret_cast<ulonglong2 *>(dir + i);
+  q[0] = make_ulonglong2(kEmpty, 0ull);
+  q[1] = make_ulonglong2(0ull, 0ull);
+}
+__global__ void k_dir_build(const uint64_t *skeys, int64_t n, int sh, DirEnt *dir, uint64_t capm1, int *d_err) {
+  int64_t p = (int64_t)blockIdx.x * blockDim.x + threadIdx.x;
+  if (p >= n) return;
+  const uint64_t id = skeys[p] >> (sh + 6);
+  if (p > 0 && (skeys[p - 1] >> (sh + 6)) == id) return;
+  uint64_t occ = 0;
+  for (int64_t q = p; q < n && q < p + 64; ++q) {
+    const uint64_t k = skeys[q];
+    if ((k >> (sh + 6)) != id) break;
+    occ |= 1ull << ((k >> sh) & 63);
+  }
+  uint64_t s = hash64(id) & capm1;
+  for (uint64_t tries = 0; tries <= capm1; ++tries) {
+    unsigned long long prev = atomicCAS(reinterpret_cast<unsigned long long *>(&dir[s].id), (unsigned long long)kEmpty, (unsigned long long)id);
+    if (prev == kEmpty) { dir[s].occ = occ; dir[s].first = (int32_t)p; return; }
+    s = (s + 1) & capm1;
+  }
+  if (d_err) atomicOr(d_err, 8);
+}
+
+template <typename L>
+__global__ __launch_bounds__(256) void k_build_map3(const uint64_t *skeys, int64_t n, int64_t n_pad, int ts, L look, int32_t *nbr, uint32_t *pmask) {
+  int64_t p = (int64_t)blockIdx.x * blockDim.x + threadIdx.x;
+  bool live = p < n;
+  int b = 0, x = 0, y = 0, z = 0;
+  if (live) unpack_key(skeys[p], b, x, y, z);
+  uint32_t m = 0;
+#pragma unroll 1
+  for (int g = 0; g < 3; ++g) {
+    uint64_t key[9];
+    bool ok[9];
+    const int zz = z + (g - 1) * ts;
+#pragma unroll
+    for (int j = 0; j < 9; ++j) {
+      const int xx = x + (j % 3 - 1) * ts, yy = y + (j / 3 - 1) * ts;
+      ok[j] = live && (((unsigned)xx | (unsigned)yy | (unsigned)zz) < (1u << kCoordBits));
+      key[j] = ok[j] ? pack_key(b, xx, yy, zz) : 0ull;
+    }
     int32_t r[9];
-#pragma unroll
-    for (int j = 0; j < 9; ++j) r[j] = ok[j] ? hvals[slot[j]] : -1;
+    look.template find<9>(key, ok, r);
 #pragma unroll
     for (int j = 0; j < 9; ++j) {
       const int k = 9 * g + j;
@@ -236,6 +314,105 @@
   unsigned wb = 1;
   while ((1ull << wb) - 1 < nw) ++wb;
   return 32u + wb > 64u ? 64u : 32u + wb;
+}
+constexpr int kWsMinLog2 = 10, kWsMaxLog2 = 14;
+inline int window_sort_log2(int64_t window) {
+  for (int l = kWsMinLog2; l <= kWsMaxLog2; ++l)
+    if (window == (1ll << l)) return l;
+  return -1;
+}
+inline size_t window_sort_lds(int log2w) { return (((size_t)1 << log2w) + ((size_t)1 << (log2w - 4))) * sizeof(double); }
+static_assert((((size_t)1 << kWsMaxLog2) + ((size_t)1 << (kWsMaxLog2 - 4))) * 8 <= 160 * 1024, "k_window_sort: LDS budget of one CU");
+constexpr unsigned long long kWsOne = 0x3ff0000000000000ull, kWsMant = 0x000fffffffffffffull;
+__device__ inline double ws_min(double x, double y) { double r; asm("v_min_f64 %0, %1, %2" : "=v"(r) : "v"(x), "v"(y)); return r; }
+__device__ inline double ws_max(double x, double y) { double r; asm("v_max_f64 %0, %1, %2" : "=v"(r) : "v"(x), "v"(y)); return r; }
+__device__ inline void ws_cmpx(double &lo, double &hi) {
+  double a;
+  asm("v_min_f64 %0, %1, %2\n\tv_max_f64 %1, %1, %2" : "=&v"(a), "+v"(hi) : "v"(lo));
+  lo = a;
+}
+template <int B>
+__device__ inline int ws_base(int t) { return ((t >> B) << (B + 4)) | (t & ((1 << B) - 1)); }
+template <int B>
+__device__ inline void ws_store(double *lds, const double (&e)[16], int t) {
+  const int base = ws_base<B>(t);
+  double *q = lds + base + (base >> 4);
+#pragma unroll
+  for (int r = 0; r < 16; ++r) q[(r << B) + ((r << B) >> 4)] = e[r];
+}
+template <int B>
+__device__ inline void ws_pass(double *lds, double (&e)[16], int t, int hi, int m, bool store) {
+  const int base = ws_base<B>(t);
+  const double *q = lds + base + (base >> 4);
+  const unsigned long long flip = ((base >> m) & 1) ? kWsMant : 0ull;
+#pragma unroll
+  for (int r = 0; r < 16; ++r) e[r] = __longlong_as_double((long long)((unsigned long long)__double_as_longlong(q[(r << B) + ((r << B) >> 4)]) ^ flip));
+#pragma unroll
+  for (int s = 3; s >= 0; --s) {
+    if (B + s > hi) continue;
+#pragma unroll
+    for (int r = 0; r < 16; ++r)
+      if (!(r & (1 << s))) ws_cmpx(e[r], e[r | (1 << s)]);
+  }
+#pragma unroll
+  for (int r = 0; r < 16; ++r) e[r] = __longlong_as_double((long long)((unsigned long long)__double_as_longlong(e[r]) ^ flip));
+  if (store) ws_store<B>(lds, e, t);
+}
+__global__ __launch_bounds__(1024) void k_window_sort(const uint32_t *__restrict__ pmask, int64_t n, int64_t n_pad, int log2w, int order,
+                                                      int32_t *__restrict__ perm) {
+  extern __shared__ double ws_lds[];
+  const int t = threadIdx.x;
+  const int64_t w0 = (int64_t)blockIdx.x << log2w;
+  double e[16];
+#pragma unroll
+  for (int r = 0; r < 16; ++r) {
+    const int64_t p = w0 + 16 * t + r;
+    const uint32_t code = p < n ? mask_sort_code(pmask[p], order) : 0xffffffffu;
+    e[r] = __longlong_as_double((long long)(kWsOne | ((unsigned long long)code << 14) | (unsigned)(16 * t + r)));
+  }
+#pragma unroll
+  for (int m = 1; m <= 4; ++m) {
+#pragma unroll
+    for (int s = m - 1; s >= 0; --s) {
+#pragma unroll
+      for (int r = 0; r < 16; ++r) {
+        if (r & (1 << s)) continue;
+        const bool up = (((16 * t) | r) & (1 << m)) == 0;
+        const double a = ws_min(e[r], e[r | (1 << s)]), b = ws_max(e[r], e[r | (1 << s)]);
+        e[r] = up ? a : b; e[r | (1 << s)] = up ? b : a;
+      }
+    }
+  }
+  ws_store<0>(ws_lds, e, t);
+  __syncthreads();
+  for (int m = 5; m <= log2w; ++m) {
+    for (int hi = m - 1; hi >= 0;) {
+      const int b = hi >= 3 ? hi - 3 : 0;
+      const bool store = !(m == log2w && b == 0);
+      switch (b) {
+        case 0: ws_pass<0>(ws_lds, e, t, hi, m, store); break;
+        case 1: ws_pass<1>(ws_lds, e, t, hi, m, store); break;
+        case 2: ws_pass<2>(ws_lds, e, t, hi, m, store); break;
+        case 3: ws_pass<3>(ws_lds, e, t, hi, m, store); break;
+        case 4: ws_pass<4>(ws_lds, e, t, hi, m, store); break;
+        case 5: ws_pass<5>(ws_lds, e, t, hi, m, store); break;
+        case 6: ws_pass<6>(ws_lds, e, t, hi, m, store); break;
+        case 7: ws_pass<7>(ws_lds, e, t, hi, m, store); break;
+        case 8: ws_pass<8>(ws_lds, e, t, hi, m, store); break;
+        case 9: ws_pass<9>(ws_lds, e, t, hi, m, store); break;
+        default: ws_pass<10>(ws_lds, e, t, hi, m, store); break;
+      }
+      __syncthreads();
+      hi = b - 1;
+    }
+  }
+  if (w0 + 16 * t >= n_pad) return;
+  int4 *dst = reinterpret_cast<int4 *>(perm + w0 + 16 * t);
+  int32_t v[16];
+#pragma unroll
+  for (int r = 0; r < 16; ++r) v[r] = (int32_t)(w0 + (int64_t)(__double_as_longlong(e[r]) & 0x3fff));
+#pragma unroll
+  for (int r = 0; r < 16; r += 4) dst[r >> 2] = make_int4(v[r], v[r + 1], v[r + 2], v[r + 3]);
 }
 __global__ void k_permute_map3(const int32_t *nbr_tmp, const uint32_t *pmask, const int32_t *perm, const int32_t *order,
                                int64_t n, int64_t n_pad, int32_t *nbr, int32_t *out_row, uint32_t *mask64) {
@@ -251,15 +428,15 @@
   if ((threadIdx.x & 63) == 0) mask64[q >> 6] = m;
 }
 
-__global__ void k_build_map3_fine(const uint64_t *fkeys, int64_t n, int64_t n_pad, int log2ts, const uint64_t *hkeys,
-                                  const int32_t *hvals, uint64_t capm1, int32_t *nbr, uint32_t *pmask) {
+template <typename L>
+__global__ __launch_bounds__(256) void k_build_map3_fine(const uint64_t *fkeys, int64_t n, int64_t n_pad, int log2ts, L look, int32_t *nbr, uint32_t *pmask) {
   int64_t p = (int64_t)blockIdx.x * blockDim.x + threadIdx.x;
   const bool live = p < n;
   int b = 0, x = 0, y = 0, z = 0;
   if (live) unpack_key(fkeys[p], b, x, y, z);
   const int ts = 1 << log2ts;
   const int ox = (x >> log2ts) & 1, oy = (y >> log2ts) & 1, oz = (z >> log2ts) & 1;
-  uint64_t key[8], slot[8], hk[8];
+  uint64_t key[8];
   int kk[8];
   bool ok[8];
 #pragma unroll
@@ -270,29 +447,13 @@
     ok[j] = live && (ox || !jx) && (oy || !jy) && (oz || !jz) && (((unsigned)xx | (unsigned)yy | (unsigned)zz) < (1u << kCoordBits));
     kk[j] = (dx + 1) + 3 * (dy + 1) + 9 * (dz + 1);
     key[j] = ok[j] ? pack_key(b, xx, yy, zz) : 0ull;
-    slot[j] = hash64(key[j]) & capm1;
-  }
-#pragma unroll
-  for (int j = 0; j < 8; ++j) hk[j] = ok[j] ? hkeys[slot[j]] : kEmpty;
-#pragma unroll
-  for (int j = 0; j < 8; ++j) {
-    if (ok[j]) {
-      uint64_t cur = hk[j], sl = slot[j];
-      while (cur != key[j] && cur != kEmpty) {
-        sl = (sl + 1) & capm1;
-        cur = hkeys[sl];
-      }
-      slot[j] = sl;
-      ok[j] = cur == key[j];
-    }
-  }
+  }
+  int32_t r[8];
+  look.template find<8>(key, ok, r);
   uint32_t m = 0;
 #pragma unroll
   for (int j = 0; j < 8; ++j)
     if (ok[j]) m |= 1u << kk[j];
-  int32_t r[8];
-#pragma unroll
-  for (int j = 0; j < 8; ++j) r[j] = ok[j] ? hvals[slot[j]] : -1;
   for (int k = 0; k < 27; ++k) {
     int32_t v = -1;
 #pragma unroll
@@ -376,6 +537,16 @@
 __global__ void k_fill_i32(int32_t *p, int64_t n, int32_t v) {
   int64_t i = (int64_t)blockIdx.x * blockDim.x + threadIdx.x;
   if (i < n) p[i] = v;
+}
+constexpr int kFillSegs = 4;
+struct FillSegs { int32_t *p[kFillSegs]; int64_t n[kFillSegs]; int32_t v[kFillSegs]; };
+__global__ void k_fill_segs(FillSegs f) {
+  int64_t i = (int64_t)blockIdx.x * blockDim.x + threadIdx.x;
+#pragma unroll
+  for (int j = 0; j < kFillSegs; ++j) {
+    if (i < f.n[j]) { f.p[j][i] = f.v[j]; return; }
+    i -= f.n[j];
+  }
 }
 __global__ void k_build_map2_fine(const uint32_t *kk_sorted, const int32_t *pp_sorted, int64_t n, const int32_t *goff,
                                   const int32_t *gsrc, const int32_t *fine_cidx, const int32_t *forder,
@@ -481,6 +652,8 @@
   uint64_t *hkeys = nullptr;
   int32_t *hvals = nullptr;
   int64_t hcap = 0;
+  DirEnt *dir = nullptr;
+  int64_t dcap = 0;
   int fine_key = -1, coarse_key = -1;
   bool origin = false;
   int32_t *cstart = nullptr;
@@ -673,6 +846,37 @@
   return 0;
 }
 
+int ensure_dir(lgs_manager *m, CoordMap &cm, hipStream_t s) {
+  if (cm.dir) return 0;
+  int64_t blocks = cm.n;
+  const int lv = cm.log2ts + 2;
+  if (lv <= kPreLevels && m->precount[lv - 1] >= 0 && m->precount[lv - 1] < blocks) blocks = m->precount[lv - 1];
+  int64_t cap = 1024;
+  while (cap < 2 * blocks) cap <<= 1;
+  cm.dcap = cap;
+  if (dalloc(m, &cm.dir, cap, s)) return 1;
+  LGS_KLAUNCH(k_dir_fill, nblk(cap), 256, 0, s, cm.dir, cap);
+  if (cm.n > 0) LGS_KLAUNCH(k_dir_build, nblk(cm.n), 256, 0, s, cm.skeys, cm.n, 3 * cm.log2ts, cm.dir, (uint64_t)(cap - 1), m->d_err);
+  LGS_HIP(hipGetLastError());
+  return 0;
+}
+inline bool use_block_dir() { return tune(T_MAP_BLOCK_DIR) != 0; }
+int ensure_lookup(lgs_manager *m, CoordMap &cm, hipStream_t s) { return use_block_dir() ? ensure_dir(m, cm, s) : ensure_hash(m, cm, s); }
+inline HashRef hash_ref(const CoordMap &cm) { return HashRef{cm.hkeys, cm.hvals, (uint64_t)(cm.hcap - 1)}; }
+inline DirRef dir_ref(const CoordMap &cm) { return DirRef{cm.dir, (uint64_t)(cm.dcap - 1), 3 * cm.log2ts, cm.order}; }
+
+int fill_segs(hipStream_t s, std::initializer_list<std::tuple<void *, int64_t, int32_t>> segs) {
+  FillSegs f = {};
+  int64_t total = 0;
+  int j = 0;
+  for (const auto &g : segs) {
+    f.p[j] = reinterpret_cast<int32_t *>(std::get<0>(g)); f.n[j] = std::get<1>(g); f.v[j] = std::get<2>(g);
+    total += f.n[j++];
+  }
+  LGS_KLAUNCH(k_fill_segs, nblk(total), 256, 0, s, f);
+  return 0;
+}
+
 int scan_incl(lgs_manager *m, const int32_t *in, int32_t *out, int64_t n, hipStream_t s) {
   size_t tb = 0;
   LGS_HIP(rocprim::inclusive_scan(nullptr, tb, in, out, (size_t)n, rocprim::plus<int32_t>(), s));
@@ -698,14 +902,26 @@
   return scan_incl(m, head, cincl, n, s);
 }
 
-int sort_map3(lgs_manager *m, int64_t n, int64_t n_pad, const int32_t *nbr_tmp, const uint32_t *pmask, const int32_t *order, uint64_t *keys,
-              uint64_t *skeys2, int32_t *vals, int32_t *perm, int32_t *nbr, int32_t *orow, uint32_t *mask, hipStream_t s) {
-  const int window = (int)tune(T_MASK_WINDOW);
-  LGS_KLAUNCH(k_mask_sort_keys, (unsigned)(n_pad / 256), 256, 0, s, pmask, n, n_pad, window, (int)tune(T_MASK_ORDER), keys, vals);
-  if (sort_pairs(m, keys, skeys2, vals, perm, n_pad, 0, mask_sort_bits(n_pad, window), s)) return 1;
-  LGS_KLAUNCH(k_permute_map3, (unsigned)(n_pad / 256), 256, 0, s, nbr_tmp, pmask, perm, order, n, n_pad, nbr, orow, mask);
-  LGS_HIP(hipGetLastError());
-  return 0;
+int window_perm(lgs_manager *m, int64_t n, int64_t n_pad, const uint32_t *pmask, int32_t *perm, hipStream_t s) {
+  const int64_t window = tune(T_MASK_WINDOW);
+  const int order = (int)tune(T_MASK_ORDER);
+  const int log2w = tune(T_MAP_WINDOW_SORT) != 0 ? window_sort_log2(window) : -1;
+  if (log2w >= 0) {
+    static bool attr_set = false;
+    if (!attr_set) {
+      LGS_HIP(hipFuncSetAttribute(reinterpret_cast<const void *>(&k_window_sort), hipFuncAttributeMaxDynamicSharedMemorySize, (int)window_sort_lds(kWsMaxLog2)));
+      attr_set = true;
+    }
+    int l = log2w;
+    while (l > kWsMinLog2 && n_pad <= (1ll << (l - 1))) --l;
+    LGS_KLAUNCH(k_window_sort, (unsigned)((n_pad + (1ll << l) - 1) >> l), 1u << (l - 4), window_sort_lds(l), s, pmask, n, n_pad, l, order, perm);
+    return 0;
+  }
+  uint64_t *keys, *skeys2; int32_t *vals;
+  if (dalloc(m, &keys, n_pad, s) || dalloc(m, &skeys2, n_pad, s) || dalloc(m, &vals, n_pad, s)) return 1;
+  LGS_KLAUNCH(k_mask_sort_keys, (unsigned)(n_pad / 256), 256, 0, s, pmask, n, n_pad, (int)window, order, keys, vals);
+  if (sort_pairs(m, keys, skeys2, vals, perm, n_pad, 0, mask_sort_bits(n_pad, (int)window), s)) return 1;
+  return dfree_now(m, keys, s) || dfree_now(m, skeys2, s) || dfree_now(m, vals, s);
 }
 
 template <typename Build>
@@ -713,16 +929,15 @@
   v = View();
   v.n_pad = st.n_pad; v.n_out = st.n; v.n_in = n_in; v.KS = 27; v.K = 27;
   if (st.n == 0) return 0;
-  int32_t *nbr, *orow, *nbr_tmp, *vals, *perm; uint32_t *mask, *pmask; uint64_t *keys, *skeys2;
+  int32_t *nbr, *orow, *nbr_tmp, *perm; uint32_t *mask, *pmask;
   if (dalloc(m, &nbr, 27 * st.n_pad, s) || dalloc(m, &mask, st.n_pad / kGroup, s) || dalloc(m, &orow, st.n_pad, s) ||
-      dalloc(m, &nbr_tmp, 27 * st.n_pad, s) || dalloc(m, &pmask, st.n_pad, s) || dalloc(m, &keys, st.n_pad, s) ||
-      dalloc(m, &skeys2, st.n_pad, s) || dalloc(m, &vals, st.n_pad, s) || dalloc(m, &perm, st.n_pad, s))
+      dalloc(m, &nbr_tmp, 27 * st.n_pad, s) || dalloc(m, &pmask, st.n_pad, s) || dalloc(m, &perm, st.n_pad, s))
     return 1;
   if (build(nbr_tmp, pmask)) return 1;
-  if (sort_map3(m, st.n, st.n_pad, nbr_tmp, pmask, st.order, keys, skeys2, vals, perm, nbr, orow, mask, s)) return 1;
-  if (dfree_now(m, nbr_tmp, s) || dfree_now(m, pmask, s) || dfree_now(m, keys, s) || dfree_now(m, skeys2, s) ||
-      dfree_now(m, vals, s) || dfree_now(m, perm, s))
-    return 1;
+  if (window_perm(m, st.n, st.n_pad, pmask, perm, s)) return 1;
+  LGS_KLAUNCH(k_permute_map3, (unsigned)(st.n_pad / 256), 256, 0, s, nbr_tmp, pmask, perm, st.order, st.n, st.n_pad, nbr, orow, mask);
+  LGS_HIP(hipGetLastError());
+  if (dfree_now(m, nbr_tmp, s) || dfree_now(m, pmask, s) || dfree_now(m, perm, s)) return 1;
   v.nbr = nbr; v.mask64 = mask; v.out_row = orow;
   return 0;
 }
@@ -735,14 +950,16 @@
 
 int probe_view27(lgs_manager *m, const CoordMap &st, const CoordMap &probed, int scale, hipStream_t s, View &v) {
   return make_view27(m, st, probed.n, s, v, [&](int32_t *nbr_tmp, uint32_t *pmask) {
-    LGS_KLAUNCH(k_build_map3, (unsigned)(st.n_pad / 256), 256, 0, s, st.skeys, st.n, st.n_pad, scale, probed.hkeys, probed.hvals,
-                (uint64_t)(probed.hcap - 1), nbr_tmp, pmask);
+    if (use_block_dir())
+      LGS_KLAUNCH(k_build_map3<DirRef>, (unsigned)(st.n_pad / 256), 256, 0, s, st.skeys, st.n, st.n_pad, scale, dir_ref(probed), nbr_tmp, pmask);
+    else
+      LGS_KLAUNCH(k_build_map3<HashRef>, (unsigned)(st.n_pad / 256), 256, 0, s, st.skeys, st.n, st.n_pad, scale, hash_ref(probed), nbr_tmp, pmask);
     return 0;
   });
 }
 
 int build_conv3(lgs_manager *m, CoordMap &ci, int dilation, hipStream_t s, lgs_kmap *km) {
-  if (ci.n > 0 && ensure_hash(m, ci, s)) return 1;
+  if (ci.n > 0 && ensure_lookup(m, ci, s)) return 1;
   View v;
   if (probe_view27(m, ci, ci, dilation * ci.ts, s, v)) return 1;
   km->fwd = v;
@@ -767,13 +984,10 @@
         dalloc(m, &cnt, 8, s) || dalloc(m, &goff, 9, s) || dalloc(m, &gsrc, 9, s) || dalloc(m, &g_nbr, gp, s) ||
         dalloc(m, &g_out, gp, s) || dalloc(m, &tile_k, gp / kGroup, s))
       return 1;
-    LGS_HIP(hipMemsetAsync(cnt, 0, 8 * sizeof(int32_t), s));
+    if (fill_segs(s, {{cnt, 8, 0}, {g_nbr, gp, -1}, {g_out, gp, -1}, {tile_k, gp / kGroup, -1}})) return 1;
     LGS_KLAUNCH(k_child_keys, nblk(n), 256, 0, s, ci.skeys, n, shift, kk, pp, cnt);
     if (sort_pairs(m, kk, kks, pp, pps, n, 0, 3, s)) return 1;
     LGS_KLAUNCH(k_group_offsets, 1, 64, 0, s, cnt, goff, gsrc);
-    LGS_KLAUNCH(k_fill_i32, nblk(gp), 256, 0, s, g_nbr, gp, -1);
-    LGS_KLAUNCH(k_fill_i32, nblk(gp), 256, 0, s, g_out, gp, -1);
-    LGS_KLAUNCH(k_fill_i32, nblk(gp / kGroup), 256, 0, s, tile_k, gp / kGroup, -1);
     LGS_KLAUNCH(k_build_map2_fine, nblk(n), 256, 0, s, kks, pps, n, goff, gsrc, co.fine_cidx, ci.order, g_nbr,
                        g_out, tile_k);
     LGS_HIP(hipGetLastError());
@@ -787,11 +1001,13 @@
 }
 
 int build_conv3_s2(lgs_manager *m, CoordMap &ci, CoordMap &co, hipStream_t s, lgs_kmap *km) {
-  if (ci.n > 0 && (ensure_hash(m, ci, s) || ensure_hash(m, co, s))) return 1;
+  if (ci.n > 0 && (ensure_lookup(m, ci, s) || ensure_lookup(m, co, s))) return 1;
   if (probe_view27(m, co, ci, ci.ts, s, km->fwd)) return 1;
   return make_view27(m, ci, co.n, s, km->bwd, [&](int32_t *nbr_tmp, uint32_t *pmask) {
-    LGS_KLAUNCH(k_build_map3_fine, (unsigned)(ci.n_pad / 256), 256, 0, s, ci.skeys, ci.n, ci.n_pad, ci.log2ts, co.hkeys, co.hvals,
-                (uint64_t)(co.hcap - 1), nbr_tmp, pmask);
+    if (use_block_dir())
+      LGS_KLAUNCH(k_build_map3_fine<DirRef>, (unsigned)(ci.n_pad / 256), 256, 0, s, ci.skeys, ci.n, ci.n_pad, ci.log2ts, dir_ref(co), nbr_tmp, pmask);
+    else
+      LGS_KLAUNCH(k_build_map3_fine<HashRef>, (unsigned)(ci.n_pad / 256), 256, 0, s, ci.skeys, ci.n, ci.n_pad, ci.log2ts, hash_ref(co), nbr_tmp, pmask);
     return 0;
   });
 }
@@ -922,23 +1138,17 @@
     return 0;
   }
   if (!m->d_err) { if (dalloc(m, &m->d_err, 1, s)) return 1; }
-  LGS_HIP(hipMemsetAsync(m->d_err, 0, sizeof(int), s));
-  uint64_t *keys, *skeys; int32_t *vals, *svals, *head, *runid, *is_first, *urow;
-  if (dalloc(m, &keys, n, s) || dalloc(m, &skeys, n, s) || dalloc(m, &vals, n, s) || dalloc(m, &svals, n, s) ||
+  uint64_t *keys, *skeys; int32_t *vals, *svals, *head, *runid, *is_first, *urow, *lvl_counts;
+  if (dalloc(m, &lvl_counts, kPreLevels + 1, s) || dalloc(m, &keys, n, s) || dalloc(m, &skeys, n, s) || dalloc(m, &vals, n, s) || dalloc(m, &svals, n, s) ||
       dalloc(m, &head, n, s) || dalloc(m, &runid, n, s) || dalloc(m, &is_first, n, s) || dalloc(m, &urow, n + 1, s))
     return 1;
+  if (fill_segs(s, {{m->d_err, 1, 0}, {urow, 1, 0}, {lvl_counts, kPreLevels + 1, 0}})) return 1;
   LGS_KLAUNCH(k_pack_keys, nblk(n), 256, 0, s, coords, n, keys, vals, m->d_err);
   if (sort_pairs(m, keys, skeys, vals, svals, n, 0, 64, s)) return 1;
   LGS_KLAUNCH(k_heads, nblk(n), 256, 0, s, skeys, n, ~0ull, head);
   LGS_KLAUNCH(k_mark_first, nblk(n), 256, 0, s, svals, head, n, is_first);
   if (scan_incl(m, head, runid, n, s)) return 1;
-  {
-    LGS_HIP(hipMemsetAsync(urow, 0, sizeof(int32_t), s));
-    if (scan_incl(m, is_first, urow + 1, n, s)) return 1;
-  }
-  int32_t *lvl_counts;
-  if (dalloc(m, &lvl_counts, kPreLevels + 1, s)) return 1;
-  LGS_HIP(hipMemsetAsync(lvl_counts, 0, sizeof(int32_t) * (kPreLevels + 1), s));
+  if (scan_incl(m, is_first, urow + 1, n, s)) return 1;
   LGS_KLAUNCH(k_count_levels, (unsigned)((n + 256 * kCountPerThread - 1) / (256 * kCountPerThread)), 256, 0, s, skeys, n, lvl_counts);
   int32_t h_nu = 0; int h_err = 0; int32_t h_lvl[kPreLevels + 1];
   LGS_HIP(hipMemcpyAsync(&h_nu, urow + n, sizeof(int32_t), hipMemcpyDeviceToHost, s));
@@ -1073,6 +1283,23 @@
   out->pairs_only[0] = t.wgrad_pairs_only(false); out->pairs_only[1] = t.wgrad_pairs_only(true);
   out->served_by_old_entry = t.old_entry;
   return 0;
+}
+
+int lgs_debug_kmap_tables(lgs_kmap *km, int bwd, int32_t *nbr, int32_t *out_row, uint32_t *mask64, void *stream, int64_t *n_pad, int *slots,
+                          int *present) {
+  LGS_REQUIRE(km && n_pad && slots && present, "lgs_debug_kmap_tables: null argument");
+  lgs_manager *m = km->mgr;
+  const View &v = bwd ? km->bwd : km->fwd;
+  *n_pad = v.n_pad; *slots = v.KS;
+  *present = (v.nbr ? 1 : 0) | (v.out_row ? 2 : 0) | (v.mask64 ? 4 : 0);
+  if (!nbr && !out_row && !mask64) return 0;
+  hipStream_t caller = (hipStream_t)stream, s = m->ms;
+  DeviceGuard guard(m->device);
+  if (begin_from_caller(m, caller)) return 1;
+  if (nbr && v.nbr && v.n_pad > 0) LGS_HIP(hipMemcpyAsync(nbr, v.nbr, sizeof(int32_t) * (size_t)(v.KS * v.n_pad), hipMemcpyDeviceToDevice, s));
+  if (out_row && v.out_row && v.n_pad > 0) LGS_HIP(hipMemcpyAsync(out_row, v.out_row, sizeof(int32_t) * (size_t)v.n_pad, hipMemcpyDeviceToDevice, s));
+  if (mask64 && v.mask64 && v.n_pad > 0) LGS_HIP(hipMemcpyAsync(mask64, v.mask64, sizeof(uint32_t) * (size_t)(v.n_pad / kGroup), hipMemcpyDeviceToDevice, s));
+  return publish(m, caller, true);
 }
 
 int lgs_manager_origin(lgs_manager *m, void *stream, int *out_key, int64_t *n_out) {
diff --git a/languagegroundedsemseg_amd/csrc/lgs_tuning.hip b/languagegroundedsemseg_amd/csrc/lgs_tuning.hip
--- a/languagegroundedsemseg_amd/csrc/lgs_tuning.hip
+++ b/languagegroundedsemseg_amd/csrc/lgs_tuning.hip
@@ -75,6 +75,13 @@
                               "passes instead of 8), and lgs_bn_forward_pair / lgs_bn_backward_pair run the two norms of a downsample block on shared "
                               "reads (5 instead of 7 passes forward, 10 instead of 13 backward, 3 launches instead of 6); 0 = the single calls, dy "
                               "masked in both launches.  Bit-identical either way"},
+    {T_MAP_WINDOW_SORT, "MAP_WINDOW_SORT", 1, "3^3 maps, the window mask sort (A/B): 1 = k_window_sort, one workgroup per MASK_WINDOW positions sorts (mask code, index in "
+                                              "window) in LDS with a bitonic network, one launch per view; 0 = 64-bit keys (window, code) through rocPRIM's radix "
+                                              "sort over the whole map (13 launches per view).  A window that is no power of two in 1024 .. 16384 takes the radix "
+                                              "sort either way.  The permutation is identical"},
+    {T_MAP_BLOCK_DIR, "MAP_BLOCK_DIR", 1, "3^3 maps, neighbour lookup (A/B): 1 = a directory with one entry per occupied 4 x 4 x 4 block of cells {block id, first "
+                                          "sorted position, 64-bit occupancy}; a probe is one entry and a popcount; 0 = the open-addressing hash with one slot "
+                                          "per voxel (>= 2 n slots of 12 bytes).  The tables are identical"},
 };
 std::atomic<int64_t> g_val[T_COUNT];
 std::once_flag g_once;
diff --git a/languagegroundedsemseg_amd/engine.py b/languagegroundedsemseg_amd/engine.py
--- a/languagegroundedsemseg_amd/engine.py
+++ b/languagegroundedsemseg_amd/engine.py
@@ -171,7 +171,7 @@
     "lgs_debug_norm_plan", "lgs_debug_instnorm_plan", "lgs_debug_seg_plan", "lgs_debug_kmap_relation",
     "lgs_manager_create", "lgs_manager_destroy", "lgs_manager_insert", "lgs_manager_stride2", "lgs_manager_check",
     "lgs_manager_parent_of", "lgs_manager_map_size", "lgs_manager_get_coords", "lgs_manager_kernel_map", "lgs_manager_kernel_map_ex",
-    "lgs_kmap_export",
+    "lgs_kmap_export", "lgs_debug_kmap_tables",
     "lgs_manager_origin", "lgs_manager_segment_map", "lgs_segmap_size", "lgs_seg_workspace_bytes", "lgs_seg_reduce",
     "lgs_seg_broadcast", "lgs_seg_max_backward",
     "lgs_in_workspace_bytes", "lgs_in_forward", "lgs_in_backward",
@@ -233,6 +233,7 @@
         "lgs_manager_kernel_map": [vp, ci, ci, ci, vp, pvp],
         "lgs_manager_kernel_map_ex": [vp, ci, ci, ci, ci, vp, pvp],
         "lgs_kmap_export": [vp, vp, vp, vp, vp, pi64],
+        "lgs_debug_kmap_tables": [vp, ci, vp, vp, vp, vp, pi64, pi, pi],
         "lgs_manager_origin": [vp, vp, pi, pi64],
         "lgs_manager_segment_map": [vp, ci, ci, vp, pvp],
         "lgs_segmap_size": [vp, pi64, pi64],
diff --git a/languagegroundedsemseg_amd/me/backend_hip.py b/languagegroundedsemseg_amd/me/backend_hip.py
--- a/languagegroundedsemseg_amd/me/backend_hip.py
+++ b/languagegroundedsemseg_amd/me/backend_hip.py
@@ -250,6 +250,18 @@
             if n:
                 engine.check(L.lgs_kmap_export(self.h, _ptr(k), _ptr(i), _ptr(o), _stream(), ctypes.byref(m)))
         return k, i, o
+
+    def tables(self, bwd=False):
+        L = engine.lib()
+        n_pad, slots, present = ctypes.c_int64(0), ctypes.c_int(0), ctypes.c_int(0)
+        with _dev(self.mgr.device):
+            engine.check(L.lgs_debug_kmap_tables(self.h, int(bwd), None, None, None, _stream(), ctypes.byref(n_pad), ctypes.byref(slots), ctypes.byref(present)))
+            n, has = n_pad.value, present.value
+            mk = lambda bit, *shape: torch.empty(*shape, dtype=torch.int32, device=self.mgr.device) if has & bit else None
+            nbr, orow, mask = mk(1, slots.value, n), mk(2, n), mk(4, n // 64)
+            engine.check(L.lgs_debug_kmap_tables(self.h, int(bwd), _ptr(nbr) if nbr is not None else None, _ptr(orow) if orow is not None else None,
+                                                 _ptr(mask) if mask is not None else None, _stream(), ctypes.byref(n_pad), ctypes.byref(slots), ctypes.byref(present)))
+        return nbr, orow, mask
 
     def _rows(self, transposed):
         n_in = self.mgr.map_size(self.in_key)
```

Result: faster. 46.45 million, median of 6 (+1.9%).
